# tumberger/gnark-fork

Hardware: AMD Instinct MI355X
Metric: Groth16 prove time + MSM G1 throughput (Mscalar-mul/s) BN254 2^24 R1CS, 1/2/4/8 GPU (higher is better)
Workload: dtype u32 limbs (BN254 Fp/Fr Montgomery, integer)

## Files before the change

gnark-fork_amd/csrc/groth16.hip:

```cpp
#include "common.h"
#include "curve.cuh"
#include "stage.h"
#include <chrono>
#include <future>
#include <memory>
#include <mutex>
#include <thread>
#include <vector>
#include <cstdlib>
#include <cstring>

struct gg_domain;
struct gg_msm_base;

namespace gg {
struct MsmSort;
struct MsmScratch;
struct MsmWork;
void compute_h_device(gg_domain* d, Fr* A, Fr* B, Fr* C, Fr* H, hipStream_t st);
void msm_device(gg_msm_base* b, const Fr* scalars_dev, void* out_jac, hipStream_t st);
size_t msm_scalars_needed(gg_msm_base* b);
gg_msm_base* msm_base_create_internal(int group, const void* host_points, size_t n,
                                      const uint32_t* sidx, int window_bits, bool keep_inf, int groups);
int choose_groups_multi(const double* bytes, const int* W, int k, double extra);
bool msm_same_shape(const gg_msm_base* a, const gg_msm_base* b);
MsmSort* msm_own_sort(gg_msm_base* b);
void msm_prepare_dev(gg_msm_base* b, MsmSort* s, const Fr* scalars_dev, hipStream_t st, int slog = 0,
                     uint32_t sres = 0);
void msm_finish_dev(gg_msm_base* b, MsmSort* s, void* out_jac, hipStream_t st, MsmScratch* scr = nullptr);
MsmWork* msm_work_new();
void msm_work_delete(MsmWork* w);
MsmSort* msm_work_sort(MsmWork* w);
void msm_prepare_derived_dev(gg_msm_base* a, MsmSort* sa, gg_msm_base* b, MsmSort* sb, const uint32_t* bmap,
                             hipStream_t st);
bool msm_derivable(const gg_msm_base* a, const gg_msm_base* b);
void msm_build_bmap(const gg_msm_base* a, const gg_msm_base* b, DevBuf& bmap);
MsmScratch* msm_work_scratch(MsmWork* w);
int msm_base_window(const gg_msm_base* b);
int choose_c(size_t n, size_t point_bytes, int total_bits);
void hshard_run(gg_hshard* hs, const Fr* a, const Fr* b, const Fr* c, size_t len, bool compact, Fr* send,
                Fr* recv, gg_exchange_fn xchg, void* ctx, hipStream_t st);
size_t hshard_m(const gg_hshard* hs, int* rank, int* world, int* log_n);
Fr* hshard_h(gg_hshard* hs);
int hshard_curve(const gg_hshard* hs);
}

struct DistH {
    gg_hshard* hs;
    gg_exchange_fn xchg;
    void* ctx;
    gg::Fr *send, *recv;
};

using namespace gg;

struct CurveBn254 {
    using FrT = Fr;
    using G1F = Fp;
    using G2F = Fp2;
    static constexpr int curve = GG_CURVE_BN254, g1 = GG_G1, g2 = GG_G2, total_bits = 255;
};
struct CurveBls12381 {
    using FrT = FrBls;
    using G1F = FpBls;
    using G2F = Fp2Bls;
    static constexpr int curve = GG_CURVE_BLS12_381, g1 = GG_BLS12_381_G1, g2 = GG_BLS12_381_G2, total_bits = 256;
};
struct PointSizes {
    size_t g1a, g2a, g1j, g2j;
};
static PointSizes point_sizes(int curve) {
    if (curve == GG_CURVE_BN254) return {64, 128, 96, 192};
    return {96, 192, 144, 288};
}

struct WireBases {
    gg_msm_base_t A = nullptr, B = nullptr, K = nullptr, B2 = nullptr;
    bool share_AK = false, share_B = false;
    bool derive_B = false;
    DevBuf bmap;
    int groups = 1;
    WireBases() = default;
    WireBases(const WireBases&) = delete;
    WireBases& operator=(const WireBases&) = delete;
    ~WireBases() {
        for (gg_msm_base_t b : {A, B, K, B2})
            if (b) gg_msm_base_release(b);
    }
};

struct WorkSet {
    MsmWork *A = nullptr, *B = nullptr, *K = nullptr, *B2 = nullptr;
    WorkSet() {
        A = msm_work_new();
        B = msm_work_new();
        K = msm_work_new();
        B2 = msm_work_new();
    }
    WorkSet(const WorkSet&) = delete;
    WorkSet& operator=(const WorkSet&) = delete;
    ~WorkSet() {
        for (MsmWork* w : {A, B, K, B2})
            if (w) msm_work_delete(w);
    }
};

struct gg_groth16_pk {
    int curve = GG_CURVE_BN254;
    int log_n = 0;
    size_t n = 0;
    gg_domain_t dom = nullptr;
    std::shared_ptr<WireBases> wb;
    gg_msm_base_t A = nullptr, B = nullptr, K = nullptr, Z = nullptr, B2 = nullptr;
    int slog = 0;
    uint32_t spart = 0;
    std::unique_ptr<WorkSet> work;
    uint8_t alpha[96], beta[96], delta[96], beta2[192], delta2[192];
    size_t n_wires = 0, nb_public = 0;
    size_t wire_lo = 0, wire_hi = 0, z_lo = 0, nZ = 0;
    bool share_AK = false, share_B = false;
    DevBuf wires, sa, sb, sc;
    hipStream_t s0 = nullptr, s1 = nullptr, s2 = nullptr, s3 = nullptr, s4 = nullptr;
    TaskQueue tq[5];
    hipStream_t* const* active() {
        act[0] = &s0, act[1] = &s1, act[2] = &s2, act[3] = &s3, act[4] = &s4;
        return act;
    }
    hipStream_t* act[5] = {};
    hipStream_t hprio = nullptr;
    std::unique_ptr<Stager> stager;
    int device = 0;
    std::mutex mu;
    ~gg_groth16_pk() {
        stager.reset();
        work.reset();
        wb.reset();
        if (Z) gg_msm_base_release(Z);
        if (dom) gg_domain_release(dom);
        task_streams_release(tq, 5, device);
        if (hprio) (void)hipStreamDestroy(hprio);
    }
};

static thread_local double g_timings[9];
static thread_local double g_ext[3];

static void ck(int rc) {
    if (rc != GG_OK) throw Error(rc, gg_last_error());
}

static std::shared_ptr<WireBases> wire_bases_build(int curve, int log_n, const void* g1_A, size_t nA,
                                                   const void* g1_B, size_t nB, const void* g1_K, size_t nK,
                                                   const void* g2_B, const uint8_t* inf_A, const uint8_t* inf_B,
                                                   size_t n_wires, size_t nb_public, const uint32_t* k_wire_index,
                                                   size_t lo, size_t hi, size_t nZ) {
    GG_CHECK(inf_A && inf_B, GG_ERR_INVALID_ARG, "null infinity masks");
    GG_CHECK(nb_public <= n_wires, GG_ERR_INVALID_ARG, "nb_public > n_wires");
    GG_CHECK(lo <= hi && hi <= n_wires, GG_ERR_INVALID_ARG, "bad wire shard range");
    GG_CHECK(curve == GG_CURVE_BN254 || curve == GG_CURVE_BLS12_381, GG_ERR_INVALID_ARG, "bad curve");
    const PointSizes ps = point_sizes(curve);
    const int g1 = curve == GG_CURVE_BN254 ? GG_G1 : GG_BLS12_381_G1;
    const int g2 = curve == GG_CURVE_BN254 ? GG_G2 : GG_BLS12_381_G2;
    const int tbits = curve == GG_CURVE_BN254 ? 255 : 256;
    std::vector<uint32_t> ia, ib, ik;
    for (size_t i = lo; i < hi; i++) {
        if (!inf_A[i]) ia.push_back((uint32_t)(i - lo));
        if (!inf_B[i]) ib.push_back((uint32_t)(i - lo));
    }
    GG_CHECK(ia.size() == nA, GG_ERR_INVALID_ARG, "len(pk.G1.A) != n_wires - NbInfinityA (shard)");
    GG_CHECK(ib.size() == nB, GG_ERR_INVALID_ARG, "len(pk.G1.B) != n_wires - NbInfinityB (shard)");
    ik.resize(nK);
    const size_t k0 = std::max(lo, nb_public);
    for (size_t i = 0; i < nK; i++) {
        size_t w = k_wire_index ? (size_t)k_wire_index[i] : k0 + i;
        GG_CHECK(w >= lo && w < hi, GG_ERR_INVALID_ARG, "K wire index outside the shard");
        ik[i] = (uint32_t)(w - lo);
    }
    GG_CHECK(nA == 0 || g1_A, GG_ERR_INVALID_ARG, "null g1_A");
    GG_CHECK(nB == 0 || (g1_B && g2_B), GG_ERR_INVALID_ARG, "null g1_B / g2_B");
    GG_CHECK(nK == 0 || g1_K, GG_ERR_INVALID_ARG, "null g1_K");
    const size_t nw = hi - lo;
    const int cAK = choose_c(std::max<size_t>(nw, 1), ps.g1a, tbits);
    int cB = choose_c(std::max<size_t>(nB, 1), 128, tbits);
    const bool try_derive = getenv("GG_G16_B_DERIVE") && atoi(getenv("GG_G16_B_DERIVE")) != 0;
    if (try_derive && cAK >= cB && cAK - cB <= 2 && nB) cB = cAK;
    if (const char* e = getenv("GG_G16_B_WINDOW")) cB = std::max(4, std::min(24, atoi(e)));
    const int cZ = choose_c(std::max<size_t>(nZ, 1), ps.g1a, tbits);
    auto wb = std::make_shared<WireBases>();
    {
        auto W = [&](int c) { return (tbits + c - 1) / c; };
        const double g1a = (double)ps.g1a, g2a = (double)ps.g2a;
        const double bytes[5] = {W(cAK) * (double)nw * g1a, W(cAK) * (double)nw * g1a, W(cB) * (double)nB * g1a,
                                 W(cB) * (double)nB * g2a, W(cZ) * (double)nZ * g1a};
        const int ws[5] = {W(cAK), W(cAK), W(cB), W(cB), W(cZ)};
        const double extra = 16.0 * (W(cAK) * (double)nw + W(cB) * (double)nB + W(cZ) * (double)nZ) +
                             12.0 * 32.0 * (double)((size_t)1 << log_n);
        wb->groups = choose_groups_multi(bytes, ws, 5, extra);
    }
    {
        const size_t pb = ps.g1a;
        std::vector<uint8_t> dense(nw * pb, 0);
        for (size_t j = 0; j < nA; j++) memcpy(&dense[(size_t)ia[j] * pb], (const uint8_t*)g1_A + j * pb, pb);
        wb->A = msm_base_create_internal(g1, dense.data(), nw, nullptr, cAK, true, wb->groups);
        std::fill(dense.begin(), dense.end(), 0);
        for (size_t j = 0; j < nK; j++) memcpy(&dense[(size_t)ik[j] * pb], (const uint8_t*)g1_K + j * pb, pb);
        wb->K = msm_base_create_internal(g1, dense.data(), nw, nullptr, cAK, true, wb->groups);
    }
    wb->B = msm_base_create_internal(g1, g1_B, nB, ib.data(), cB, false, wb->groups);
    wb->B2 = msm_base_create_internal(g2, g2_B, nB, ib.data(), msm_base_window(wb->B), false, wb->groups);
    wb->share_AK = msm_same_shape(wb->A, wb->K);
    wb->share_B = msm_same_shape(wb->B, wb->B2);
    if (try_derive && wb->share_B && msm_derivable(wb->A, wb->B)) {
        msm_build_bmap(wb->A, wb->B, wb->bmap);
        wb->derive_B = true;
    }
    return wb;
}

static void h_priority_ab(gg_groth16_pk* pk) {
    if (!(getenv("GG_G16_H_PRIORITY") && atoi(getenv("GG_G16_H_PRIORITY")))) return;
    if (!pk->hprio) create_copy_stream(&pk->hprio);
    pk->s1 = pk->hprio;
}

static void pk_finish(gg_groth16_pk* pk, std::shared_ptr<WireBases> wb, int curve, int log_n,
                      const void* omega_mont, const void* coset_gen_mont, const void* g1_Z, size_t z_lo, size_t nZ,
                      const void* alpha1, const void* beta1, const void* delta1, const void* beta2,
                      const void* delta2, size_t n_wires, size_t nb_public, size_t lo, size_t hi, int slog,
                      uint32_t spart) {
    GG_CHECK(omega_mont && coset_gen_mont && alpha1 && beta1 && delta1 && beta2 && delta2,
             GG_ERR_INVALID_ARG, "null argument");
    GG_CHECK(log_n >= 0 && log_n <= 28, GG_ERR_INVALID_ARG, "log_n out of range");
    const PointSizes ps = point_sizes(curve);
    const int g1 = curve == GG_CURVE_BN254 ? GG_G1 : GG_BLS12_381_G1;
    const int tbits = curve == GG_CURVE_BN254 ? 255 : 256;
    pk->curve = curve;
    pk->log_n = log_n;
    pk->n = (size_t)1 << log_n;
    pk->n_wires = n_wires;
    pk->nb_public = nb_public;
    pk->wire_lo = lo;
    pk->wire_hi = hi;
    pk->z_lo = z_lo;
    pk->nZ = nZ;
    const size_t nz_full = pk->n > 1 ? pk->n - 1 : 0;
    GG_CHECK(z_lo + nZ <= nz_full, GG_ERR_INVALID_ARG,
             "Z shard beyond domain cardinality - 1 (setup.go:266)");
    GG_CHECK(nZ == 0 || g1_Z, GG_ERR_INVALID_ARG, "null g1_Z");
    GG_HIP(hipGetDevice(&pk->device));
    memcpy(pk->alpha, alpha1, ps.g1a);
    memcpy(pk->beta, beta1, ps.g1a);
    memcpy(pk->delta, delta1, ps.g1a);
    memcpy(pk->beta2, beta2, ps.g2a);
    memcpy(pk->delta2, delta2, ps.g2a);
    ck(gg_domain_create_ex(curve, log_n, omega_mont, coset_gen_mont, &pk->dom));
    pk->wb = std::move(wb);
    pk->A = pk->wb->A;
    pk->B = pk->wb->B;
    pk->K = pk->wb->K;
    pk->B2 = pk->wb->B2;
    pk->share_AK = pk->wb->share_AK;
    pk->share_B = pk->wb->share_B;
    if (slog) {
        int cmin = 64;
        for (gg_msm_base_t b : {pk->A, pk->B})
            if (msm_scalars_needed(b)) cmin = std::min(cmin, msm_base_window(b));
        GG_CHECK(slog <= cmin - 2, GG_ERR_INVALID_ARG, "bucket stripe too fine for the tables' windows");
        GG_CHECK(spart < (1u << slog), GG_ERR_INVALID_ARG, "stripe part out of range");
        pk->slog = slog;
        pk->spart = spart;
        pk->work.reset(new WorkSet());
    }
    const int cZ = choose_c(std::max<size_t>(nZ, 1), ps.g1a, tbits);
    pk->Z = msm_base_create_internal(g1, g1_Z, nZ, nullptr, cZ, false, pk->wb->groups);
    int cur = 0;
    GG_HIP(hipGetDevice(&cur));
    task_streams_init(pk->active(), pk->tq, 5, cur, true);
    h_priority_ab(pk);
}

static void pk_build(gg_groth16_pk* pk, int curve, int log_n, const void* omega_mont, const void* coset_gen_mont,
                     const void* g1_A, size_t nA, const void* g1_B, size_t nB, const void* g1_Z,
                     size_t z_lo, size_t nZ, const void* g1_K, size_t nK, const void* alpha1,
                     const void* beta1, const void* delta1, const void* g2_B, const void* beta2,
                     const void* delta2, const uint8_t* inf_A, const uint8_t* inf_B, size_t n_wires,
                     size_t nb_public, const uint32_t* k_wire_index, size_t lo, size_t hi) {
    GG_CHECK(log_n >= 0 && log_n <= 28, GG_ERR_INVALID_ARG, "log_n out of range");
    auto wb = wire_bases_build(curve, log_n, g1_A, nA, g1_B, nB, g1_K, nK, g2_B, inf_A, inf_B, n_wires, nb_public,
                               k_wire_index, lo, hi, nZ);
    pk_finish(pk, std::move(wb), curve, log_n, omega_mont, coset_gen_mont, g1_Z, z_lo, nZ, alpha1, beta1, delta1,
              beta2, delta2, n_wires, nb_public, lo, hi, 0, 0);
}

namespace gg {
std::shared_ptr<WireBases> g16_wire_bases(int curve, int log_n, const void* g1_A, size_t nA, const void* g1_B,
                                          size_t nB, const void* g1_K, size_t nK, const void* g2_B,
                                          const uint8_t* inf_A, const uint8_t* inf_B, size_t n_wires,
                                          size_t nb_public, const uint32_t* k_wire_index, size_t nZ) {
    return wire_bases_build(curve, log_n, g1_A, nA, g1_B, nB, g1_K, nK, g2_B, inf_A, inf_B, n_wires, nb_public,
                            k_wire_index, 0, n_wires, nZ);
}
gg_groth16_pk* g16_stripe_shard(std::shared_ptr<WireBases> wb, int curve, int log_n, const void* omega_mont,
                                const void* coset_gen_mont, const void* g1_Z, size_t z_lo, size_t nZ,
                                const void* alpha1, const void* beta1, const void* delta1, const void* beta2,
                                const void* delta2, size_t n_wires, size_t nb_public, int slog, uint32_t spart) {
    std::unique_ptr<gg_groth16_pk> pk(new gg_groth16_pk());
    pk_finish(pk.get(), std::move(wb), curve, log_n, omega_mont, coset_gen_mont, g1_Z, z_lo, nZ, alpha1, beta1,
              delta1, beta2, delta2, n_wires, nb_public, 0, n_wires, slog, spart);
    return pk.release();
}
int g16_wire_window(int curve, size_t n_wires, size_t nB) {
    const PointSizes ps = point_sizes(curve);
    const int tbits = curve == GG_CURVE_BN254 ? 255 : 256;
    int c = 64;
    if (n_wires) c = std::min(c, choose_c(n_wires, ps.g1a, tbits));
    if (nB) c = std::min(c, choose_c(nB, 128, tbits));
    return c;
}
void g16_restream(gg_groth16_pk* pk, bool dedicated) {
    std::lock_guard<std::mutex> lk(pk->mu);
    task_streams_switch(pk->active(), pk->tq, 5, pk->device, dedicated);
    h_priority_ab(pk);
}
}

extern "C" int gg_groth16_pk_create_ex(int curve, int log_n, const void* omega_mont, const void* coset_gen_mont,
                                       const void* g1_A, size_t nA, const void* g1_B, size_t nB,
                                       const void* g1_Z, size_t nZ, const void* g1_K, size_t nK,
                                       const void* alpha1, const void* beta1, const void* delta1,
                                       const void* g2_B, const void* beta2, const void* delta2,
                                       const uint8_t* inf_A, const uint8_t* inf_B, size_t n_wires,
                                       size_t nb_public, const uint32_t* k_wire_index,
                                       gg_groth16_pk_t* out) {
    GG_CAPI_BEGIN
    GG_CHECK(out, GG_ERR_INVALID_ARG, "null argument");
    GG_CHECK(log_n >= 0 && log_n <= 28, GG_ERR_INVALID_ARG, "log_n out of range");
    const size_t n = (size_t)1 << log_n;
    GG_CHECK(nZ + 1 == n || (n == 1 && nZ == 0), GG_ERR_INVALID_ARG,
             "len(pk.G1.Z) must be domain cardinality - 1 (setup.go:266)");
    std::unique_ptr<gg_groth16_pk> pk(new gg_groth16_pk());
    if (!k_wire_index) GG_CHECK(nb_public + nK <= n_wires, GG_ERR_INVALID_ARG, "len(pk.G1.K) too large");
    pk_build(pk.get(), curve, log_n, omega_mont, coset_gen_mont, g1_A, nA, g1_B, nB, g1_Z, 0, nZ, g1_K, nK,
             alpha1, beta1, delta1, g2_B, beta2, delta2, inf_A, inf_B, n_wires, nb_public,
             k_wire_index, 0, n_wires);
    *out = pk.release();
    GG_CAPI_END
}

extern "C" int gg_groth16_pk_create(int log_n, const void* omega_mont, const void* coset_gen_mont,
                                    const void* g1_A, size_t nA, const void* g1_B, size_t nB,
                                    const void* g1_Z, size_t nZ, const void* g1_K, size_t nK,
                                    const void* alpha1, const void* beta1, const void* delta1,
                                    const void* g2_B, const void* beta2, const void* delta2,
                                    const uint8_t* inf_A, const uint8_t* inf_B, size_t n_wires,
                                    size_t nb_public, const uint32_t* k_wire_index,
                                    gg_groth16_pk_t* out) {
    return gg_groth16_pk_create_ex(GG_CURVE_BN254, log_n, omega_mont, coset_gen_mont, g1_A, nA, g1_B, nB, g1_Z,
                                   nZ, g1_K, nK, alpha1, beta1, delta1, g2_B, beta2, delta2, inf_A, inf_B,
                                   n_wires, nb_public, k_wire_index, out);
}

extern "C" int gg_groth16_pk_create_shard_ex(int curve, int log_n, const void* omega_mont,
                                             const void* coset_gen_mont, const void* g1_A, size_t nA,
                                             const void* g1_B, size_t nB, const void* g1_Z, size_t z_lo,
                                             size_t nZ, const void* g1_K, size_t nK, const void* alpha1,
                                             const void* beta1, const void* delta1, const void* g2_B,
                                             const void* beta2, const void* delta2, const uint8_t* inf_A,
                                             const uint8_t* inf_B, size_t n_wires, size_t nb_public,
                                             const uint32_t* k_wire_index, size_t wire_lo, size_t wire_hi,
                                             gg_groth16_pk_t* out) {
    GG_CAPI_BEGIN
    GG_CHECK(out, GG_ERR_INVALID_ARG, "null argument");
    std::unique_ptr<gg_groth16_pk> pk(new gg_groth16_pk());
    pk_build(pk.get(), curve, log_n, omega_mont, coset_gen_mont, g1_A, nA, g1_B, nB, g1_Z, z_lo, nZ, g1_K, nK,
             alpha1, beta1, delta1, g2_B, beta2, delta2, inf_A, inf_B, n_wires, nb_public, k_wire_index, wire_lo,
             wire_hi);
    *out = pk.release();
    GG_CAPI_END
}

extern "C" int gg_groth16_pk_create_shard(int log_n, const void* omega_mont, const void* coset_gen_mont,
                                          const void* g1_A, size_t nA, const void* g1_B, size_t nB,
                                          const void* g1_Z, size_t z_lo, size_t nZ, const void* g1_K,
                                          size_t nK, const void* alpha1, const void* beta1,
                                          const void* delta1, const void* g2_B, const void* beta2,
                                          const void* delta2, const uint8_t* inf_A,
                                          const uint8_t* inf_B, size_t n_wires, size_t nb_public,
                                          const uint32_t* k_wire_index, size_t wire_lo,
                                          size_t wire_hi, gg_groth16_pk_t* out) {
    return gg_groth16_pk_create_shard_ex(GG_CURVE_BN254, log_n, omega_mont, coset_gen_mont, g1_A, nA, g1_B, nB,
                                         g1_Z, z_lo, nZ, g1_K, nK, alpha1, beta1, delta1, g2_B, beta2, delta2,
                                         inf_A, inf_B, n_wires, nb_public, k_wire_index, wire_lo, wire_hi, out);
}

extern "C" int gg_groth16_pk_create_stripe_ex(int curve, int log_n, const void* omega_mont,
                                              const void* coset_gen_mont, const void* g1_A, size_t nA,
                                              const void* g1_B, size_t nB, const void* g1_Z, size_t z_lo,
                                              size_t nZ, const void* g1_K, size_t nK, const void* alpha1,
                                              const void* beta1, const void* delta1, const void* g2_B,
                                              const void* beta2, const void* delta2, const uint8_t* inf_A,
                                              const uint8_t* inf_B, size_t n_wires, size_t nb_public,
                                              const uint32_t* k_wire_index, int stripe_log, int stripe_part,
                                              gg_groth16_pk_t* out) {
    GG_CAPI_BEGIN
    GG_CHECK(out, GG_ERR_INVALID_ARG, "null argument");
    GG_CHECK(stripe_log >= 0 && stripe_log <= 8 && stripe_part >= 0 && stripe_part < (1 << stripe_log),
             GG_ERR_INVALID_ARG, "stripe_log in [0, 8], stripe_part < 2^stripe_log");
    GG_CHECK(log_n >= 0 && log_n <= 28, GG_ERR_INVALID_ARG, "log_n out of range");
    if (!k_wire_index) GG_CHECK(nb_public + nK <= n_wires, GG_ERR_INVALID_ARG, "len(pk.G1.K) too large");
    auto wb = wire_bases_build(curve, log_n, g1_A, nA, g1_B, nB, g1_K, nK, g2_B, inf_A, inf_B, n_wires, nb_public,
                               k_wire_index, 0, n_wires, nZ);
    *out = g16_stripe_shard(std::move(wb), curve, log_n, omega_mont, coset_gen_mont, g1_Z, z_lo, nZ, alpha1, beta1,
                            delta1, beta2, delta2, n_wires, nb_public, stripe_log, (uint32_t)stripe_part);
    GG_CAPI_END
}

extern "C" int gg_groth16_pk_stripe(gg_groth16_pk_t pk, int* stripe_log, int* stripe_part) {
    GG_CAPI_BEGIN
    GG_CHECK(pk, GG_ERR_INVALID_ARG, "null key");
    if (stripe_log) *stripe_log = pk->slog;
    if (stripe_part) *stripe_part = (int)pk->spart;
    GG_CAPI_END
}

extern "C" int gg_groth16_pk_base_info(gg_groth16_pk_t pk, int which, size_t* n_points, int* window_bits,
                                       int* n_windows) {
    GG_CAPI_BEGIN
    GG_CHECK(pk && which >= 0 && which <= 4, GG_ERR_INVALID_ARG, "bad argument");
    gg_msm_base_t b[5] = {pk->A, pk->B, pk->K, pk->Z, pk->B2};
    return gg_msm_base_info(b[which], n_points, window_bits, n_windows);
    GG_CAPI_END
}

extern "C" int gg_groth16_pk_base_layout(gg_groth16_pk_t pk, int which, int* groups, int* stored_windows,
                                         size_t* table_bytes) {
    GG_CAPI_BEGIN
    GG_CHECK(pk && which >= 0 && which <= 4, GG_ERR_INVALID_ARG, "bad argument");
    gg_msm_base_t b[5] = {pk->A, pk->B, pk->K, pk->Z, pk->B2};
    return gg_msm_base_layout(b[which], groups, stored_windows, table_bytes);
    GG_CAPI_END
}

extern "C" int gg_groth16_pk_release(gg_groth16_pk_t pk) {
    GG_CAPI_BEGIN
    delete pk;
    GG_CAPI_END
}

static double now_ms() {
    return std::chrono::duration<double, std::milli>(
               std::chrono::steady_clock::now().time_since_epoch())
        .count();
}

template <class T>
static T from_bytes(const void* p) {
    T x;
    memcpy(&x, p, sizeof(T));
    return x;
}

struct G16Partials {
    alignas(16) uint8_t a[144], b1[144], k[144], z[144];
    alignas(16) uint8_t b2[288];
};
static void set_g1_inf(int curve, void* p) {
    if (curve == GG_CURVE_BN254) {
        G1Jac j = G1Jac::inf();
        memcpy(p, &j, sizeof(j));
    } else {
        Jac<FpBls> j = Jac<FpBls>::inf();
        memcpy(p, &j, sizeof(j));
    }
}
static void partials_put(int curve, const G16Partials& p, void* out) {
    const PointSizes ps = point_sizes(curve);
    uint8_t* o = (uint8_t*)out;
    memcpy(o, p.a, ps.g1j);
    memcpy(o + ps.g1j, p.b1, ps.g1j);
    memcpy(o + 2 * ps.g1j, p.k, ps.g1j);
    memcpy(o + 3 * ps.g1j, p.z, ps.g1j);
    memcpy(o + 4 * ps.g1j, p.b2, ps.g2j);
}
static void partials_get(int curve, const void* in, G16Partials& p) {
    const PointSizes ps = point_sizes(curve);
    const uint8_t* q = (const uint8_t*)in;
    memcpy(p.a, q, ps.g1j);
    memcpy(p.b1, q + ps.g1j, ps.g1j);
    memcpy(p.k, q + 2 * ps.g1j, ps.g1j);
    memcpy(p.z, q + 3 * ps.g1j, ps.g1j);
    memcpy(p.b2, q + 4 * ps.g1j, ps.g2j);
}

struct Joiner {
    std::vector<gg::Task<void>>& v;
    ~Joiner() {
        for (auto& t : v)
            if (t.valid()) t.wait();
    }
};

static void prove_device(gg_groth16_pk* pk, const void* wires, const void* sol_a,
                         const void* sol_b, const void* sol_c, size_t n_cons,
                         bool inputs_on_device, void* h_dev_out, G16Partials& out,
                         const DistH* dh = nullptr) {
    double t0 = now_ms();
    const size_t n = pk->n;
    const size_t nbytes = n * 32;
    const size_t nw_shard = pk->wire_hi - pk->wire_lo;
    const Fr* wdev = (const Fr*)wires;
    if (!inputs_on_device) {
        if (!pk->stager) pk->stager.reset(new Stager(pk->device));
        pk->wires.reserve(std::max<size_t>(nw_shard, 1) * 32);
        pk->stager->upload(pk->wires.p, (const uint8_t*)wires + pk->wire_lo * 32, nw_shard * 32);
        const hipStream_t cons[4] = {pk->s0, pk->s2, pk->s3, pk->s4};
        pk->stager->ready(cons, 4);
        wdev = pk->wires.as<Fr>();
    } else {
        wdev += pk->wire_lo;
    }
    double t_up = now_ms();

    set_g1_inf(pk->curve, out.z);
    double t_h = 0, t_z = 0, t_a = 0, t_b = 0, t_k = 0, t_upabc = 0;
    std::mutex emu;
    std::string werr;
    int wcode = GG_OK;
    const int dev = pk->device;
    auto guarded = [&](auto fn) {
        return [&, fn]() {
            try {
                GG_HIP(hipSetDevice(dev));
                fn();
            } catch (const Error& e) {
                std::lock_guard<std::mutex> g(emu);
                if (wcode == GG_OK) { werr = e.what(); wcode = e.code; }
            } catch (const std::exception& e) {
                std::lock_guard<std::mutex> g(emu);
                if (wcode == GG_OK) { werr = e.what(); wcode = GG_ERR_INTERNAL; }
            }
        };
    };
    const bool serial = getenv("GG_G16_SERIAL") && atoi(getenv("GG_G16_SERIAL"));
    std::vector<gg::Task<void>> workers;
    Joiner joiner{workers};
    auto spawn = [&](auto fn) {
        if (serial) fn();
        else workers.push_back(gg::run_task(fn));
    };
    auto inputs_abc = [&](Fr*& A, Fr*& B, Fr*& C, size_t& len) {
        const void* src[3] = {sol_a, sol_b, sol_c};
        Fr* dst[3] = {pk->sa.as<Fr>(), pk->sb.as<Fr>(), pk->sc.as<Fr>()};
        len = n_cons;
        const double a = now_ms();
        if (inputs_on_device) {
            for (int i = 0; i < 3; i++) {
                if (dh) { dst[i] = (Fr*)src[i]; continue; }
                if (n_cons) GG_HIP(hipMemcpyAsync(dst[i], src[i], n_cons * 32, hipMemcpyDeviceToDevice, pk->s1));
                if (n_cons < n) GG_HIP(hipMemsetAsync((char*)dst[i] + n_cons * 32, 0, nbytes - n_cons * 32, pk->s1));
            }
        } else if (dh) {
            int rank = 0, world = 1, lg = 0;
            hshard_m(dh->hs, &rank, &world, &lg);
            len = n_cons > (size_t)rank ? (n_cons - (size_t)rank + world - 1) / world : 0;
            for (int i = 0; i < 3; i++)
                pk->stager->upload_strided(dst[i], src[i], 32, (size_t)rank, (size_t)world, len);
            pk->stager->ready(&pk->s1, 1);
        } else {
            for (int i = 0; i < 3; i++) {
                if (n_cons < n) GG_HIP(hipMemsetAsync((char*)dst[i] + n_cons * 32, 0, nbytes - n_cons * 32, pk->s1));
                pk->stager->upload(dst[i], src[i], n_cons * 32);
            }
            pk->stager->ready(&pk->s1, 1);
        }
        t_upabc = now_ms() - a;
        A = dst[0];
        B = dst[1];
        C = dst[2];
    };
    pk->sa.reserve(nbytes);
    pk->sb.reserve(nbytes);
    pk->sc.reserve(nbytes);
    if (dh) spawn(guarded([&] {
        Fr *A, *B, *C;
        size_t len;
        double a = now_ms();
        inputs_abc(A, B, C, len);
        const bool compact = !inputs_on_device;
        hshard_run(dh->hs, A, B, C, len, compact, dh->send, dh->recv, dh->xchg, dh->ctx, pk->s1);
        GG_WAIT_STREAM(pk->s1);
        double b = now_ms();
        t_h = b - a;
        msm_device(pk->Z, hshard_h(dh->hs), out.z, pk->s1);
        t_z = now_ms() - b;
    }));
    else spawn(guarded([&] {
        Fr *A, *B, *C;
        size_t len;
        double a = now_ms();
        inputs_abc(A, B, C, len);
        compute_h_device(pk->dom, A, B, C, A, pk->s1);
        GG_WAIT_STREAM(pk->s1);
        double b = now_ms();
        t_h = b - a;
        if (h_dev_out) GG_HIP(hipMemcpyAsync(h_dev_out, A, nbytes, hipMemcpyDeviceToDevice, pk->s1));
        if (n > 1) msm_device(pk->Z, A + pk->z_lo, out.z, pk->s1);
        t_z = now_ms() - b;
    }));
    MsmSort *sAK = nullptr, *sB = nullptr, *sK = nullptr, *sB2 = nullptr;
    MsmScratch *xA = nullptr, *xB = nullptr, *xK = nullptr, *xB2 = nullptr;
    WorkSet* ws = pk->work.get();
    guarded([&] {
        sAK = ws ? msm_work_sort(ws->A) : msm_own_sort(pk->A);
        sB = ws ? msm_work_sort(ws->B) : msm_own_sort(pk->B);
        sK = pk->share_AK ? sAK : (ws ? msm_work_sort(ws->K) : msm_own_sort(pk->K));
        sB2 = pk->share_B ? sB : (ws ? msm_work_sort(ws->B2) : msm_own_sort(pk->B2));
        if (ws) {
            xA = msm_work_scratch(ws->A);
            xB = msm_work_scratch(ws->B);
            xK = msm_work_scratch(ws->K);
            xB2 = msm_work_scratch(ws->B2);
        }
        msm_prepare_dev(pk->A, sAK, wdev, pk->s2, pk->slog, pk->spart);
        if (pk->wb->derive_B)
            msm_prepare_derived_dev(pk->A, sAK, pk->B, sB, pk->wb->bmap.as<uint32_t>(), pk->s3);
        else
            msm_prepare_dev(pk->B, sB, wdev, pk->s3, pk->slog, pk->spart);
        if (!pk->share_AK) msm_prepare_dev(pk->K, sK, wdev, pk->s4, pk->slog, pk->spart);
        if (!pk->share_B) msm_prepare_dev(pk->B2, sB2, wdev, pk->s0, pk->slog, pk->spart);
    })();
    double t2 = now_ms(), te = t2;
    if (wcode == GG_OK) {
        spawn(guarded([&] { double a = now_ms(); msm_finish_dev(pk->A, sAK, out.a, pk->s2, xA); t_a = now_ms() - a; }));
        spawn(guarded([&] { double a = now_ms(); msm_finish_dev(pk->B, sB, out.b1, pk->s3, xB); t_b = now_ms() - a; }));
        spawn(guarded([&] { double a = now_ms(); msm_finish_dev(pk->K, sK, out.k, pk->s4, xK); t_k = now_ms() - a; }));
        t2 = now_ms();
        guarded([&] { msm_finish_dev(pk->B2, sB2, out.b2, pk->s0, xB2); })();
        te = now_ms();
    }
    for (auto& w : workers) w.wait();
    if (wcode != GG_OK) throw Error(wcode, werr);
    g_timings[0] = t_up - t0;
    g_timings[1] = t_h;
    g_timings[2] = t_a;
    g_timings[3] = t_b;
    g_timings[4] = t_k;
    g_timings[5] = t_z;
    g_timings[6] = te - t2;
    g_ext[0] = t_upabc;
}

template <class Cv>
struct G16Fixed {
    typename Cv::FrT rc, sc;
    Jac<typename Cv::G1F> rd, sd, krd;
    Jac<typename Cv::G2F> sd2;
};

template <class Cv>
static gg::Task<G16Fixed<Cv>> fixed_terms_async(const void* delta_aff, const void* delta2_aff, const void* r_mont,
                                                   const void* s_mont) {
    using G1 = typename Cv::G1F;
    using G2 = typename Cv::G2F;
    using FrT = typename Cv::FrT;
    const Affine<G1> delta = from_bytes<Affine<G1>>(delta_aff);
    const Affine<G2> delta2 = from_bytes<Affine<G2>>(delta2_aff);
    const FrT r = from_bytes<FrT>(r_mont), s = from_bytes<FrT>(s_mont);
    return gg::run_task([delta, delta2, r, s] {
        G16Fixed<Cv> f;
        FrT kr = -(r * s);
        f.rc = from_mont(r);
        f.sc = from_mont(s);
        FrT krc = from_mont(kr);
        Jac<G1> dl = Jac<G1>::from_affine(delta);
        auto f_rd = gg::run_task([&] { return jac_mul(dl, f.rc.v); });
        auto f_sd = gg::run_task([&] { return jac_mul(dl, f.sc.v); });
        auto f_sd2 = gg::run_task([&] { return jac_mul(Jac<G2>::from_affine(delta2), f.sc.v); });
        f.krd = jac_mul(dl, krc.v);
        f.rd = f_rd.get();
        f.sd = f_sd.get();
        f.sd2 = f_sd2.get();
        return f;
    });
}

template <class Cv>
static void g16_combine(const G16Partials& p, const G16Fixed<Cv>& f, const void* alpha_aff, const void* beta_aff,
                        const void* beta2_aff, void* ar_aff, void* bs_aff, void* krs_aff) {
    using G1 = typename Cv::G1F;
    using G2 = typename Cv::G2F;
    const Affine<G1> alpha = from_bytes<Affine<G1>>(alpha_aff), beta = from_bytes<Affine<G1>>(beta_aff);
    const Affine<G2> beta2 = from_bytes<Affine<G2>>(beta2_aff);
    const Jac<G1> pa = from_bytes<Jac<G1>>(p.a), pb1 = from_bytes<Jac<G1>>(p.b1), pk = from_bytes<Jac<G1>>(p.k),
                  pz = from_bytes<Jac<G1>>(p.z);
    const Jac<G2> pb2 = from_bytes<Jac<G2>>(p.b2);
    Jac<G1> ar = jac_add(jac_add_affine(pa, alpha), f.rd);
    Jac<G1> bs1 = jac_add(jac_add_affine(pb1, beta), f.sd);
    auto f_sar = gg::run_task([&] { return jac_mul(ar, f.sc.v); });
    Jac<G1> rbs = jac_mul(bs1, f.rc.v);
    Jac<G1> krs = jac_add(jac_add(pk, f.krd), pz);
    krs = jac_add(krs, f_sar.get());
    krs = jac_add(krs, rbs);
    Jac<G2> bs = jac_add_affine(jac_add(pb2, f.sd2), beta2);
    const Affine<G1> o_ar = jac_to_affine(ar), o_krs = jac_to_affine(krs);
    const Affine<G2> o_bs = jac_to_affine(bs);
    memcpy(ar_aff, &o_ar, sizeof(o_ar));
    memcpy(krs_aff, &o_krs, sizeof(o_krs));
    memcpy(bs_aff, &o_bs, sizeof(o_bs));
}

template <class Cv>
static void prove_whole(gg_groth16_pk* pk, const void* wires, const void* sol_a, const void* sol_b,
                        const void* sol_c, size_t n_cons, bool on_dev, const void* r_mont, const void* s_mont,
                        void* ar_aff, void* bs_aff, void* krs_aff, void* h_dev_out) {
    double t0 = now_ms();
    auto fixed = fixed_terms_async<Cv>(pk->delta, pk->delta2, r_mont, s_mont);
    G16Partials p;
    prove_device(pk, wires, sol_a, sol_b, sol_c, n_cons, on_dev, h_dev_out, p);
    double tep = now_ms();
    g16_combine<Cv>(p, fixed.get(), pk->alpha, pk->beta, pk->beta2, ar_aff, bs_aff, krs_aff);
    double tend = now_ms();
    g_timings[7] = tend - tep;
    g_timings[8] = tend - t0;
}

static void check_prove_args(gg_groth16_pk_t pk, const void* wires, size_t n_wires, const void* a,
                             const void* b, const void* c, size_t n_cons) {
    GG_CHECK(pk && wires && a && b && c, GG_ERR_INVALID_ARG, "null argument");
    GG_CHECK(n_wires == pk->n_wires, GG_ERR_INVALID_ARG, "len(wires) != pk wires");
    GG_CHECK(n_cons <= pk->n, GG_ERR_INVALID_ARG, "nbConstraints > domain cardinality");
}

extern "C" int gg_groth16_prove(gg_groth16_pk_t pk, const void* wires, size_t n_wires,
                                const void* sol_a, const void* sol_b, const void* sol_c,
                                size_t n_cons, int inputs_on_device, const void* r_mont,
                                const void* s_mont, void* ar_aff, void* bs_aff, void* krs_aff,
                                void* h_dev_out) {
    GG_CAPI_BEGIN
    check_prove_args(pk, wires, n_wires, sol_a, sol_b, sol_c, n_cons);
    GG_CHECK(r_mont && s_mont && ar_aff && bs_aff && krs_aff, GG_ERR_INVALID_ARG, "null argument");
    GG_CHECK(pk->wire_lo == 0 && pk->wire_hi == pk->n_wires && pk->z_lo == 0 && pk->slog == 0 &&
                 pk->nZ == (pk->n > 1 ? pk->n - 1 : 0),
             GG_ERR_INVALID_ARG, "gg_groth16_prove needs the whole key; a shard proves with "
                                 "gg_groth16_prove_partial + gg_groth16_finalize");
    g_ext[1] = now_ms();
    std::lock_guard<std::mutex> lk(pk->mu);
    g_ext[0] = 0;
    if (pk->curve == GG_CURVE_BN254)
        prove_whole<CurveBn254>(pk, wires, sol_a, sol_b, sol_c, n_cons, inputs_on_device != 0, r_mont, s_mont,
                                ar_aff, bs_aff, krs_aff, h_dev_out);
    else
        prove_whole<CurveBls12381>(pk, wires, sol_a, sol_b, sol_c, n_cons, inputs_on_device != 0, r_mont, s_mont,
                                   ar_aff, bs_aff, krs_aff, h_dev_out);
    g_ext[2] = now_ms();
    if (kAccumProbe) {
        set_last_error("traffic-probe build (GG_ACCUM_PROBE): the MSM sums are wrong, the proof is NOT valid");
        return GG_REHEARSAL;
    }
    GG_CAPI_END
}

extern "C" int gg_groth16_prove_partial(gg_groth16_pk_t pk, const void* wires, size_t n_wires,
                                        const void* sol_a, const void* sol_b, const void* sol_c,
                                        size_t n_cons, int inputs_on_device, void* partials,
                                        void* h_dev_out) {
    GG_CAPI_BEGIN
    check_prove_args(pk, wires, n_wires, sol_a, sol_b, sol_c, n_cons);
    GG_CHECK(partials, GG_ERR_INVALID_ARG, "null argument");
    std::lock_guard<std::mutex> lk(pk->mu);
    g_ext[0] = 0;
    double t0 = now_ms();
    G16Partials p;
    prove_device(pk, wires, sol_a, sol_b, sol_c, n_cons, inputs_on_device != 0, h_dev_out, p);
    partials_put(pk->curve, p, partials);
    g_timings[7] = 0;
    g_timings[8] = now_ms() - t0;
    GG_PROBE_GUARD();
    GG_CAPI_END
}

extern "C" int gg_groth16_prove_partial_dist(gg_groth16_pk_t pk, gg_hshard_t hs, const void* wires,
                                             size_t n_wires, const void* sol_a, const void* sol_b,
                                             const void* sol_c, size_t n_cons, int inputs_on_device,
                                             gg_exchange_fn xchg, void* xchg_ctx, void* send_dev,
                                             void* recv_dev, void* partials) {
    GG_CAPI_BEGIN
    check_prove_args(pk, wires, n_wires, sol_a, sol_b, sol_c, n_cons);
    GG_CHECK(hs && xchg && send_dev && recv_dev && partials, GG_ERR_INVALID_ARG, "null argument");
    GG_CHECK(hshard_curve(hs) == pk->curve, GG_ERR_INVALID_ARG, "hshard and key are over different curves");
    int rank = 0, world = 1, log_n = 0;
    size_t m = hshard_m(hs, &rank, &world, &log_n);
    GG_CHECK(log_n == pk->log_n, GG_ERR_INVALID_ARG, "hshard and key have different domains");
    GG_CHECK(pk->z_lo == (size_t)rank * m && pk->nZ == std::min(m, pk->n - 1 - pk->z_lo),
             GG_ERR_INVALID_ARG, "key shard must own Z positions [rank*m, (rank+1)*m)");
    std::lock_guard<std::mutex> lk(pk->mu);
    g_ext[0] = 0;
    double t0 = now_ms();
    G16Partials p;
    DistH dh{hs, xchg, xchg_ctx, (Fr*)send_dev, (Fr*)recv_dev};
    prove_device(pk, wires, sol_a, sol_b, sol_c, n_cons, inputs_on_device != 0, nullptr, p, &dh);
    partials_put(pk->curve, p, partials);
    g_timings[7] = 0;
    g_timings[8] = now_ms() - t0;
    GG_PROBE_GUARD();
    GG_CAPI_END
}

extern "C" int gg_groth16_finalize_ex(int curve, const void* alpha1, const void* beta1, const void* delta1,
                                      const void* beta2, const void* delta2, const void* partials,
                                      const void* r_mont, const void* s_mont, void* ar_aff, void* bs_aff,
                                      void* krs_aff) {
    GG_CAPI_BEGIN
    GG_CHECK(alpha1 && beta1 && delta1 && beta2 && delta2 && partials && r_mont && s_mont && ar_aff && bs_aff &&
                 krs_aff,
             GG_ERR_INVALID_ARG, "null argument");
    GG_CHECK(curve == GG_CURVE_BN254 || curve == GG_CURVE_BLS12_381, GG_ERR_INVALID_ARG, "bad curve");
    G16Partials p;
    partials_get(curve, partials, p);
    if (curve == GG_CURVE_BN254) {
        auto fixed = fixed_terms_async<CurveBn254>(delta1, delta2, r_mont, s_mont);
        g16_combine<CurveBn254>(p, fixed.get(), alpha1, beta1, beta2, ar_aff, bs_aff, krs_aff);
    } else {
        auto fixed = fixed_terms_async<CurveBls12381>(delta1, delta2, r_mont, s_mont);
        g16_combine<CurveBls12381>(p, fixed.get(), alpha1, beta1, beta2, ar_aff, bs_aff, krs_aff);
    }
    GG_CAPI_END
}

struct gg_g16_fixed {
    int curve = GG_CURVE_BN254;
    gg::Task<G16Fixed<CurveBn254>> bn;
    gg::Task<G16Fixed<CurveBls12381>> bls;
};

extern "C" int gg_groth16_finalize_begin(int curve, const void* delta1, const void* delta2, const void* r_mont,
                                         const void* s_mont, gg_g16_fixed_t* out) {
    GG_CAPI_BEGIN
    GG_CHECK(delta1 && delta2 && r_mont && s_mont && out, GG_ERR_INVALID_ARG, "null argument");
    GG_CHECK(curve == GG_CURVE_BN254 || curve == GG_CURVE_BLS12_381, GG_ERR_INVALID_ARG, "bad curve");
    std::unique_ptr<gg_g16_fixed> h(new gg_g16_fixed());
    h->curve = curve;
    if (curve == GG_CURVE_BN254) h->bn = fixed_terms_async<CurveBn254>(delta1, delta2, r_mont, s_mont);
    else h->bls = fixed_terms_async<CurveBls12381>(delta1, delta2, r_mont, s_mont);
    *out = h.release();
    GG_CAPI_END
}

extern "C" int gg_groth16_finalize_end(gg_g16_fixed_t h, const void* alpha1, const void* beta1, const void* beta2,
                                       const void* partials, void* ar_aff, void* bs_aff, void* krs_aff) {
    GG_CAPI_BEGIN
    GG_CHECK(h, GG_ERR_INVALID_ARG, "null handle");
    std::unique_ptr<gg_g16_fixed> own(h);
    if (!partials) return GG_OK;
    GG_CHECK(alpha1 && beta1 && beta2 && ar_aff && bs_aff && krs_aff, GG_ERR_INVALID_ARG, "null argument");
    G16Partials p;
    partials_get(h->curve, partials, p);
    if (h->curve == GG_CURVE_BN254) g16_combine<CurveBn254>(p, h->bn.get(), alpha1, beta1, beta2, ar_aff, bs_aff, krs_aff);
    else g16_combine<CurveBls12381>(p, h->bls.get(), alpha1, beta1, beta2, ar_aff, bs_aff, krs_aff);
    GG_CAPI_END
}

extern "C" int gg_groth16_finalize(const void* alpha1, const void* beta1, const void* delta1,
                                   const void* beta2, const void* delta2, const void* partials,
                                   const void* r_mont, const void* s_mont, void* ar_aff,
                                   void* bs_aff, void* krs_aff) {
    return gg_groth16_finalize_ex(GG_CURVE_BN254, alpha1, beta1, delta1, beta2, delta2, partials, r_mont, s_mont,
                                  ar_aff, bs_aff, krs_aff);
}

extern "C" int gg_groth16_last_timings_ex(double* ms, int cap) {
    GG_CAPI_BEGIN
    GG_CHECK(ms && cap >= 0, GG_ERR_INVALID_ARG, "null argument");
    double all[12];
    memcpy(all, g_timings, sizeof(g_timings));
    all[9] = g_ext[0];
    all[10] = g_ext[1];
    all[11] = g_ext[2];
    memcpy(ms, all, sizeof(double) * (size_t)std::min(cap, 12));
    GG_CAPI_END
}

extern "C" int gg_groth16_last_timings(double* ms9) {
    GG_CAPI_BEGIN
    GG_CHECK(ms9, GG_ERR_INVALID_ARG, "null argument");
    memcpy(ms9, g_timings, sizeof(g_timings));
    GG_CAPI_END
}
```

gnark-fork_amd/csrc/msm.hip:

```cpp
#include "msm_impl.cuh"
#include <cmath>

namespace gg {
void create_base_g1(gg_msm_base* b, const void* points, size_t n, int on_device,
                    const uint32_t* sidx, int window_bits, bool keep_inf, int groups);
void create_base_g2(gg_msm_base* b, const void* points, size_t n, int on_device,
                    const uint32_t* sidx, int window_bits, bool keep_inf, int groups);
void create_base_bls(gg_msm_base* b, const void* points, size_t n, int on_device,
                     const uint32_t* sidx, int window_bits, bool keep_inf, int groups);
void create_base_bls2(gg_msm_base* b, const void* points, size_t n, int on_device,
                      const uint32_t* sidx, int window_bits, bool keep_inf, int groups);
void msm_run_bls2(gg_msm_base* b, MsmWork* w, const Fr* scalars_dev, void* out_jac, hipStream_t st);
void msm_finish_bls2(gg_msm_base* b, MsmSort* s, MsmScratch* scr, void* out_jac, hipStream_t st);
void msm_run_g1(gg_msm_base* b, MsmWork* w, const Fr* scalars_dev, void* out_jac, hipStream_t st);
void msm_run_g2(gg_msm_base* b, MsmWork* w, const Fr* scalars_dev, void* out_jac, hipStream_t st);
void msm_run_bls(gg_msm_base* b, MsmWork* w, const Fr* scalars_dev, void* out_jac, hipStream_t st);
void msm_finish_g1(gg_msm_base* b, MsmSort* s, MsmScratch* scr, void* out_jac, hipStream_t st);
void msm_finish_g2(gg_msm_base* b, MsmSort* s, MsmScratch* scr, void* out_jac, hipStream_t st);
void msm_finish_bls(gg_msm_base* b, MsmSort* s, MsmScratch* scr, void* out_jac, hipStream_t st);
void msm_run_batch_g1(gg_msm_base* b, MsmWork* w, const VecPtrs& vp, int nvec, void* const* out_jac, hipStream_t st);
void msm_run_batch_g2(gg_msm_base* b, MsmWork* w, const VecPtrs& vp, int nvec, void* const* out_jac, hipStream_t st);
void msm_run_batch_bls(gg_msm_base* b, MsmWork* w, const VecPtrs& vp, int nvec, void* const* out_jac, hipStream_t st);
void msm_run_batch_bls2(gg_msm_base* b, MsmWork* w, const VecPtrs& vp, int nvec, void* const* out_jac,
                        hipStream_t st);
}

using namespace gg;

extern "C" int gg_msm_base_create(int group, const void* points, size_t n, int points_on_device,
                                  const uint32_t* scalar_index, int window_bits,
                                  gg_msm_base_t* out) {
    GG_CAPI_BEGIN
    GG_CHECK(out, GG_ERR_INVALID_ARG, "null out");
    GG_CHECK(group == GG_G1 || group == GG_G2 || group == GG_BLS12_381_G1 || group == GG_BLS12_381_G2,
             GG_ERR_INVALID_ARG, "group must be GG_G1, GG_G2, GG_BLS12_381_G1 or GG_BLS12_381_G2");
    GG_CHECK(n == 0 || points, GG_ERR_INVALID_ARG, "null points");
    GG_CHECK(n < 0x80000000ull, GG_ERR_INVALID_ARG, "n too large");
    std::unique_ptr<gg_msm_base> b(new gg_msm_base());
    b->group = group;
    if (group == GG_G1) create_base_g1(b.get(), points, n, points_on_device, scalar_index, window_bits, false, 0);
    else if (group == GG_G2) create_base_g2(b.get(), points, n, points_on_device, scalar_index, window_bits, false, 0);
    else if (group == GG_BLS12_381_G1) create_base_bls(b.get(), points, n, points_on_device, scalar_index, window_bits, false, 0);
    else create_base_bls2(b.get(), points, n, points_on_device, scalar_index, window_bits, false, 0);
    *out = b.release();
    GG_CAPI_END
}

extern "C" int gg_msm_base_release(gg_msm_base_t b) {
    GG_CAPI_BEGIN
    delete b;
    GG_CAPI_END
}

extern "C" int gg_msm_base_layout(gg_msm_base_t b, int* groups, int* stored_windows, size_t* table_bytes) {
    GG_CAPI_BEGIN
    GG_CHECK(b, GG_ERR_INVALID_ARG, "null base");
    if (groups) *groups = b->G;
    if (stored_windows) *stored_windows = b->Ws;
    if (table_bytes) *table_bytes = b->pts.bytes;
    GG_CAPI_END
}

extern "C" int gg_msm_base_info(gg_msm_base_t b, size_t* n_points, int* window_bits, int* n_windows) {
    GG_CAPI_BEGIN
    GG_CHECK(b, GG_ERR_INVALID_ARG, "null base");
    if (n_points) *n_points = b->n;
    if (window_bits) *window_bits = b->c;
    if (n_windows) *n_windows = b->W;
    GG_CAPI_END
}

namespace gg {
void msm_device_work(gg_msm_base* b, MsmWork* w, const Fr* scalars_dev, void* out_jac, hipStream_t st) {
    if (b->group == GG_G1) msm_run_g1(b, w, scalars_dev, out_jac, st);
    else if (b->group == GG_G2) msm_run_g2(b, w, scalars_dev, out_jac, st);
    else if (b->group == GG_BLS12_381_G1) msm_run_bls(b, w, scalars_dev, out_jac, st);
    else msm_run_bls2(b, w, scalars_dev, out_jac, st);
}
void msm_device_work_batch(gg_msm_base* b, MsmWork* w, const Fr* const* scalars_dev, int nvec, void* const* out_jac,
                           hipStream_t st) {
    GG_CHECK(nvec >= 1 && nvec <= kMaxBatch, GG_ERR_INVALID_ARG, "batch of 1..4 scalar vectors");
    VecPtrs vp{};
    for (int v = 0; v < nvec; v++) vp.p[v] = scalars_dev[v];
    if (b->group == GG_G1) msm_run_batch_g1(b, w, vp, nvec, out_jac, st);
    else if (b->group == GG_G2) msm_run_batch_g2(b, w, vp, nvec, out_jac, st);
    else if (b->group == GG_BLS12_381_G1) msm_run_batch_bls(b, w, vp, nvec, out_jac, st);
    else msm_run_batch_bls2(b, w, vp, nvec, out_jac, st);
}
static void msm_device_locked(gg_msm_base* b, const Fr* scalars_dev, void* out_jac, hipStream_t st) {
    msm_device_work(b, &b->own, scalars_dev, out_jac, st);
}
void msm_device(gg_msm_base* b, const Fr* scalars_dev, void* out_jac, hipStream_t st) {
    std::lock_guard<std::mutex> lk(b->mu);
    msm_device_locked(b, scalars_dev, out_jac, st);
}
gg_msm_base* msm_base_create_internal(int group, const void* host_points, size_t n,
                                      const uint32_t* sidx, int window_bits, bool keep_inf, int groups) {
    std::unique_ptr<gg_msm_base> b(new gg_msm_base());
    b->group = group;
    if (group == GG_G1) create_base_g1(b.get(), host_points, n, 0, sidx, window_bits, keep_inf, groups);
    else if (group == GG_G2) create_base_g2(b.get(), host_points, n, 0, sidx, window_bits, keep_inf, groups);
    else if (group == GG_BLS12_381_G1) create_base_bls(b.get(), host_points, n, 0, sidx, window_bits, keep_inf, groups);
    else create_base_bls2(b.get(), host_points, n, 0, sidx, window_bits, keep_inf, groups);
    return b.release();
}
bool msm_same_shape(const gg_msm_base* a, const gg_msm_base* b) {
    if (a->n != b->n || a->c != b->c || a->W != b->W || a->G != b->G || a->has_sidx != b->has_sidx) return false;
    if (!a->has_sidx || a->n == 0) return true;
    std::vector<uint32_t> x(a->n), y(b->n);
    GG_HIP(hipMemcpy(x.data(), a->sidx.p, a->n * 4, hipMemcpyDeviceToHost));
    GG_HIP(hipMemcpy(y.data(), b->sidx.p, b->n * 4, hipMemcpyDeviceToHost));
    return x == y;
}
MsmSort* msm_own_sort(gg_msm_base* b) { return &b->own.sort; }
MsmWork* msm_work_new() { return new MsmWork(); }
void msm_work_delete(MsmWork* w) { delete w; }
int msm_base_window(const gg_msm_base* b) { return b->c; }
int msm_base_groups(const gg_msm_base* b) { return b->G; }
void msm_prepare_dev(gg_msm_base* b, MsmSort* s, const Fr* scalars_dev, hipStream_t st, int slog, uint32_t sres) {
    if (b->n) msm_prepare(b, s, scalars_dev, st, slog, sres);
}
void msm_finish_dev(gg_msm_base* b, MsmSort* s, void* out_jac, hipStream_t st, MsmScratch* scr) {
    if (!scr) scr = &b->own.scr;
    if (b->group == GG_G1) msm_finish_g1(b, s, scr, out_jac, st);
    else if (b->group == GG_G2) msm_finish_g2(b, s, scr, out_jac, st);
    else if (b->group == GG_BLS12_381_G1) msm_finish_bls(b, s, scr, out_jac, st);
    else msm_finish_bls2(b, s, scr, out_jac, st);
}
void msm_prepare_derived_dev(gg_msm_base* a, MsmSort* sa, gg_msm_base* b, MsmSort* sb, const uint32_t* bmap,
                             hipStream_t st) {
    if (b->n) msm_prepare_derived(a, sa, b, sb, bmap, st);
}
__global__ void k_bmap_scatter(const uint32_t* sidx, size_t nb_pts, uint32_t na, uint32_t* bmap) {
    const size_t j = (size_t)blockIdx.x * blockDim.x + threadIdx.x;
    if (j < nb_pts && sidx[j] < na) bmap[sidx[j]] = (uint32_t)j;
}
void msm_build_bmap(const gg_msm_base* a, const gg_msm_base* b, DevBuf& bmap) {
    bmap.alloc(std::max<size_t>(a->n, 1) * 4);
    GG_HIP(hipMemset(bmap.p, 0xff, std::max<size_t>(a->n, 1) * 4));
    if (b->n) {
        hipLaunchKernelGGL(k_bmap_scatter, dim3(grid_for(b->n, 256)), dim3(256), 0, hipStreamPerThread,
                           b->sidx.as<uint32_t>(), b->n, (uint32_t)a->n, bmap.as<uint32_t>());
        GG_HIP(hipGetLastError());
    }
    GG_WAIT_STREAM(hipStreamPerThread);
}
bool msm_derivable(const gg_msm_base* a, const gg_msm_base* b) {
    if (a->c != b->c || a->W != b->W || a->G != b->G || a->has_sidx || !b->has_sidx) return false;
    for (int w = 0; w < a->W; w++)
        if (a->win.bits[w] != b->win.bits[w] || a->win.off[w] != b->win.off[w]) return false;
    return (double)a->W * (double)a->n < 4294967295.0;
}
MsmSort* msm_work_sort(MsmWork* w) { return &w->sort; }
MsmScratch* msm_work_scratch(MsmWork* w) { return &w->scr; }
bool msm_batch_fits(size_t n, int W, int c, int G, int nvec) {
    int kp = 1;
    while (kp < nvec) kp <<= 1;
    const double entries = (double)W * (double)n * (double)nvec;
    const double buckets = (double)G * std::ldexp(1.0, c - 1) * (double)kp;
    return entries + 64.0 < 4294967296.0 && buckets < 2147483648.0;
}
bool msm_base_batch_fits(const gg_msm_base* b, int nvec) { return msm_batch_fits(b->n, b->W, b->c, b->G, nvec); }
size_t msm_scalars_needed(gg_msm_base* b) {
    return b->has_sidx ? (b->n ? (size_t)b->max_sidx + 1 : 0) : b->n;
}
}

extern "C" int gg_msm(gg_msm_base_t b, const void* scalars, size_t n_scalars, int scalars_on_device,
                      void* out_jac, void* hip_stream) {
    GG_CAPI_BEGIN
    GG_CHECK(b && out_jac, GG_ERR_INVALID_ARG, "null argument");
    hipStream_t st = hip_stream ? (hipStream_t)hip_stream : hipStreamPerThread;
    size_t need = msm_scalars_needed(b);
    GG_CHECK(n_scalars >= need, GG_ERR_INVALID_ARG,
             "scalar vector shorter than the points/index map require");
    GG_CHECK(need == 0 || scalars, GG_ERR_INVALID_ARG, "null scalars");
    std::lock_guard<std::mutex> lk(b->mu);
    const Fr* sdev = (const Fr*)scalars;
    if (!scalars_on_device && need) {
        b->own.scr.scal.reserve(need * 32);
        GG_HIP(hipMemcpyAsync(b->own.scr.scal.p, scalars, need * 32, hipMemcpyHostToDevice, st));
        sdev = b->own.scr.scal.as<Fr>();
    }
    msm_device_locked(b, sdev, out_jac, st);
    GG_PROBE_GUARD();
    GG_CAPI_END
}

extern "C" int gg_msm_batch(gg_msm_base_t b, const void* const* scalars, int n_vectors, size_t n_scalars,
                            int scalars_on_device, void* const* out_jac, void* hip_stream) {
    GG_CAPI_BEGIN
    GG_CHECK(b && scalars && out_jac, GG_ERR_INVALID_ARG, "null argument");
    GG_CHECK(n_vectors >= 1 && n_vectors <= kMaxBatch, GG_ERR_INVALID_ARG, "n_vectors must be 1..4");
    hipStream_t st = hip_stream ? (hipStream_t)hip_stream : hipStreamPerThread;
    const size_t need = msm_scalars_needed(b);
    GG_CHECK(n_scalars >= need, GG_ERR_INVALID_ARG, "scalar vector shorter than the points/index map require");
    for (int v = 0; v < n_vectors; v++) {
        GG_CHECK(need == 0 || scalars[v], GG_ERR_INVALID_ARG, "null scalars");
        GG_CHECK(out_jac[v], GG_ERR_INVALID_ARG, "null out_jac");
    }
    GG_CHECK(msm_base_batch_fits(b, n_vectors), GG_ERR_UNSUPPORTED,
             "MSM batch too large for 32-bit sort indices (gg_msm_batch_shape); use one MSM per vector");
    std::lock_guard<std::mutex> lk(b->mu);
    const Fr* sdev[kMaxBatch] = {};
    if (!scalars_on_device && need) {
        b->own.scr.scal.reserve((size_t)n_vectors * need * 32);
        for (int v = 0; v < n_vectors; v++) {
            sdev[v] = b->own.scr.scal.as<Fr>() + (size_t)v * need;
            GG_HIP(hipMemcpyAsync((void*)sdev[v], scalars[v], need * 32, hipMemcpyHostToDevice, st));
        }
    } else {
        for (int v = 0; v < n_vectors; v++) sdev[v] = (const Fr*)scalars[v];
    }
    msm_device_work_batch(b, &b->own, sdev, n_vectors, out_jac, st);
    GG_PROBE_GUARD();
    GG_CAPI_END
}

extern "C" int gg_msm_stripe(gg_msm_base_t b, const void* scalars, size_t n_scalars, int scalars_on_device,
                             int stripe_log, int stripe_part, void* out_jac, void* hip_stream) {
    GG_CAPI_BEGIN
    GG_CHECK(b && out_jac, GG_ERR_INVALID_ARG, "null argument");
    GG_CHECK(stripe_log >= 0 && stripe_log <= b->c - 2 && stripe_part >= 0 && stripe_part < (1 << stripe_log),
             GG_ERR_INVALID_ARG, "bucket stripe out of range (stripe_log <= window_bits - 2, part < 2^stripe_log)");
    hipStream_t st = hip_stream ? (hipStream_t)hip_stream : hipStreamPerThread;
    size_t need = msm_scalars_needed(b);
    GG_CHECK(n_scalars >= need, GG_ERR_INVALID_ARG,
             "scalar vector shorter than the points/index map require");
    GG_CHECK(need == 0 || scalars, GG_ERR_INVALID_ARG, "null scalars");
    std::lock_guard<std::mutex> lk(b->mu);
    const Fr* sdev = (const Fr*)scalars;
    if (!scalars_on_device && need) {
        b->own.scr.scal.reserve(need * 32);
        GG_HIP(hipMemcpyAsync(b->own.scr.scal.p, scalars, need * 32, hipMemcpyHostToDevice, st));
        sdev = b->own.scr.scal.as<Fr>();
    }
    if (b->n == 0) {
        msm_device_work(b, &b->own, sdev, out_jac, st);
        return GG_OK;
    }
    msm_prepare_dev(b, &b->own.sort, sdev, st, stripe_log, (uint32_t)stripe_part);
    msm_finish_dev(b, &b->own.sort, out_jac, st, nullptr);
    GG_PROBE_GUARD();
    GG_CAPI_END
}

extern "C" int gg_msm_batch_shape(size_t n_points, int window_bits, int n_windows, int groups, int n_vectors) {
    GG_CAPI_BEGIN
    GG_CHECK(window_bits >= 2 && window_bits <= 30 && n_windows >= 1 && groups >= 1 && (groups & (groups - 1)) == 0,
             GG_ERR_INVALID_ARG, "window_bits 2..30, n_windows >= 1, groups a power of two");
    GG_CHECK(n_vectors >= 1 && n_vectors <= kMaxBatch, GG_ERR_INVALID_ARG, "n_vectors must be 1..4");
    GG_CHECK(msm_batch_fits(n_points, n_windows, window_bits, groups, n_vectors), GG_ERR_UNSUPPORTED,
             "MSM batch too large for 32-bit sort indices: n_vectors * n_windows * n_points entries must stay "
             "below 2^32 and n_vectors' bucket spaces below 2^31 buckets; use one MSM per vector");
    GG_CAPI_END
}
```

gnark-fork_amd/csrc/msm_bls.hip:

```cpp
#include "msm_impl.cuh"

namespace gg {
void create_base_bls(gg_msm_base* b, const void* points, size_t n, int on_device,
                     const uint32_t* sidx, int window_bits, bool keep_inf, int groups) {
    create_base<FpBls>(b, points, n, on_device, sidx, window_bits, keep_inf, 1, groups);
}
void msm_run_bls(gg_msm_base* b, MsmWork* w, const Fr* scalars_dev, void* out_jac, hipStream_t st) {
    Jac<FpBls> j = xyzz_to_jac(msm_run<FpBls>(b, w, scalars_dev, st));
    memcpy(out_jac, &j, sizeof(j));
}
void msm_finish_bls(gg_msm_base* b, MsmSort* s, MsmScratch* scr, void* out_jac, hipStream_t st) {
    Jac<FpBls> j = xyzz_to_jac(msm_finish<FpBls>(b, s, scr, st));
    memcpy(out_jac, &j, sizeof(j));
}
void msm_run_batch_bls(gg_msm_base* b, MsmWork* w, const VecPtrs& vp, int nvec, void* const* out_jac,
                        hipStream_t st) {
    Xyzz<FpBls> r[kMaxBatch];
    msm_run_batch<FpBls>(b, w, vp, nvec, st, r);
    for (int v = 0; v < nvec; v++) {
        Jac<FpBls> j = xyzz_to_jac(r[v]);
        memcpy(out_jac[v], &j, sizeof(j));
    }
}
}
```

gnark-fork_amd/csrc/msm_g1.hip:

```cpp
#include "msm_impl.cuh"

namespace gg {
void create_base_g1(gg_msm_base* b, const void* points, size_t n, int on_device,
                    const uint32_t* sidx, int window_bits, bool keep_inf, int groups) {
    create_base<Fp>(b, points, n, on_device, sidx, window_bits, keep_inf, 0, groups);
}
void msm_run_g1(gg_msm_base* b, MsmWork* w, const Fr* scalars_dev, void* out_jac, hipStream_t st) {
    G1Jac j = xyzz_to_jac(msm_run<Fp>(b, w, scalars_dev, st));
    memcpy(out_jac, &j, sizeof(j));
}
void msm_finish_g1(gg_msm_base* b, MsmSort* s, MsmScratch* scr, void* out_jac, hipStream_t st) {
    G1Jac j = xyzz_to_jac(msm_finish<Fp>(b, s, scr, st));
    memcpy(out_jac, &j, sizeof(j));
}
void msm_run_batch_g1(gg_msm_base* b, MsmWork* w, const VecPtrs& vp, int nvec, void* const* out_jac,
                        hipStream_t st) {
    Xyzz<Fp> r[kMaxBatch];
    msm_run_batch<Fp>(b, w, vp, nvec, st, r);
    for (int v = 0; v < nvec; v++) {
        G1Jac j = xyzz_to_jac(r[v]);
        memcpy(out_jac[v], &j, sizeof(j));
    }
}
}
```

gnark-fork_amd/csrc/msm_impl.cuh:

```cuda
#pragma once
#include "common.h"
#include "curve.cuh"
#include "field29.cuh"
#include "prof.h"
#include <mutex>
#include <vector>
#include <algorithm>
#include <memory>
#include <cmath>
#include <cstdlib>
#include <cstring>

struct gg_msm_base;

namespace gg {

template <class T>
__device__ __forceinline__ T ld(const T* p) {
    static_assert(sizeof(T) % 16 == 0, "16B multiple");
    T r;
    const uint4* s = reinterpret_cast<const uint4*>(p);
    uint4* d = reinterpret_cast<uint4*>(&r);
#pragma unroll
    for (int i = 0; i < (int)(sizeof(T) / 16); i++) d[i] = s[i];
    return r;
}
template <class T>
__device__ __forceinline__ void st(T* p, const T& v) {
    uint4* d = reinterpret_cast<uint4*>(p);
    const uint4* s = reinterpret_cast<const uint4*>(&v);
#pragma unroll
    for (int i = 0; i < (int)(sizeof(T) / 16); i++) d[i] = s[i];
}

__global__ void k_scan_block(const uint32_t* in, uint32_t* out, uint32_t* sums, size_t n);
__global__ void k_scan_add(uint32_t* out, const uint32_t* sums, size_t n);
__global__ void k_set_total(uint32_t* out, const uint32_t* in, size_t n);
__global__ void k_bucket_max(const uint32_t* offsets, size_t nb, uint32_t* maxcnt);
void exclusive_scan(const uint32_t* in, uint32_t* out, size_t n, hipStream_t st,
                    std::vector<DevBuf>& tmp, int depth = 0);
int choose_c(size_t n, size_t point_bytes, int total_bits = 255);
int choose_groups(double bytes, double extra, int W);
int choose_groups_multi(const double* bytes, const int* W, int k, double extra);
inline int scalar_total_bits(int scurve) { return scurve ? 256 : 255; }
struct WinSpec {
    uint8_t bits[64];
    uint8_t off[64];
};
inline WinSpec make_windows(int c, int W, int total) {
    WinSpec ws{};
    const int q = total / W, r = total % W;
    int o = 0;
    for (int w = 0; w < W; w++) {
        ws.bits[w] = (uint8_t)(q + (w < r ? 1 : 0));
        ws.off[w] = (uint8_t)o;
        o += ws.bits[w];
    }
    (void)c;
    return ws;
}
struct MsmSort;
constexpr int kMaxBatch = 4;
struct VecPtrs {
    const void* p[kMaxBatch];
};
void sort_entries(const gg_msm_base* b, MsmSort* s, const VecPtrs& vp, hipStream_t st);
void msm_prepare(const gg_msm_base* b, MsmSort* s, const Fr* scalars_dev, hipStream_t st, int slog = 0,
                 uint32_t sres = 0);
bool msm_batch_fits(size_t n, int W, int c, int G, int nvec);
void msm_prepare_batch(const gg_msm_base* b, MsmSort* s, const VecPtrs& vp, int nvec, hipStream_t st, int slog = 0,
                       uint32_t sres = 0);
void msm_prepare_derived(const gg_msm_base* a, const MsmSort* sa, const gg_msm_base* b, MsmSort* sb,
                         const uint32_t* bmap, hipStream_t st);

constexpr uint32_t LIGHT = 16;
__device__ __forceinline__ uint32_t bucket_perm(uint32_t B, int c) {
    const uint32_t m = (1u << (c - 1)) - 1;
    return (B & ~m) | (__brev(B & m) >> (33 - c));
}
template <class F>
struct RadixOf {
    static constexpr bool on = false;
    using C = Fp29Cfg;
};
template <>
struct RadixOf<Fp> {
    static constexpr bool on = true;
    using C = Fp29Cfg;
};
template <>
struct RadixOf<Fp2> {
    static constexpr bool on = true;
    using C = Fp29Cfg;
};
template <>
struct RadixOf<FpBls> {
    static constexpr bool on = true;
    using C = FpBls28Cfg;
};
template <class C>
__global__ void __launch_bounds__(256) k_to_radix(Fe<typename C::Std>* v, size_t n) {
    const size_t i = (size_t)blockIdx.x * blockDim.x + threadIdx.x;
    if (i >= n) return;
    Fe<typename C::Std> x = v[i];
    v[i] = to_rl<C>(x);
}

template <class F>
struct PartialOf {
    using T = Xyzz<F>;
};
template <>
struct PartialOf<Fp> {
    using T = XyzzL<Fp29Cfg>;
};
template <>
struct PartialOf<FpBls> {
    using T = XyzzL<FpBls28Cfg>;
};
template <>
struct PartialOf<Fp2> {
    using T = Xyzz2_29;
};

template <class F>
struct PartialOps {
    using T = typename PartialOf<F>::T;
    using C = typename RadixOf<F>::C;
    static __device__ __forceinline__ T inf() { return inf_l<C>(); }
    static __device__ __forceinline__ T add(const T& p, const T& q) { return xyzzl_add(p, q); }
    static __device__ __forceinline__ T neg(const T& p) {
        T r = p;
        if (!is_inf_l(r)) r.y = sub<8>(Fl<C>{}, r.y);
        return r;
    }
};
template <>
struct PartialOps<Fp2> {
    using T = Xyzz2_29;
    static __device__ __forceinline__ T inf() { return inf2_29(); }
    static __device__ __forceinline__ T add(const T& p, const T& q) { return xyzz2_29_add(p, q); }
    static __device__ __forceinline__ T neg(const T& p) { return xyzz2_29_neg(p); }
};

template <class P>
__device__ __forceinline__ void range_store(const P& acc, bool first, bool last, uint32_t q, int c, size_t t,
                                            P* head, P* tail, P* S) {
    if (first) st(head + t, acc);
    else if (last) st(tail + t, acc);
    else st(S + bucket_perm(q, c), acc);
}

#ifndef GG_G2_WAVES1
#define GG_G2_WAVES1 0
#endif
#ifndef GG_G1_WAVES
#define GG_G1_WAVES 2
#endif
#ifndef GG_BLS_WAVES
#define GG_BLS_WAVES 2
#endif
template <class F>
constexpr int kAccumWaves = (GG_G2_WAVES1 && std::is_same<F, Fp2>::value) || std::is_same<F, Fp2Bls>::value
                                ? 1
                                : (std::is_same<F, Fp>::value ? GG_G1_WAVES
                                                              : (std::is_same<F, FpBls>::value ? GG_BLS_WAVES : 2));

__device__ __forceinline__ uint32_t chunk_at(const uint4& c, uint32_t k) {
    return k == 0 ? c.x : (k == 1 ? c.y : (k == 2 ? c.z : c.w));
}
__device__ __forceinline__ uint4 chunk_ld(const uint32_t* sorted, uint32_t base4) {
    return *reinterpret_cast<const uint4*>(sorted + base4);
}

#ifndef GG_ACCUM_R4LOOP
#define GG_ACCUM_R4LOOP 0
#endif
#ifndef GG_G1_PIPE
#define GG_G1_PIPE 0
#endif
#ifndef GG_PT_NT
#define GG_PT_NT 1
#endif
template <bool NT, class T>
__device__ __forceinline__ T ld_pt(const T* p) {
    if constexpr (NT) {
        typedef unsigned int u4v __attribute__((ext_vector_type(4)));
        static_assert(sizeof(T) % 16 == 0, "16B multiple");
        T r;
        const u4v* s = reinterpret_cast<const u4v*>(p);
        u4v* d = reinterpret_cast<u4v*>(&r);
#pragma unroll
        for (int i = 0; i < (int)(sizeof(T) / 16); i++) d[i] = __builtin_nontemporal_load(s + i);
        return r;
    } else {
        return ld(p);
    }
}
template <int NCH>
struct LdsRing {
    uint4* wb;
    uint32_t lane;
    __device__ __forceinline__ explicit LdsRing(uint4* lds)
        : wb(lds + (threadIdx.x >> 6) * (2u * NCH * 64u)), lane(threadIdx.x & 63u) {}
    __device__ __forceinline__ void gather(const void* src, uint32_t slot) const {
#pragma unroll
        for (int k = 0; k < NCH; k++)
            __builtin_amdgcn_global_load_lds((const void*)((const char*)src + 16 * k),
                                             (__attribute__((address_space(3))) void*)(wb + (slot * NCH + k) * 64u),
                                             16, 0, GG_PT_NT == 2 ? 2 : 0);
    }
    template <class T>
    __device__ __forceinline__ T read(uint32_t slot) const {
        static_assert(sizeof(T) == 16 * NCH, "point size");
        T r;
        uint4* d = reinterpret_cast<uint4*>(&r);
#pragma unroll
        for (int k = 0; k < NCH; k++) d[k] = wb[(slot * NCH + k) * 64u + lane];
        return r;
    }
};
#ifndef GG_RING_CHUNKS
#define GG_RING_CHUNKS 1
#endif
#ifndef GG_RING_CHUNKS_G2
#define GG_RING_CHUNKS_G2 0
#endif
struct EntryChunks {
    uint4 c0, c1;
    __device__ __forceinline__ EntryChunks(const uint32_t* sorted, uint32_t e0)
        : c0(chunk_ld(sorted, e0)), c1(chunk_ld(sorted, e0 + 4)) {}
    __device__ __forceinline__ void advance(const uint32_t* sorted, uint32_t e0, uint32_t i) {
        if (((i + 2) & 3u) == 0) {
            c0 = c1;
            c1 = chunk_ld(sorted, e0 + i + 6);
        }
    }
    __device__ __forceinline__ uint32_t next2(uint32_t i) const { return chunk_at(c0, (i + 2) & 3u); }
};
#ifndef GG_G1_LDS
#define GG_G1_LDS 1
#endif
template <class F>
constexpr bool kLdsGather = !GG_ACCUM_R4LOOP && (std::is_same<F, Fp2>::value || std::is_same<F, FpBls>::value ||
                                                 (GG_G1_LDS && std::is_same<F, Fp>::value));
template <class F>
constexpr size_t kAccumLds = kLdsGather<F> ? 4 * 2 * sizeof(Affine<F>) * 64 : 0;

template <class F, bool NT>
__global__ void __launch_bounds__(256, kAccumWaves<F>) k_accum_range(const Affine<F>* pts, const uint32_t* sorted,
                                                     const uint32_t* offsets, uint32_t nb, int c,
                                                     uint32_t K, int skip_inf, typename PartialOf<F>::T* head,
                                                     typename PartialOf<F>::T* tail, typename PartialOf<F>::T* S,
                                                     uint32_t* tbucket, uint32_t pmask) {
    const uint32_t E = offsets[nb];
    const size_t t = (size_t)blockIdx.x * blockDim.x + threadIdx.x;
    const uint64_t e0w = (uint64_t)t * K;
    if (e0w >= E) return;
    const uint32_t e0 = (uint32_t)e0w;
    const uint32_t e1 = (uint32_t)min<uint64_t>(e0w + K, E);
    uint32_t lo = 0, hi = nb;
    while (hi - lo > 1) {
        const uint32_t mid = (lo + hi) >> 1;
        if (offsets[mid] <= e0) lo = mid;
        else hi = mid;
    }
    uint32_t q = lo;
    tbucket[t] = q;
    uint32_t bnd = offsets[q + 1], bnd2 = offsets[min(q + 2, nb)];
    uint32_t seg0 = e0;
    if constexpr (std::is_same<F, Fp>::value || std::is_same<F, FpBls>::value) {
        using C = typename RadixOf<F>::C;
        XyzzL<C> acc = inf_l<C>();
        if constexpr (kLdsGather<F>) {
            extern __shared__ uint4 acc_lds[];
            const LdsRing<sizeof(Affine<F>) / 16> ring(acc_lds);
#if GG_RING_CHUNKS
            EntryChunks ec(sorted, e0);
            uint32_t v = ec.c0.x, vn = ec.c0.y;
            ring.gather(pts + (v & pmask), 0);
            for (uint32_t i = 0;; i++) {
                const uint32_t e = e0 + i;
                if (e >= e1) break;
                const uint32_t sl = i & 1u;
                const Affine<F> qp = ring.template read<Affine<F>>(sl);
                const uint32_t cv = v;
                if (e == bnd) {
                    range_store(acc, seg0 == e0, false, q, c, t, head, tail, S);
                    acc = inf_l<C>();
                    seg0 = e;
                    q++;
                    bnd = bnd2;
                    if (bnd == e) {
                        uint32_t b2;
                        do {
                            q++;
                            b2 = offsets[min(q + 1, nb)];
                        } while (b2 == e);
                        bnd = b2;
                    }
                }
                ec.advance(sorted, e0, i);
                const uint32_t nidx = (e + 1 < e1) ? vn : v;
                ring.gather(pts + (nidx & pmask), sl ^ 1u);
                v = nidx;
                vn = ec.next2(i);
                bnd2 = offsets[min(q + 2, nb)];
#else
            const uint32_t elast = e1 - 1;
            uint32_t v = sorted[e0], vn = sorted[min(e0 + 1, elast)];
            ring.gather(pts + (v & pmask), 0);
            for (uint32_t e = e0; e < e1; e++) {
                const uint32_t sl = (e - e0) & 1u;
                const Affine<F> qp = ring.template read<Affine<F>>(sl);
                const uint32_t cv = v;
                if (e == bnd) {
                    range_store(acc, seg0 == e0, false, q, c, t, head, tail, S);
                    acc = inf_l<C>();
                    seg0 = e;
                    q++;
                    bnd = bnd2;
                    if (bnd == e) {
                        uint32_t b2;
                        do {
                            q++;
                            b2 = offsets[min(q + 1, nb)];
                        } while (b2 == e);
                        bnd = b2;
                    }
                }
                const uint32_t nidx = (e + 1 < e1) ? vn : v;
                ring.gather(pts + (nidx & pmask), sl ^ 1u);
                v = nidx;
                vn = sorted[min(e + 2, elast)];
                bnd2 = offsets[min(q + 2, nb)];
#endif
                if (skip_inf && qp.is_inf()) continue;
                const Fl<C> x = unpack_l<C>(qp.x);
                Fl<C> y = unpack_l<C>(qp.y);
                if (cv >> 31) y = sub_nn<2>(Fl<C>{}, y);
                xyzzl_madd(acc, x, y);
            }
            range_store(acc, seg0 == e0, true, q, c, t, head, tail, S);
            return;
        }
#if !GG_G1_PIPE
        uint4 ch = chunk_ld(sorted, (e0 + 1) & ~3u);
        uint32_t v = sorted[e0], vn = (e0 + 1 < e1) ? chunk_at(ch, (e0 + 1) & 3u) : 0u;
        Affine<F> p = ld_pt<NT>(pts + (v & pmask));
        for (uint32_t e = e0; e < e1; e++) {
            Affine<F> qp = p;
            const uint32_t cv = v;
            if (e + 1 < e1) {
                p = ld_pt<NT>(pts + (vn & pmask));
                v = vn;
                if (e + 2 < e1) {
                    const uint32_t j = e + 2;
                    if ((j & 3u) == 0) ch = chunk_ld(sorted, j);
                    vn = chunk_at(ch, j & 3u);
                }
            }
            if (e == bnd) {
                range_store(acc, seg0 == e0, false, q, c, t, head, tail, S);
                acc = inf_l<C>();
                seg0 = e;
                do { q++; bnd = bnd2; bnd2 = offsets[min(q + 2, nb)]; } while (bnd == e);
            }
#else
        const uint32_t elast = e1 - 1;
        uint32_t v = sorted[e0], vn = sorted[min(e0 + 1, elast)];
        Affine<F> p = ld_pt<NT>(pts + (v & pmask));
        for (uint32_t e = e0; e < e1; e++) {
            Affine<F> qp = p;
            const uint32_t cv = v;
            const uint32_t nidx = (e + 1 < e1) ? vn : v;
            p = ld_pt<NT>(pts + (nidx & pmask));
            v = nidx;
            vn = sorted[min(e + 2, elast)];
            if (e == bnd) {
                range_store(acc, seg0 == e0, false, q, c, t, head, tail, S);
                acc = inf_l<C>();
                seg0 = e;
                q++;
                bnd = bnd2;
                if (bnd == e) {
                    uint32_t b2;
                    do {
                        q++;
                        b2 = offsets[min(q + 1, nb)];
                    } while (b2 == e);
                    bnd = b2;
                }
            }
            bnd2 = offsets[min(q + 2, nb)];
#endif
            if (skip_inf && qp.is_inf()) continue;
            const Fl<C> x = unpack_l<C>(qp.x);
            Fl<C> y = unpack_l<C>(qp.y);
            if (cv >> 31) y = sub_nn<2>(Fl<C>{}, y);
            xyzzl_madd(acc, x, y);
        }
        range_store(acc, seg0 == e0, true, q, c, t, head, tail, S);
        return;
    }
    if constexpr (std::is_same<F, Fp2>::value) {
#if GG_ACCUM_R4LOOP
        Xyzz2_29 acc = inf2_29();
        uint2 ch = *reinterpret_cast<const uint2*>(sorted + (e0 & ~1u));
        for (uint32_t e = e0; e < e1; e++) {
            if (e == bnd) {
                range_store(acc, seg0 == e0, false, q, c, t, head, tail, S);
                acc = inf2_29();
                seg0 = e;
                do { q++; bnd = bnd2; bnd2 = offsets[min(q + 2, nb)]; } while (bnd == e);
            }
            if ((e & 1u) == 0 && e != e0) ch = *reinterpret_cast<const uint2*>(sorted + e);
            const uint32_t cv = (e & 1u) ? ch.y : ch.x;
            const Affine<F> pt = ld(pts + (cv & pmask));
#else
        extern __shared__ uint4 acc_lds[];
        const LdsRing<8> ring(acc_lds);
        Xyzz2_29 acc = inf2_29();
#if GG_RING_CHUNKS_G2
        EntryChunks ec(sorted, e0);
        uint32_t v = ec.c0.x, vn = ec.c0.y;
        ring.gather(pts + (v & pmask), 0);
        for (uint32_t i = 0;; i++) {
            const uint32_t e = e0 + i;
            if (e >= e1) break;
            const uint32_t s = i & 1u;
#else
        const uint32_t elast = e1 - 1;
        uint32_t v = sorted[e0], vn = sorted[min(e0 + 1, elast)];
        ring.gather(pts + (v & pmask), 0);
        for (uint32_t e = e0; e < e1; e++) {
            const uint32_t s = (e - e0) & 1u;
#endif
            const Affine<F> pt = ring.template read<Affine<F>>(s);
            const uint32_t cv = v;
            if (e == bnd) {
                range_store(acc, seg0 == e0, false, q, c, t, head, tail, S);
                acc = inf2_29();
                seg0 = e;
                q++;
                bnd = bnd2;
                if (bnd == e) {
                    uint32_t b2;
                    do {
                        q++;
                        b2 = offsets[min(q + 1, nb)];
                    } while (b2 == e);
                    bnd = b2;
                }
            }
#if GG_RING_CHUNKS_G2
            ec.advance(sorted, e0, i);
            const uint32_t nidx = (e + 1 < e1) ? vn : v;
            ring.gather(pts + (nidx & pmask), s ^ 1u);
            v = nidx;
            vn = ec.next2(i);
#else
            const uint32_t nidx = (e + 1 < e1) ? vn : v;
            ring.gather(pts + (nidx & pmask), s ^ 1u);
            v = nidx;
            vn = sorted[min(e + 2, elast)];
#endif
            bnd2 = offsets[min(q + 2, nb)];
#endif
            if (skip_inf && pt.is_inf()) continue;
            const Fp2_29 x{unpack29(pt.x.a0), unpack29(pt.x.a1)};
            Fp2_29 y{unpack29(pt.y.a0), unpack29(pt.y.a1)};
            if (cv >> 31) y = Fp2_29{sub<2>(Fp29{}, y.c0), sub<2>(Fp29{}, y.c1)};
            xyzz2_29_madd(acc, x, y);
        }
        range_store(acc, seg0 == e0, true, q, c, t, head, tail, S);
        return;
    }
    if constexpr (std::is_same<typename PartialOf<F>::T, Xyzz<F>>::value) {
        Xyzz<F> acc = Xyzz<F>::inf();
        if constexpr (sizeof(F) <= 32) {
            uint32_t v = sorted[e0], vn = (e0 + 1 < e1) ? sorted[e0 + 1] : 0u;
            Affine<F> p = ld(pts + (v & pmask));
            for (uint32_t e = e0; e < e1; e++) {
                Affine<F> qp = p;
                const uint32_t cv = v;
                if (e + 1 < e1) {
                    p = ld(pts + (vn & pmask));
                    v = vn;
                    if (e + 2 < e1) vn = sorted[e + 2];
                }
                if (e == bnd) {
                    range_store(acc, seg0 == e0, false, q, c, t, head, tail, S);
                    acc = Xyzz<F>::inf();
                    seg0 = e;
                    do { q++; bnd = bnd2; bnd2 = offsets[min(q + 2, nb)]; } while (bnd == e);
                }
                if (skip_inf && qp.is_inf()) continue;
                if (cv >> 31) qp.y = -qp.y;
                xyzz_madd_inplace(acc, qp);
            }
        } else {
            for (uint32_t e = e0; e < e1; e++) {
                if (e == bnd) {
                    range_store(acc, seg0 == e0, false, q, c, t, head, tail, S);
                    acc = Xyzz<F>::inf();
                    seg0 = e;
                    do { q++; bnd = bnd2; bnd2 = offsets[min(q + 2, nb)]; } while (bnd == e);
                }
                const uint32_t v = sorted[e];
                Affine<F> p = ld(pts + (v & pmask));
                if (skip_inf && p.is_inf()) continue;
                if (v >> 31) p.y = -p.y;
                xyzz_madd_inplace(acc, p);
            }
        }
        range_store(acc, seg0 == e0, true, q, c, t, head, tail, S);
    }
}

template <int SRC, class T>
__device__ __forceinline__ T quad_bcast(const T& v) {
    static_assert(sizeof(T) % 4 == 0 && SRC >= 0 && SRC < 4, "word-sized, lane of a quad");
    T r;
    const int* s = reinterpret_cast<const int*>(&v);
    int* d = reinterpret_cast<int*>(&r);
#pragma unroll
    for (int i = 0; i < (int)(sizeof(T) / 4); i++)
        d[i] = __builtin_amdgcn_mov_dpp(s[i], SRC * 0x55, 0xf, 0xf, false);
    return r;
}

template <class T>
__device__ __forceinline__ T sel4(uint32_t k, const T& a0, const T& a1, const T& a2, const T& a3) {
    T r;
    const uint32_t* w0 = reinterpret_cast<const uint32_t*>(&a0);
    const uint32_t* w1 = reinterpret_cast<const uint32_t*>(&a1);
    const uint32_t* w2 = reinterpret_cast<const uint32_t*>(&a2);
    const uint32_t* w3 = reinterpret_cast<const uint32_t*>(&a3);
    uint32_t* d = reinterpret_cast<uint32_t*>(&r);
    const uint32_t m0 = 0u - (k == 0), m1 = 0u - (k == 1), m2 = 0u - (k == 2), m3 = 0u - (k == 3);
#pragma unroll
    for (int i = 0; i < (int)(sizeof(T) / 4); i++)
        d[i] = (w0[i] & m0) | (w1[i] & m1) | (w2[i] & m2) | (w3[i] & m3);
    return r;
}

template <class F>
__device__ __forceinline__ void xyzz_add_quad(Xyzz<F>& p, const Xyzz<F>& q, uint32_t k) {
    if (q.is_inf()) return;
    if (p.is_inf()) {
        p = q;
        return;
    }
    F m = sel4(k, p.x, p.y, q.x, q.y) * sel4(k, q.zz, q.zzz, p.zz, p.zzz);
    const F U1 = quad_bcast<0>(m), S1 = quad_bcast<1>(m);
    const F P = quad_bcast<2>(m) - U1, R = quad_bcast<3>(m) - S1;
    if (P.is_zero()) {
        p = R.is_zero() ? xyzz_dbl(p) : Xyzz<F>::inf();
        return;
    }
    m = sel4(k, P, R, p.zz, p.zzz) * sel4(k, P, R, q.zz, q.zzz);
    const F PP = quad_bcast<0>(m), RR = quad_bcast<1>(m), Z2 = quad_bcast<2>(m), Z3 = quad_bcast<3>(m);
    m = sel4(k, P, U1, Z2, P) * PP;
    const F PPP = quad_bcast<0>(m), Q = quad_bcast<1>(m), ZZ3 = quad_bcast<2>(m);
    const F X3 = RR - PPP - dbl(Q);
    const F D = Q - X3;
    m = sel4(k, R, S1, Z3, R) * sel4(k, D, PPP, PPP, D);
    p.y = quad_bcast<0>(m) - quad_bcast<1>(m);
    p.zzz = quad_bcast<2>(m);
    p.x = X3;
    p.zz = ZZ3;
}

template <class T>
__device__ __forceinline__ T shfl_xor_words(const T& v, int mask) {
    static_assert(sizeof(T) % 4 == 0, "word-sized struct");
    T r;
    const int* s = reinterpret_cast<const int*>(&v);
    int* d = reinterpret_cast<int*>(&r);
#pragma unroll
    for (int i = 0; i < (int)(sizeof(T) / 4); i++) d[i] = __shfl_xor(s[i], mask, 64);
    return r;
}

struct BucketSpan {
    uint32_t t0, t1;
    bool empty, first, direct;
};
__device__ __forceinline__ BucketSpan bucket_span(const uint32_t* offsets, uint32_t q, uint32_t E, uint32_t K) {
    BucketSpan s{};
    const uint32_t o0 = offsets[q], o1 = offsets[q + 1];
    s.empty = o0 == o1;
    if (s.empty) return s;
    s.t0 = o0 / K;
    s.t1 = (o1 - 1) / K;
    s.first = o0 == s.t0 * K;
    const uint32_t end1 = (uint32_t)min<uint64_t>((uint64_t)(s.t1 + 1) * K, E);
    s.direct = s.t0 == s.t1 && !s.first && o1 != end1;
    return s;
}

template <class F>
__global__ void __launch_bounds__(256) k_range_tree(Xyzz<F>* head, const uint32_t* tbucket,
                                                    const uint32_t* offsets, uint32_t nb, uint32_t K,
                                                    uint32_t stride, uint32_t fan) {
    const size_t g = (size_t)blockIdx.x * blockDim.x + threadIdx.x;
    const uint32_t lane = (uint32_t)g & 3;
    const size_t p = g >> 2;
    const uint32_t E = offsets[nb];
    if ((uint64_t)p * K >= E) return;
    const uint32_t q = tbucket[p];
    const BucketSpan s = bucket_span(offsets, q, E, K);
    const uint32_t m = s.t1 - s.t0;
    if (m <= LIGHT || p <= s.t0) return;
    const uint32_t j = (uint32_t)p - (s.t0 + 1);
    if (j % (fan * stride)) return;
    if (j + stride >= m) return;
    Xyzz<F> acc = ld(head + p);
    for (uint32_t k = 1; k < fan && j + k * stride < m; k++) xyzz_add_quad(acc, ld(head + p + k * stride), lane);
    if (lane == 0) st(head + p, acc);
}

template <class F>
__global__ void __launch_bounds__(256) k_bucket_combine(const Xyzz<F>* head, const Xyzz<F>* tail,
                                                        const uint32_t* offsets, uint32_t nb, int c,
                                                        uint32_t K, Xyzz<F>* S) {
    const size_t g = (size_t)blockIdx.x * blockDim.x + threadIdx.x;
    const uint32_t lane = (uint32_t)g & 3;
    const size_t q = g >> 2;
    if (q >= nb) return;
    const uint32_t E = offsets[nb];
    const BucketSpan s = bucket_span(offsets, (uint32_t)q, E, K);
    Xyzz<F>* out = S + bucket_perm((uint32_t)q, c);
    if (s.empty) {
        if (lane == 0) st(out, Xyzz<F>::inf());
        return;
    }
    if (s.direct) return;
    Xyzz<F> acc = ld((s.first ? head : tail) + s.t0);
    const uint32_t m = s.t1 - s.t0;
    if (m > LIGHT) xyzz_add_quad(acc, ld(head + s.t0 + 1), lane);
    else
        for (uint32_t t = s.t0 + 1; t <= s.t1; t++) xyzz_add_quad(acc, ld(head + t), lane);
    if (lane == 0) st(out, acc);
}

template <class F>
__global__ void __launch_bounds__(256) k_bucket_combine_r(const typename PartialOf<F>::T* headP,
                                                          const typename PartialOf<F>::T* tailP,
                                                          const typename PartialOf<F>::T* SP, const uint32_t* offsets,
                                                          uint32_t nb, int c, uint32_t K, Xyzz<F>* S) {
    const size_t g = (size_t)blockIdx.x * blockDim.x + threadIdx.x;
    const uint32_t lane = (uint32_t)g & 3;
    const size_t q = g >> 2;
    if (q >= nb) return;
    const uint32_t E = offsets[nb];
    const BucketSpan s = bucket_span(offsets, (uint32_t)q, E, K);
    const uint32_t pq = bucket_perm((uint32_t)q, c);
    Xyzz<F>* out = S + pq;
    if (s.empty) {
        if (lane == 0) st(out, Xyzz<F>::inf());
        return;
    }
    if (s.direct) {
        if (lane == 0) st(out, to_std(ld(SP + pq)));
        return;
    }
    Xyzz<F> acc = to_std(ld((s.first ? headP : tailP) + s.t0));
    const uint32_t m = s.t1 - s.t0;
    if (m > LIGHT) xyzz_add_quad(acc, to_std(ld(headP + s.t0 + 1)), lane);
    else
        for (uint32_t t = s.t0 + 1; t <= s.t1; t++) xyzz_add_quad(acc, to_std(ld(headP + t)), lane);
    if (lane == 0) st(out, acc);
}

template <class F>
__global__ void __launch_bounds__(256) k_range_tree_r(typename PartialOf<F>::T* head, const uint32_t* tbucket,
                                                      const uint32_t* offsets, uint32_t nb, uint32_t K,
                                                      uint32_t stride, uint32_t fan) {
    using O = PartialOps<F>;
    const size_t p = (size_t)blockIdx.x * blockDim.x + threadIdx.x;
    const uint32_t E = offsets[nb];
    if ((uint64_t)p * K >= E) return;
    const BucketSpan s = bucket_span(offsets, tbucket[p], E, K);
    const uint32_t m = s.t1 - s.t0;
    if (m <= LIGHT || p <= s.t0) return;
    const uint32_t j = (uint32_t)p - (s.t0 + 1);
    if (j % (fan * stride) || j + stride >= m) return;
    typename O::T acc = ld(head + p);
    for (uint32_t k = 1; k < fan && j + k * stride < m; k++) acc = O::add(acc, ld(head + p + k * stride));
    st(head + p, acc);
}

template <class F>
__global__ void __launch_bounds__(256) k_partials_to_std(const typename PartialOf<F>::T* in, size_t n,
                                                         Xyzz<F>* out) {
    const size_t i = (size_t)blockIdx.x * blockDim.x + threadIdx.x;
    if (i < n) st(out + i, to_std(ld(in + i)));
}

#ifndef GG_G2_SUM_WAVES
#define GG_G2_SUM_WAVES 1
#endif
template <class F>
constexpr int kSumWaves = std::is_same<F, Fp2>::value ? GG_G2_SUM_WAVES : 1;
template <class F>
__global__ void __launch_bounds__(256, kSumWaves<F>) k_bucket_sum_r(const typename PartialOf<F>::T* head,
                                                       const typename PartialOf<F>::T* tail,
                                                       const typename PartialOf<F>::T* S, const uint32_t* offsets,
                                                       uint32_t nb_total, int c, uint32_t K, int logL,
                                                       typename PartialOf<F>::T* Sr) {
    using O = PartialOps<F>;
    const uint32_t B = blockIdx.x * blockDim.x + threadIdx.x;
    if (B >= nb_total) return;
    const uint32_t nseg = nb_total >> logL;
    const BucketSpan sp = bucket_span(offsets, bucket_perm(B, c), offsets[nb_total], K);
    typename O::T acc = O::inf();
    if (!sp.empty) {
        acc = ld(sp.direct ? S + B : (sp.first ? head : tail) + sp.t0);
        const uint32_t rend = sp.direct ? sp.t0 : (sp.t1 - sp.t0 > LIGHT ? sp.t0 + 1 : sp.t1);
        for (uint32_t r = sp.t0 + 1; r <= rend; r++) acc = O::add(acc, ld(head + r));
    }
    st(Sr + (size_t)(B & ((1u << logL) - 1)) * nseg + (B >> logL), acc);
}

template <class F>
__global__ void __launch_bounds__(256) k_bucket_runsum(const typename PartialOf<F>::T* Sr, uint32_t nseg, int logL,
                                                        Xyzz<F>* Dout, Xyzz<F>* Rout) {
    using O = PartialOps<F>;
    using T = typename O::T;
    constexpr bool kPf = !std::is_same<F, Fp2>::value;
    const uint32_t t = blockIdx.x * blockDim.x + threadIdx.x;
    if (t >= nseg) return;
    const int L = 1 << logL, steps = 2 * L + logL + 1;
    T R = O::inf(), A = O::inf(), cur, nxt;
    if constexpr (kPf) nxt = ld(Sr + (size_t)(L - 1) * nseg + t);
    for (int k = 0; k < steps; k++) {
        T x, y;
        if (k < 2 * L) {
            const int i = L - 1 - (k >> 1);
            if (k & 1) {
                x = A;
                y = R;
            } else {
                if constexpr (kPf) {
                    cur = nxt;
                    if (i > 0) nxt = ld(Sr + (size_t)(i - 1) * nseg + t);
                } else {
                    cur = ld(Sr + (size_t)i * nseg + t);
                }
                x = R;
                y = cur;
            }
        } else {
            if (k == 2 * L) st(Rout + t, to_std(R));
            x = k < 2 * L + logL ? R : A;
            y = k < 2 * L + logL ? R : O::neg(R);
        }
        const T z = O::add(x, y);
        if (k < 2 * L) {
            if (k & 1) A = z;
            else R = z;
        } else if (k < 2 * L + logL) {
            R = z;
        } else {
            A = z;
        }
    }
    st(Dout + t, to_std(A));
}

constexpr int MAX_GATHER = 192;
template <class F>
struct GatherList {
    const Xyzz<F>* src[MAX_GATHER];
    uint32_t off[MAX_GATHER + 1];
    int n;
};
template <class F>
__global__ void k_gather_items(GatherList<F> L, Xyzz<F>* out) {
    uint32_t t = blockIdx.x * blockDim.x + threadIdx.x;
    int q = 0;
    while (q < L.n && t >= L.off[q + 1]) q++;
    if (q >= L.n) return;
    st(out + t, ld(L.src[q] + (t - L.off[q])));
}

template <class F>
struct RedJob {
    const Xyzz<F>* in;
    Xyzz<F>* out;
    uint32_t A, Bc, sa, sb, G, nthreads;
};
constexpr int MAX_RED_JOBS = 16;
template <class F>
struct RedJobs {
    RedJob<F> j[MAX_RED_JOBS];
    int n;
};

template <class F>
__global__ void __launch_bounds__(256) k_reduce_jobs(RedJobs<F> J) {
    const uint32_t g = blockIdx.x * blockDim.x + threadIdx.x;
    const uint32_t lane = g & 3;
    uint32_t t = g >> 2;
    int q = 0;
    while (q < J.n && t >= J.j[q].nthreads) { t -= J.j[q].nthreads; q++; }
    if (q >= J.n) return;
    const RedJob<F>& jb = J.j[q];
    uint32_t a2 = t / jb.Bc, c = t % jb.Bc;
    uint32_t a0 = a2 * jb.G;
    uint32_t a1 = min(jb.A, a0 + jb.G);
    Xyzz<F> acc = ld(jb.in + (size_t)a0 * jb.sa + (size_t)c * jb.sb);
    for (uint32_t a = a0 + 1; a < a1; a++)
        xyzz_add_quad(acc, ld(jb.in + (size_t)a * jb.sa + (size_t)c * jb.sb), lane);
    if (lane == 0) st(jb.out + (size_t)a2 * jb.Bc + c, acc);
}

template <class F>
__global__ void __launch_bounds__(256) k_reduce_block(RedJobs<F> J) {
    __shared__ Xyzz<F> sh[32];
    uint32_t t = blockIdx.x;
    int q = 0;
    while (q < J.n && t >= J.j[q].nthreads) { t -= J.j[q].nthreads; q++; }
    if (q >= J.n) return;
    const RedJob<F>& jb = J.j[q];
    const uint32_t lane = threadIdx.x & 3, quad = threadIdx.x >> 2, NQ = blockDim.x >> 2;
    Xyzz<F> acc = Xyzz<F>::inf();
    for (uint32_t a = quad; a < jb.A; a += NQ)
        xyzz_add_quad(acc, ld(jb.in + (size_t)a * jb.sa + (size_t)t * jb.sb), lane);
    for (uint32_t h = NQ >> 1; h >= 1; h >>= 1) {
        if (quad >= h && quad < 2 * h && lane == 0) sh[quad - h] = acc;
        __syncthreads();
        if (quad < h) xyzz_add_quad(acc, sh[quad], lane);
        __syncthreads();
    }
    if (threadIdx.x == 0) st(jb.out + t, acc);
}

template <class F>
__global__ void k_pre_init(const Affine<F>* in, size_t n, Affine<F>* out0, Xyzz<F>* cur) {
    size_t i = (size_t)blockIdx.x * blockDim.x + threadIdx.x;
    if (i >= n) return;
    Affine<F> p = ld(in + i);
    st(out0 + i, p);
    st(cur + i, Xyzz<F>::from_affine(p));
}

template <class F>
__global__ void __launch_bounds__(256) k_pre_dbl(Xyzz<F>* cur, size_t n, int c) {
    size_t i = (size_t)blockIdx.x * blockDim.x + threadIdx.x;
    if (i >= n) return;
    Xyzz<F> p = ld(cur + i);
    for (int k = 0; k < c; k++) p = xyzz_dbl(p);
    st(cur + i, p);
}


template <class F>
__global__ void __launch_bounds__(256) k_pre_normalize(const Xyzz<F>* cur, size_t n, size_t T,
                                                       F* prefix, Affine<F>* out) {
    size_t t = (size_t)blockIdx.x * blockDim.x + threadIdx.x;
    if (t >= T) return;
    F acc = F::one();
    for (size_t i = t; i < n; i += T) {
        st(prefix + i, acc);
        F z = ld(cur + i).zzz;
        if (!z.is_zero()) acc = acc * z;
    }
    F inv = inverse(acc);
    size_t last = t + ((n - 1 - t) / T) * T;
    for (size_t i = last;; i -= T) {
        Xyzz<F> p = ld(cur + i);
        if (p.zzz.is_zero()) {
            st(out + i, Affine<F>::inf());
        } else {
            F izzz = inv * ld(prefix + i);
            inv = inv * p.zzz;
            F izz = sqr(izzz) * sqr(p.zz);
            st(out + i, Affine<F>{p.x * izz, p.y * izzz});
        }
        if (i < T) break;
    }
}

}

using gg::DevBuf;
namespace gg {
struct MsmSort {
    DevBuf sorted, counts, offsets, maxcnt;
    DevBuf keys, tmp_entry, tmp_key, hist, hoff, bin_start, seg2, chunk_start, chunk_hist, chunk_pos,
        chunk_desc;
    std::vector<DevBuf> scan_tmp;
    int slog = 0;
    uint32_t sres = 0;
    int nvec = 1, kp = 1;
    uint32_t* pin = nullptr;
    hipEvent_t pin_ev = nullptr;
    hipEvent_t ready_ev = nullptr;
    void ensure_events() {
        if (!pin) GG_HIP(hipHostMalloc((void**)&pin, 16, hipHostMallocDefault));
        if (!pin_ev) GG_HIP(hipEventCreateWithFlags(&pin_ev, hipEventDisableTiming));
        if (!ready_ev) GG_HIP(hipEventCreateWithFlags(&ready_ev, hipEventDisableTiming));
    }
    MsmSort() = default;
    MsmSort(const MsmSort&) = delete;
    MsmSort& operator=(const MsmSort&) = delete;
    ~MsmSort() {
        if (pin) (void)hipHostFree(pin);
        if (pin_ev) (void)hipEventDestroy(pin_ev);
        if (ready_ev) (void)hipEventDestroy(ready_ev);
    }
};
struct MsmScratch {
    DevBuf head, tail, tbucket, S, arena, scal, seg;
    DevBuf headP, tailP, SP;
};
struct MsmWork {
    MsmSort sort;
    MsmScratch scr;
};
}

struct gg_msm_base {
    int group = GG_G1;
    size_t n = 0;
    int c = 0, W = 0;
    gg::WinSpec win{};
    int G = 1, Ws = 0;
    size_t nb = 0;
    DevBuf pts;
    DevBuf sidx;
    bool has_sidx = false;
    bool has_inf = false;
    int scurve = 0;
    uint32_t max_sidx = 0;
    std::mutex mu;
    gg::MsmWork own;
};

namespace gg {

template <class F>
inline void precompute(gg_msm_base* b, const Affine<F>* dev_in, hipStream_t st) {
    const size_t n = b->n;
    b->pts.alloc((size_t)b->Ws * n * sizeof(Affine<F>));
    Affine<F>* out = b->pts.as<Affine<F>>();
    DevBuf cur(n * sizeof(Xyzz<F>));
    const size_t T = std::min<size_t>(n, std::max<size_t>(16384, n / 64));
    DevBuf prefix(n * sizeof(F));
    hipLaunchKernelGGL(k_pre_init<F>, dim3(grid_for(n, 256)), dim3(256), 0, st, dev_in, n, out,
                       cur.as<Xyzz<F>>());
    GG_HIP(hipGetLastError());
    for (int w = 1; w < b->Ws; w++) {
        const int dbl = b->G == 1 ? (int)b->win.bits[w - 1] : b->G * b->c;
        hipLaunchKernelGGL(k_pre_dbl<F>, dim3(grid_for(n, 256)), dim3(256), 0, st,
                           cur.as<Xyzz<F>>(), n, dbl);
        GG_HIP(hipGetLastError());
        hipLaunchKernelGGL(k_pre_normalize<F>, dim3(grid_for(T, 256)), dim3(256), 0, st,
                           (const Xyzz<F>*)cur.p, n, T, prefix.as<F>(), out + (size_t)w * n);
        GG_HIP(hipGetLastError());
    }
    if constexpr (RadixOf<F>::on) {
        using C = typename RadixOf<F>::C;
        using E = Fe<typename C::Std>;
        const size_t total = (size_t)b->Ws * n * 2 * (sizeof(F) / sizeof(E));
        hipLaunchKernelGGL(k_to_radix<C>, dim3(grid_for(total, 256)), dim3(256), 0, st, (E*)out, total);
        GG_HIP(hipGetLastError());
    }
    GG_WAIT_STREAM(st);
}

template <class F>
struct RedItem {
    const Xyzz<F>* X;
    uint32_t n, off;
    int mlog;
    bool plain;
    int mult = 1;
    int res = 0;
};

template <class F>
inline std::vector<Xyzz<F>> reduce_terms_multi(std::vector<RedItem<F>> items, int nres, MsmScratch* scr,
                                               hipStream_t st) {
    static const bool split = getenv("GG_RED_SPLIT") && atoi(getenv("GG_RED_SPLIT"));
    if (split && items.size() > 1) {
        std::vector<Xyzz<F>> acc(nres, Xyzz<F>::inf());
        for (const auto& it : items)
            acc[it.res] = xyzz_add(acc[it.res], reduce_terms_multi<F>({it}, nres, scr, st)[it.res]);
        return acc;
    }
    const size_t XB = sizeof(Xyzz<F>);
    size_t total = 0;
    for (const auto& it : items) total += it.n;
    const size_t arena_elems = 3 * total + 1024 * (items.size() + 1);
    scr->arena.reserve(arena_elems * XB);
    Xyzz<F>* arena = scr->arena.as<Xyzz<F>>();
    size_t used = 0;
    auto alloc = [&](size_t cnt) {
        GG_CHECK(used + cnt <= arena_elems, GG_ERR_INTERNAL, "bucket reduction arena overflow");
        Xyzz<F>* p = arena + used;
        used += cnt;
        return p;
    };
    using Item = RedItem<F>;
    struct Job { const Xyzz<F>* in; uint32_t A, Bc, sa, sb; Item dest; };
    std::vector<Item> host_items;
    uint32_t HOST_N = 8;
    if (const char* e = getenv("GG_RED_HOST_N")) HOST_N = (uint32_t)std::max(2, atoi(e));
    while (!items.empty()) {
        std::vector<Job> jobs;
        for (const Item& it : items) {
            if (it.n <= HOST_N) { host_items.push_back(it); continue; }
            int lg = 31 - __builtin_clz(it.n);
            int mlg = lg / 2;
            uint32_t M = 1u << mlg, rows = it.n >> mlg;
            if (it.plain) {
                jobs.push_back({it.X, M, rows, 1u, M, Item{nullptr, rows, 0u, it.mlog, true, it.mult, it.res}});
                continue;
            }
            jobs.push_back({it.X, M, rows, 1u, M, Item{nullptr, rows, 0u, it.mlog + mlg, false, it.mult, it.res}});
            jobs.push_back({it.X, rows, M, M, 1u, Item{nullptr, M, it.off, it.mlog, false, it.mult, it.res}});
        }
        static const bool block_mode = !(getenv("GG_RED_BLOCK") && atoi(getenv("GG_RED_BLOCK")) == 0);
        if (block_mode && !jobs.empty()) {
            RedJobs<F> J;
            J.n = 0;
            size_t blocks = 0;
            uint32_t maxA = 1;
            auto flush = [&]() {
                if (!J.n) return;
                uint32_t nq = 1;
                while (nq < maxA && nq < 64) nq <<= 1;
                hipLaunchKernelGGL(k_reduce_block<F>, dim3((unsigned)blocks), dim3(4 * nq), 0, st, J);
                GG_HIP(hipGetLastError());
                J.n = 0;
                blocks = 0;
                maxA = 1;
            };
            for (auto& j : jobs) {
                Xyzz<F>* out = alloc(j.Bc);
                J.j[J.n++] = RedJob<F>{j.in, out, j.A, j.Bc, j.sa, j.sb, j.A, j.Bc};
                blocks += j.Bc;
                maxA = std::max(maxA, j.A);
                j.in = out;
                j.A = 1;
                j.sa = j.Bc;
                j.sb = 1;
                if (J.n == MAX_RED_JOBS) flush();
            }
            flush();
        }
        bool active = false;
        for (auto& j : jobs) if (j.A > 1) active = true;
        while (active) {
            size_t t2 = 0;
            for (auto& j : jobs) if (j.A > 1) t2 += (size_t)((j.A + 1) / 2) * j.Bc;
            uint32_t G = t2 >= (256u << 10) ? 8 : (t2 >= (96u << 10) ? 4 : 2);
            RedJobs<F> J;
            J.n = 0;
            size_t threads = 0;
            auto flush = [&]() {
                if (!J.n) return;
                hipLaunchKernelGGL(k_reduce_jobs<F>, dim3(grid_for(4 * threads, 256)), dim3(256), 0, st, J);
                GG_HIP(hipGetLastError());
                J.n = 0;
                threads = 0;
            };
            active = false;
            for (auto& j : jobs) {
                if (j.A <= 1) continue;
                uint32_t A2 = (j.A + G - 1) / G;
                Xyzz<F>* out = alloc((size_t)A2 * j.Bc);
                J.j[J.n++] = RedJob<F>{j.in, out, j.A, j.Bc, j.sa, j.sb, G, A2 * j.Bc};
                threads += (size_t)A2 * j.Bc;
                j.in = out;
                j.A = A2;
                j.sa = j.Bc;
                j.sb = 1;
                if (A2 > 1) active = true;
                if (J.n == MAX_RED_JOBS) flush();
            }
            flush();
        }
        std::vector<Item> next;
        for (auto& j : jobs) { Item it = j.dest; it.X = j.in; next.push_back(it); }
        items.swap(next);
    }
    GG_CHECK(host_items.size() <= (size_t)MAX_GATHER, GG_ERR_INTERNAL, "too many host reduction items");
    GatherList<F> GL;
    GL.n = (int)host_items.size();
    GL.off[0] = 0;
    for (size_t k = 0; k < host_items.size(); k++) {
        GL.src[k] = host_items[k].X;
        GL.off[k + 1] = GL.off[k] + host_items[k].n;
    }
    std::vector<Xyzz<F>> flat(GL.off[GL.n]);
    if (GL.n) {
        Xyzz<F>* stage = alloc(GL.off[GL.n]);
        hipLaunchKernelGGL(k_gather_items<F>, dim3(grid_for(GL.off[GL.n], 256)), dim3(256), 0, st, GL, stage);
        GG_HIP(hipGetLastError());
        GG_HIP(hipMemcpyAsync(flat.data(), stage, flat.size() * XB, hipMemcpyDeviceToHost, st));
    }
    GG_WAIT_STREAM(st);
    std::vector<std::vector<Xyzz<F>>> hx(host_items.size());
    for (size_t k = 0; k < host_items.size(); k++)
        hx[k].assign(flat.begin() + GL.off[k], flat.begin() + GL.off[k + 1]);
    std::vector<std::vector<std::pair<int, Xyzz<F>>>> vals(nres);
    auto scaled = [](const Xyzz<F>& v, int m) {
        if (m == 1 || v.is_inf()) return v;
        const uint32_t u = (uint32_t)(m < 0 ? -m : m);
        Xyzz<F> r = Xyzz<F>::inf();
        for (int bit = 31; bit >= 0; bit--) {
            if (!r.is_inf()) r = xyzz_dbl(r);
            if ((u >> bit) & 1u) r = xyzz_add(r, v);
        }
        if (m < 0 && !r.is_inf()) r.y = -r.y;
        return r;
    };
    auto finish = [&](int r) {
        auto& vr = vals[r];
        for (size_t k = 0; k < host_items.size(); k++) {
            if (host_items[k].res != r) continue;
            const auto& X = hx[k];
            Xyzz<F> run = Xyzz<F>::inf(), acc = Xyzz<F>::inf();
            if (host_items[k].plain) {
                for (const auto& x : X) acc = xyzz_add(acc, x);
                vr.push_back({host_items[k].mlog, scaled(acc, host_items[k].mult)});
                continue;
            }
            for (size_t j = X.size(); j-- > 1;) {
                run = xyzz_add(run, X[j]);
                acc = xyzz_add(acc, run);
            }
            if (host_items[k].off) {
                run = xyzz_add(run, X[0]);
                for (uint32_t o = 0; o < host_items[k].off; o++) acc = xyzz_add(acc, run);
            }
            vr.push_back({host_items[k].mlog, scaled(acc, host_items[k].mult)});
        }
        std::sort(vr.begin(), vr.end(), [](const auto& x, const auto& y) { return x.first > y.first; });
        Xyzz<F> acc = Xyzz<F>::inf();
        int cur = vr.empty() ? 0 : vr[0].first;
        for (auto& v : vr) {
            for (; cur > v.first; cur--) acc = acc.is_inf() ? acc : xyzz_dbl(acc);
            acc = xyzz_add(acc, v.second);
        }
        for (; cur > 0; cur--) acc = acc.is_inf() ? acc : xyzz_dbl(acc);
        return acc;
    };
    std::vector<Xyzz<F>> out(nres, Xyzz<F>::inf());
    for (int r = 0; r < nres; r++) out[r] = finish(r);
    return out;
}
template <class F>
inline Xyzz<F> reduce_terms(std::vector<RedItem<F>> items, MsmScratch* scr, hipStream_t st) {
    return reduce_terms_multi<F>(std::move(items), 1, scr, st)[0];
}

template <class F>
constexpr bool kSegsumGroup = RadixOf<F>::on && (std::is_same<F, Fp>::value || std::is_same<F, FpBls>::value ||
                                                   std::is_same<F, Fp2>::value);
inline bool segsum_enabled() {
    const char* e = getenv("GG_MSM_SEGSUM");
    return !(e && atoi(e) == 0);
}
inline bool combine_fused() {
    const char* e = getenv("GG_MSM_COMBINE_FUSED");
    return !(e && atoi(e) == 0);
}


template <class F>
inline uint32_t range_length(size_t E) {
    if (const char* e = getenv("GG_MSM_K1")) return (uint32_t)std::max(1, atoi(e));
    static const double C = [] {
        int blocks = 0, cus = 0, dev = 0;
        if (hipGetDevice(&dev) != hipSuccess ||
            hipDeviceGetAttribute(&cus, hipDeviceAttributeMultiprocessorCount, dev) != hipSuccess ||
            hipOccupancyMaxActiveBlocksPerMultiprocessor(&blocks, k_accum_range<F, false>, 256, kAccumLds<F>) != hipSuccess ||
            blocks < 1 || cus < 1) {
            (void)hipGetLastError();
            return 256.0 * 256 * 2;
        }
        return (double)blocks * cus * 256;
    }();
    const double kpref = E < ((size_t)4 << 20) ? 32 : (E >= ((size_t)1 << 26) ? 128 : 64);
    const double rounds = std::max(1.0, std::round((double)E / (C * kpref)));
    return (uint32_t)std::max(1.0, std::ceil((double)E / (rounds * C)));
}

template <class F>
inline void msm_finish_multi(gg_msm_base* b, MsmSort* s, MsmScratch* scr, hipStream_t st, Xyzz<F>* out) {
    const int slog = s->slog, nvec = s->nvec, kp = s->kp;
    const size_t n = b->n, nb = (b->nb >> slog) * (size_t)kp;
    const int ce = b->c - slog;
    const int Gb = b->G, Ge = b->G * kp;
    for (int v = 0; v < nvec; v++) out[v] = Xyzz<F>::inf();
    if (n == 0) return;
    GG_HIP(hipStreamWaitEvent(st, s->ready_ev, 0));
    const uint32_t* offs = s->offsets.as<uint32_t>();
    size_t E = (size_t)b->W * n * (size_t)nvec;
    if (slog) {
        GG_WAIT_EVENT(s->pin_ev);
        E = std::max<size_t>(s->pin[1], 1);
    }
    uint32_t K = range_length<F>(E);
    if constexpr (kLdsGather<F>)
        if ((std::is_same<F, Fp2>::value ? GG_RING_CHUNKS_G2 : GG_RING_CHUNKS) != 0) K = (K + 3u) & ~3u;
    const size_t T = (E + K - 1) / K;
    using PT = typename PartialOf<F>::T;
    constexpr bool kRadixP = !std::is_same<PT, Xyzz<F>>::value;
    scr->head.reserve((T + 1) * sizeof(Xyzz<F>));
    scr->tail.reserve((T + 1) * sizeof(Xyzz<F>));
    scr->tbucket.reserve((T + 1) * 4);
    scr->S.reserve(nb * sizeof(Xyzz<F>));
    Xyzz<F>* head = scr->head.as<Xyzz<F>>();
    Xyzz<F>* S = scr->S.as<Xyzz<F>>();
    PT *hP = (PT*)head, *tP = scr->tail.as<PT>(), *SP = (PT*)S;
    if constexpr (kRadixP) {
        scr->headP.reserve((T + 1) * sizeof(PT));
        scr->tailP.reserve((T + 1) * sizeof(PT));
        scr->SP.reserve(nb * sizeof(PT));
        hP = scr->headP.as<PT>();
        tP = scr->tailP.as<PT>();
        SP = scr->SP.as<PT>();
    }
    {
        const char* acc_name = sizeof(F) == sizeof(Fp) ? "msm_accum" : (sizeof(F) == sizeof(Fp2) ? "msm_accum_g2" : "msm_accum_bls");
        ProfScope ps_acc(acc_name, st, (double)n);
        uint32_t pmask = 0x7fffffffu;
        if (kAccumProbe) {
            pmask = 1023u;
            while (pmask && pmask >= n) pmask >>= 1;
        }
        static const double nt_min = [] {
            const char* e = getenv("GG_ACCUM_NT_GB");
            return 1e9 * (e ? atof(e) : 4.0);
        }();
        const bool nt = !kLdsGather<F> && (GG_PT_NT == 2 || (GG_PT_NT == 1 && std::is_same<F, Fp>::value &&
                                                              (double)b->pts.bytes >= nt_min));
        auto* const accum = nt ? &k_accum_range<F, true> : &k_accum_range<F, false>;
        hipLaunchKernelGGL(accum, dim3(grid_for(T, 256)), dim3(256), kAccumLds<F>, st,
                           (const Affine<F>*)b->pts.p,
                           s->sorted.as<uint32_t>(), offs, (uint32_t)nb, ce, K, (int)b->has_inf, hP, tP, SP,
                           scr->tbucket.as<uint32_t>(), pmask);
        GG_HIP(hipGetLastError());
        ps_acc.stop(st);
    }
    GG_WAIT_EVENT(s->pin_ev);
    const uint32_t maxcnt = s->pin[0];
    const uint32_t max_ranges = maxcnt / K + 1;
    ProfScope ps_acc2("msm_accum2", st, (double)n);
    const size_t nbg = nb / (size_t)Ge;
    static const int seg_minlog = [] {
        const char* e = getenv("GG_MSM_SEGSUM_MINLOG");
        return e ? std::max(8, std::min(18, atoi(e))) : 17;
    }();
    static const int segs_log = [] {
        const char* e = getenv("GG_MSM_SEGS_LOG");
        return e ? std::max(12, std::min(20, atoi(e))) : 17;
    }();
    const int lgb = 31 - __builtin_clz((unsigned)std::max<size_t>(nbg, 1));
    const int logL = lgb >= segs_log + 1 ? std::min(4, lgb - segs_log) : (lgb >= seg_minlog ? 1 : 0);
    if constexpr (kSegsumGroup<F>) {
        if (segsum_enabled() && logL >= 1) {
            for (uint32_t stride = 1; max_ranges > LIGHT && stride < max_ranges;) {
                const uint32_t fan = (stride == 1) ? 4u : 2u;
                hipLaunchKernelGGL(k_range_tree_r<F>, dim3(grid_for(T, 256)), dim3(256), 0, st, hP,
                                   (const uint32_t*)scr->tbucket.p, offs, (uint32_t)nb, K, stride, fan);
                GG_HIP(hipGetLastError());
                stride *= fan;
            }
            const uint32_t Tg = (uint32_t)(nbg >> logL), G = (uint32_t)Ge;
            scr->seg.reserve(2 * (size_t)G * Tg * sizeof(Xyzz<F>) + nb * sizeof(PT));
            Xyzz<F>* D = scr->seg.as<Xyzz<F>>();
            Xyzz<F>* Rs = D + (size_t)G * Tg;
            PT* Sr = reinterpret_cast<PT*>(Rs + (size_t)G * Tg);
            hipLaunchKernelGGL(k_bucket_sum_r<F>, dim3(grid_for(nb, 256)), dim3(256), 0, st, (const PT*)hP,
                               (const PT*)tP, (const PT*)SP, offs, (uint32_t)nb, ce, K, logL, Sr);
            GG_HIP(hipGetLastError());
            hipLaunchKernelGGL(k_bucket_runsum<F>, dim3(grid_for((size_t)G * Tg, 256)), dim3(256), 0, st,
                               (const PT*)Sr, (uint32_t)(G * Tg), logL, D, Rs);
            GG_HIP(hipGetLastError());
            ps_acc2.stop(st);
            ProfScope ps_red("msm_reduce", st, (double)nb);
            const int sneg = slog ? -(int)((1u << slog) - 1u - s->sres) : 0;
            std::vector<RedItem<F>> terms;
            for (int jg = 0; jg < nvec * Gb; jg++) {
                const int j = jg % Gb, v = jg / Gb;
                terms.push_back({(const Xyzz<F>*)Rs + (size_t)jg * Tg, Tg, 1u, j * b->c + logL + slog, false, 1, v});
                terms.push_back({(const Xyzz<F>*)D + (size_t)jg * Tg, Tg, 0u, j * b->c + slog, true, 1, v});
                if (sneg) terms.push_back({(const Xyzz<F>*)Rs + (size_t)jg * Tg, Tg, 0u, j * b->c, true, sneg, v});
            }
            const std::vector<Xyzz<F>> res = reduce_terms_multi<F>(std::move(terms), nvec, scr, st);
            for (int v = 0; v < nvec; v++) out[v] = res[v];
            ps_red.stop(st);
            return;
        }
    }
    bool combined = false;
    if constexpr (kRadixP) {
        if (combine_fused()) {
            for (uint32_t stride = 1; max_ranges > LIGHT && stride < max_ranges;) {
                const uint32_t fan = (stride == 1) ? 4u : 2u;
                hipLaunchKernelGGL(k_range_tree_r<F>, dim3(grid_for(T, 256)), dim3(256), 0, st, hP,
                                   (const uint32_t*)scr->tbucket.p, offs, (uint32_t)nb, K, stride, fan);
                GG_HIP(hipGetLastError());
                stride *= fan;
            }
            hipLaunchKernelGGL(k_bucket_combine_r<F>, dim3(grid_for(4 * nb, 256)), dim3(256), 0, st, (const PT*)hP,
                               (const PT*)tP, (const PT*)SP, offs, (uint32_t)nb, ce, K, S);
            GG_HIP(hipGetLastError());
            combined = true;
        } else {
            hipLaunchKernelGGL(k_partials_to_std<F>, dim3(grid_for(T + 1, 256)), dim3(256), 0, st, (const PT*)hP,
                               T + 1, head);
            hipLaunchKernelGGL(k_partials_to_std<F>, dim3(grid_for(T + 1, 256)), dim3(256), 0, st, (const PT*)tP,
                               T + 1, scr->tail.as<Xyzz<F>>());
            hipLaunchKernelGGL(k_partials_to_std<F>, dim3(grid_for(nb, 256)), dim3(256), 0, st, (const PT*)SP, nb, S);
            GG_HIP(hipGetLastError());
        }
    }
    if (!combined) {
        for (uint32_t stride = 1; max_ranges > LIGHT && stride < max_ranges;) {
            const uint32_t fan = (stride == 1) ? 4u : 2u;
            hipLaunchKernelGGL(k_range_tree<F>, dim3(grid_for(4 * T, 256)), dim3(256), 0, st, head,
                               (const uint32_t*)scr->tbucket.p, offs, (uint32_t)nb, K, stride, fan);
            GG_HIP(hipGetLastError());
            stride *= fan;
        }
        hipLaunchKernelGGL(k_bucket_combine<F>, dim3(grid_for(4 * nb, 256)), dim3(256), 0, st, (const Xyzz<F>*)head,
                           (const Xyzz<F>*)scr->tail.p, offs, (uint32_t)nb, ce, K, S);
        GG_HIP(hipGetLastError());
    }
    ps_acc2.stop(st);
    ProfScope ps_red("msm_reduce", st, (double)nb);
    const int sneg = slog ? -(int)((1u << slog) - 1u - s->sres) : 0;
    std::vector<RedItem<F>> terms;
    for (int jg = 0; jg < nvec * Gb; jg++) {
        const int j = jg % Gb, v = jg / Gb;
        const Xyzz<F>* Sj = (const Xyzz<F>*)S + (size_t)jg * nbg;
        terms.push_back({Sj, (uint32_t)nbg, 1u, j * b->c + slog, false, 1, v});
        if (sneg) terms.push_back({Sj, (uint32_t)nbg, 0u, j * b->c, true, sneg, v});
    }
    const std::vector<Xyzz<F>> res = reduce_terms_multi<F>(std::move(terms), nvec, scr, st);
    for (int v = 0; v < nvec; v++) out[v] = res[v];
    ps_red.stop(st);
}

template <class F>
inline Xyzz<F> msm_finish(gg_msm_base* b, MsmSort* s, MsmScratch* scr, hipStream_t st) {
    GG_CHECK(s->nvec == 1, GG_ERR_INTERNAL, "msm_finish of a batch sort");
    Xyzz<F> r;
    msm_finish_multi<F>(b, s, scr, st, &r);
    return r;
}

template <class F>
inline Xyzz<F> msm_run(gg_msm_base* b, MsmWork* w, const Fr* scalars_dev, hipStream_t st) {
    if (b->n == 0) return Xyzz<F>::inf();
    msm_prepare(b, &w->sort, scalars_dev, st);
    return msm_finish<F>(b, &w->sort, &w->scr, st);
}

template <class F>
inline void msm_run_batch(gg_msm_base* b, MsmWork* w, const VecPtrs& vp, int nvec, hipStream_t st, Xyzz<F>* out) {
    if (b->n == 0) {
        for (int v = 0; v < nvec; v++) out[v] = Xyzz<F>::inf();
        return;
    }
    msm_prepare_batch(b, &w->sort, vp, nvec, st);
    msm_finish_multi<F>(b, &w->sort, &w->scr, st, out);
}

template <class F>
__global__ void k_base_keep(const Affine<F>* pts, size_t n, int keep_inf, uint32_t* keep, uint32_t* any_inf) {
    const size_t i = (size_t)blockIdx.x * blockDim.x + threadIdx.x;
    if (i >= n) return;
    const bool inf = pts[i].is_inf();
    if (inf) *any_inf = 1u;
    keep[i] = (!inf || keep_inf) ? 1u : 0u;
}
template <class F>
__global__ void k_base_compact(const Affine<F>* pts, size_t n, const uint32_t* keep, const uint32_t* pos,
                               Affine<F>* out, uint32_t* idx) {
    const size_t i = (size_t)blockIdx.x * blockDim.x + threadIdx.x;
    if (i >= n || !keep[i]) return;
    out[pos[i]] = pts[i];
    idx[pos[i]] = (uint32_t)i;
}

template <class F>
inline void window_layout(gg_msm_base* b, int window_bits, int total, int groups) {
    const size_t pb = sizeof(Affine<F>);
    b->c = window_bits ? window_bits : choose_c(std::max<size_t>(b->n, 1), pb, total);
    GG_CHECK(b->c >= 2 && b->c <= 24, GG_ERR_INVALID_ARG, "window_bits out of range [2, 24]");
    b->W = (total + b->c - 1) / b->c;
    b->c = (total + b->W - 1) / b->W;
    GG_CHECK(b->W <= 64, GG_ERR_INVALID_ARG, "too many windows");
    if (groups == 0) groups = choose_groups((double)b->W * (double)b->n * (double)pb, 0.0, b->W);
    GG_CHECK(groups >= 1 && groups <= 16 && (groups & (groups - 1)) == 0, GG_ERR_INVALID_ARG,
             "precompute groups must be 1, 2, 4, 8 or 16");
    b->G = std::min(groups, 1 << (31 - __builtin_clz((unsigned)b->W)));
    b->Ws = (b->W + b->G - 1) / b->G;
    if (b->G == 1) {
        b->win = make_windows(b->c, b->W, total);
    } else {
        for (int w = 0; w < b->W; w++) {
            b->win.bits[w] = (uint8_t)b->c;
            b->win.off[w] = (uint8_t)(w * b->c);
        }
    }
    b->nb = (size_t)b->G << (b->c - 1);
    GG_CHECK(b->nb < ((size_t)1 << 30), GG_ERR_UNSUPPORTED, "too many buckets");
    GG_CHECK((double)b->W * (double)b->n < 2147483648.0, GG_ERR_UNSUPPORTED,
             "too many points x windows for 31-bit entry ids");
}

template <class F>
inline void create_base_dev(gg_msm_base* b, const Affine<F>* pts, size_t n, int window_bits, bool keep_inf,
                            int total, int groups) {
    hipStream_t st = hipStreamPerThread;
    DevBuf keep(std::max<size_t>(n, 1) * 4), pos(std::max<size_t>(n, 1) * 4), flag(16);
    GG_HIP(hipMemsetAsync(flag.p, 0, 4, st));
    hipLaunchKernelGGL(k_base_keep<F>, dim3(grid_for(n, 256)), dim3(256), 0, st, pts, n, (int)keep_inf,
                       keep.as<uint32_t>(), flag.as<uint32_t>());
    GG_HIP(hipGetLastError());
    std::vector<DevBuf> tmp;
    exclusive_scan(keep.as<uint32_t>(), pos.as<uint32_t>(), n, st, tmp);
    uint32_t last_pos = 0, last_keep = 0, any_inf = 0;
    GG_HIP(hipMemcpyAsync(&last_pos, pos.as<uint32_t>() + (n - 1), 4, hipMemcpyDeviceToHost, st));
    GG_HIP(hipMemcpyAsync(&last_keep, keep.as<uint32_t>() + (n - 1), 4, hipMemcpyDeviceToHost, st));
    GG_HIP(hipMemcpyAsync(&any_inf, flag.p, 4, hipMemcpyDeviceToHost, st));
    GG_WAIT_STREAM(st);
    const size_t kept = (size_t)last_pos + last_keep;
    b->n = kept;
    b->has_inf = keep_inf && any_inf;
    const bool dropped = kept < n;
    b->has_sidx = dropped;
    window_layout<F>(b, window_bits, total, groups);
    if (!kept) {
        b->max_sidx = 0;
        if (dropped) b->sidx.alloc(4);
        return;
    }
    DevBuf cmp(kept * sizeof(Affine<F>)), idx(kept * 4);
    hipLaunchKernelGGL(k_base_compact<F>, dim3(grid_for(n, 256)), dim3(256), 0, st, pts, n, keep.as<uint32_t>(),
                       pos.as<uint32_t>(), cmp.as<Affine<F>>(), idx.as<uint32_t>());
    GG_HIP(hipGetLastError());
    uint32_t max_idx = 0;
    GG_HIP(hipMemcpyAsync(&max_idx, idx.as<uint32_t>() + (kept - 1), 4, hipMemcpyDeviceToHost, st));
    GG_WAIT_STREAM(st);
    b->max_sidx = max_idx;
    if (dropped) b->sidx = std::move(idx);
    precompute<F>(b, cmp.as<Affine<F>>(), st);
}

template <class F>
inline void create_base(gg_msm_base* b, const void* points, size_t n, int on_device,
                        const uint32_t* sidx, int window_bits, bool keep_inf = false,
                        int scurve = 0, int groups = 0) {
    b->scurve = scurve;
    const int total = scalar_total_bits(scurve);
    const size_t pb = sizeof(Affine<F>);
    if (on_device && !sidx && n) {
        create_base_dev<F>(b, (const Affine<F>*)points, n, window_bits, keep_inf, total, groups);
        return;
    }
    std::vector<uint8_t> host;
    const uint8_t* src;
    if (on_device) {
        host.resize(n * pb);
        if (n) GG_HIP(hipMemcpy(host.data(), points, n * pb, hipMemcpyDeviceToHost));
        src = host.data();
    } else {
        src = (const uint8_t*)points;
    }
    std::vector<uint8_t> keep;
    keep.reserve(n * pb);
    std::vector<uint32_t> idx;
    idx.reserve(n);
    bool dropped = false;
    static const uint8_t zero[128] = {0};
    for (size_t i = 0; i < n; i++) {
        const uint8_t* p = src + i * pb;
        if (memcmp(p, zero, pb) == 0) {
            if (keep_inf) b->has_inf = true;
            else { dropped = true; continue; }
        }
        keep.insert(keep.end(), p, p + pb);
        idx.push_back(sidx ? sidx[i] : (uint32_t)i);
    }
    b->n = idx.size();
    b->has_sidx = dropped || sidx != nullptr;
    b->max_sidx = 0;
    for (uint32_t v : idx) b->max_sidx = std::max(b->max_sidx, v);
    window_layout<F>(b, window_bits, total, groups);
    if (b->has_sidx) {
        b->sidx.alloc(std::max<size_t>(b->n, 1) * 4);
        if (b->n) GG_HIP(hipMemcpy(b->sidx.p, idx.data(), b->n * 4, hipMemcpyHostToDevice));
    }
    if (b->n == 0) return;
    DevBuf tmp(b->n * pb);
    GG_HIP(hipMemcpy(tmp.p, keep.data(), b->n * pb, hipMemcpyHostToDevice));
    precompute<F>(b, tmp.as<Affine<F>>(), hipStreamPerThread);
}

}
```

gnark-fork_amd/csrc/ntt.hip:

```cpp
#include "common.h"
#include "field.cuh"
#include "prof.h"
#include <vector>
#include <mutex>
#include <memory>
#include <algorithm>
#include <cstring>
#include <type_traits>

namespace gg {

enum ScaleKind {
    SK_G_NAT = 0,
    SK_G_BR = 1,
    SK_GINV_NAT_N = 2,
    SK_GINV_BR_N = 3,
    SK_NINV = 4,
    SK_H_FWD = 5,
    SK_H_INV = 6,
    SK_DEN_N = 7,
    SK_COUNT = 8
};

template <class F>
struct ScaleSpec {
    const F* hi;
    const F* lo;
    int shift;
    int bitrev;
};

template <class F>
struct PassParams {
    const F* in;
    F* out;
    const F* tw;
    int log_n;
    int b_lo;
    int k;
    int tl;
    int dit;
    int has_pre;
    ScaleSpec<F> pre;
    int has_post;
    ScaleSpec<F> post;
    int epi_mul_sub;
    int epi_mul;
    int epi_sub;
    const F* ea;
    const F* eb;
    int canon_out;
};

template <class F>
struct NttLazy {
    static constexpr bool on = false;
};
template <>
struct NttLazy<Fr> {
    static constexpr bool on = true;
};
template <class C>
GG_HD constexpr uint32_t twop_limb(int i) {
    uint64_t c = 0;
    uint32_t v = 0;
    for (int j = 0; j <= i; j++) {
        const uint64_t t = (uint64_t)C::P[j] * 2 + c;
        v = (uint32_t)t;
        c = t >> 32;
    }
    return v;
}
template <class C>
__device__ __forceinline__ Fe<C> red2p(const Fe<C>& x) {
    Fe<C> s, r;
    uint32_t br = 0;
#pragma unroll
    for (int i = 0; i < 8; i++) s.v[i] = __builtin_subc(x.v[i], twop_limb<C>(i), br, &br);
#pragma unroll
    for (int i = 0; i < 8; i++) r.v[i] = br ? x.v[i] : s.v[i];
    return r;
}
template <class C>
__device__ __forceinline__ Fe<C> add2p(const Fe<C>& a, const Fe<C>& b) {
    Fe<C> r;
    uint32_t c = 0;
#pragma unroll
    for (int i = 0; i < 8; i++) r.v[i] = __builtin_addc(a.v[i], b.v[i], c, &c);
    return red2p(r);
}
template <class C>
__device__ __forceinline__ Fe<C> subnr2p(const Fe<C>& a, const Fe<C>& b) {
    Fe<C> r;
    uint32_t br = 0, c = 0;
#pragma unroll
    for (int i = 0; i < 8; i++) r.v[i] = __builtin_subc(a.v[i], b.v[i], br, &br);
#pragma unroll
    for (int i = 0; i < 8; i++) r.v[i] = __builtin_addc(r.v[i], twop_limb<C>(i), c, &c);
    return r;
}
template <class C>
__device__ __forceinline__ Fe<C> sub2p(const Fe<C>& a, const Fe<C>& b) {
    Fe<C> r, s;
    uint32_t br = 0, c = 0;
#pragma unroll
    for (int i = 0; i < 8; i++) r.v[i] = __builtin_subc(a.v[i], b.v[i], br, &br);
#pragma unroll
    for (int i = 0; i < 8; i++) s.v[i] = __builtin_addc(r.v[i], twop_limb<C>(i), c, &c);
#pragma unroll
    for (int i = 0; i < 8; i++) r.v[i] = br ? s.v[i] : r.v[i];
    return r;
}
template <class C>
__device__ __forceinline__ Fe<C> canon(const Fe<C>& x) {
    Fe<C> s, r;
    uint32_t br = 0;
#pragma unroll
    for (int i = 0; i < 8; i++) s.v[i] = __builtin_subc(x.v[i], C::P[i], br, &br);
#pragma unroll
    for (int i = 0; i < 8; i++) r.v[i] = br ? x.v[i] : s.v[i];
    return r;
}

__device__ __forceinline__ uint32_t brev_bits(uint32_t i, int L) {
    return L ? (__brev(i) >> (32 - L)) : 0u;
}

template <class F>
__device__ __forceinline__ F apply_scale(const ScaleSpec<F>& s, uint32_t g, int L, const F& x) {
    uint32_t e = s.bitrev ? brev_bits(g, L) : g;
    F f = ld_fr(s.hi + (e >> s.shift));
    if (s.lo) f = f * ld_fr(s.lo + (e & ((1u << s.shift) - 1)));
    return x * f;
}

__device__ __forceinline__ int lidx(int e) { return e + (e >> 5); }

template <class F, int NB, bool DIT>
__device__ __forceinline__ void ntt_round(const PassParams<F>& P, uint32_t* lds, int TP, int T, int qlo,
                                          bool first, bool last, uint32_t base_hi, uint32_t lo0) {
    constexpr int R = 1 << NB;
    const int tl = P.tl;
    const uint32_t tl_mask = (1u << tl) - 1;
    const int pos = qlo + tl;
    const uint32_t lowmask = (1u << pos) - 1;
    const int groups = T >> NB;
    for (int gi = threadIdx.x; gi < groups; gi += blockDim.x) {
        uint32_t e[R], g[R];
        F x[R];
        const uint32_t low = (uint32_t)gi & lowmask, high = ((uint32_t)gi >> pos) << (pos + NB);
#pragma unroll
        for (int m = 0; m < R; m++) {
            e[m] = high | ((uint32_t)m << pos) | low;
            g[m] = base_hi | ((e[m] >> tl) << P.b_lo) | (lo0 + (e[m] & tl_mask));
        }
        if (first) {
#pragma unroll
            for (int m = 0; m < R; m++) {
                x[m] = ld_fr(P.in + g[m]);
                if (P.has_pre) x[m] = apply_scale(P.pre, g[m], P.log_n, x[m]);
            }
        } else {
#pragma unroll
            for (int m = 0; m < R; m++) {
#pragma unroll
                for (int l = 0; l < 8; l++) x[m].v[l] = lds[l * TP + lidx((int)e[m])];
            }
        }
#pragma unroll
        for (int s2 = 0; s2 < NB; s2++) {
            const int r = DIT ? s2 : (NB - 1 - s2);
            const int b = P.b_lo + qlo + r;
            const uint32_t bmask = (1u << b) - 1;
            const F* twb = P.tw + bmask;
#pragma unroll
            for (int m = 0; m < R; m++) {
                if (m & (1 << r)) continue;
                const int m2 = m | (1 << r);
                const uint32_t i = g[m] & bmask;
                if constexpr (NttLazy<F>::on) {
                    if (DIT) {
                        F t = i ? mul_nored(x[m2], ld_fr(twb + i)) : x[m2];
                        x[m2] = sub2p(x[m], t);
                        x[m] = add2p(x[m], t);
                    } else {
                        F d = subnr2p(x[m], x[m2]);
                        x[m] = add2p(x[m], x[m2]);
                        x[m2] = i ? mul_nored(d, ld_fr(twb + i)) : red2p(d);
                    }
                    continue;
                }
                if (DIT) {
                    F t = i ? x[m2] * ld_fr(twb + i) : x[m2];
                    x[m2] = x[m] - t;
                    x[m] = x[m] + t;
                } else {
                    F d = x[m] - x[m2];
                    x[m] = x[m] + x[m2];
                    x[m2] = i ? d * ld_fr(twb + i) : d;
                }
            }
        }
        if (last) {
#pragma unroll
            for (int m = 0; m < R; m++) {
                F y = x[m];
                if (NttLazy<F>::on && P.canon_out && !P.has_post) y = canon(y);
                if (P.has_post) y = apply_scale(P.post, g[m], P.log_n, y);
                if (P.epi_mul_sub) y = ld_fr(P.ea + g[m]) * ld_fr(P.eb + g[m]) - y;
                if (P.epi_mul) y = ld_fr(P.ea + g[m]) * y;
                if (P.epi_sub) y = y - ld_fr(P.ea + g[m]);
                st_fr(P.out + g[m], y);
            }
        } else {
#pragma unroll
            for (int m = 0; m < R; m++) {
#pragma unroll
                for (int l = 0; l < 8; l++) lds[l * TP + lidx((int)e[m])] = x[m].v[l];
            }
        }
    }
}

template <int MAXNB>
constexpr int kNttThreads = MAXNB == 3 ? 256 : (MAXNB == 2 ? 512 : 1024);
template <int MAXNB>
constexpr int kNttWaves = MAXNB == 3 ? 1 : (MAXNB == 2 ? 4 : 8);
template <class F, bool DIT, int MAXNB>
__global__ void __launch_bounds__(kNttThreads<MAXNB>, kNttWaves<MAXNB>) k_ntt_pass(PassParams<F> P) {
    extern __shared__ __attribute__((aligned(16))) uint32_t lds[];
    const int k = P.k, tl = P.tl;
    const int T = 1 << (k + tl);
    const int TP = T + (T >> 5);
    const int nlo_log = P.b_lo - tl;
    const uint32_t tile = blockIdx.x;
    const uint32_t lob = tile & ((1u << nlo_log) - 1);
    const uint32_t hi = tile >> nlo_log;
    const uint32_t base_hi = hi << (P.b_lo + k);
    const uint32_t lo0 = lob << tl;
    if (k == 0) {
        for (int e = threadIdx.x; e < T; e += blockDim.x) {
            uint32_t g = base_hi | (lo0 + (uint32_t)e);
            F x = ld_fr(P.in + g);
            if (P.has_pre) x = apply_scale(P.pre, g, P.log_n, x);
            if (P.has_post) x = apply_scale(P.post, g, P.log_n, x);
            if (P.epi_mul_sub) x = ld_fr(P.ea + g) * ld_fr(P.eb + g) - x;
            if (P.epi_mul) x = ld_fr(P.ea + g) * x;
            if (P.epi_sub) x = x - ld_fr(P.ea + g);
            st_fr(P.out + g, x);
        }
        return;
    }
    int done = 0;
    bool first = true;
    while (done < k) {
        const int nb = min(MAXNB, k - done);
        const int qlo = DIT ? done : (k - done - nb);
        const bool last = (done + nb == k);
        if (!first) __syncthreads();
        if constexpr (MAXNB >= 3) {
            if (nb == 3) {
                ntt_round<F, 3, DIT>(P, lds, TP, T, qlo, first, last, base_hi, lo0);
                first = false;
                done += nb;
                continue;
            }
        }
        if constexpr (MAXNB >= 2) {
            if (nb == 2) {
                ntt_round<F, 2, DIT>(P, lds, TP, T, qlo, first, last, base_hi, lo0);
                first = false;
                done += nb;
                continue;
            }
        }
        ntt_round<F, 1, DIT>(P, lds, TP, T, qlo, first, last, base_hi, lo0);
        first = false;
        done += nb;
    }
}

template <class F>
__global__ void k_stage_twiddles(F* out, size_t count, int L, const F* hi, const F* lo, int S) {
    size_t t = (size_t)blockIdx.x * blockDim.x + threadIdx.x;
    if (t >= count) return;
    uint32_t v = (uint32_t)t + 1;
    int b = 31 - __clz((int)v);
    uint32_t i = v - (1u << b);
    uint32_t ex = i << (L - 1 - b);
    F x = ld_fr(hi + (ex >> S)) * ld_fr(lo + (ex & ((1u << S) - 1)));
    st_fr(out + t, x);
}


struct Pass {
    int b_lo, k, tl;
};

static std::vector<Pass> plan_passes(int L, bool dit) {
    std::vector<Pass> up;
    if (L <= 11) {
        up.push_back({0, L, 0});
    } else {
        up.push_back({0, 11, 0});
        int rem = L - 11, P = (rem + 8) / 9, b = 11;
        for (int i = 0; i < P; i++) {
            int k = rem / (P - i);
            up.push_back({b, k, 11 - k});
            b += k;
            rem -= k;
        }
    }
    if (dit) return up;
    std::vector<Pass> v(up.rbegin(), up.rend());
    return v;
}

}

using namespace gg;

namespace gg {
template <class C>
struct DomainT {
    using F = Fe<C>;
    int log_n = 0;
    size_t n = 1;
    F omega, omega_inv, g, g_inv, n_inv, den;
    DevBuf tw, twinv;
    int S = 0;
    DevBuf scale_hi[SK_COUNT], scale_lo[SK_COUNT];
    ScaleSpec<F> spec[SK_COUNT];
};
}

struct gg_domain {
    int curve = GG_CURVE_BN254;
    int log_n = 0;
    size_t n = 1;
    std::unique_ptr<DomainT<FrCfg>> bn;
    std::unique_ptr<DomainT<FrBlsCfg>> bls;
    DevBuf scratch;
    std::mutex mu;
};

namespace gg {

template <class F>
static void build_pow_tables(int L, int S, const F& x, const F& c, std::vector<F>& hi,
                             std::vector<F>& lo) {
    size_t nlo = (size_t)1 << S, nhi = (size_t)1 << (L - S);
    lo.resize(nlo);
    hi.resize(nhi);
    F acc = F::one();
    for (size_t i = 0; i < nlo; i++) { lo[i] = acc; acc = acc * x; }
    F step = acc;
    acc = c;
    for (size_t i = 0; i < nhi; i++) { hi[i] = acc; acc = acc * step; }
}

template <class F>
static void upload(DevBuf& b, const std::vector<F>& v) {
    b.alloc(v.size() * sizeof(F));
    GG_HIP(hipMemcpy(b.p, v.data(), v.size() * sizeof(F), hipMemcpyHostToDevice));
}

static int ntt_radix() {
    const char* e = getenv("GG_NTT_RADIX");
    const int r = e ? atoi(e) : 4;
    return (r == 2 || r == 8) ? r : 4;
}

static hipStream_t pick_stream(void* s) { return s ? (hipStream_t)s : hipStreamPerThread; }

enum { EPI_MUL_SUB = 0, EPI_MUL = 1, EPI_SUB = 2 };
template <class C>
void run_transform(DomainT<C>* d, const Fe<C>* in, Fe<C>* out, bool dit, bool inverse_tw, int pre_kind,
                   int post_kind, const Fe<C>* ea, const Fe<C>* eb, hipStream_t st, int epi = EPI_MUL_SUB,
                   const std::vector<Pass>* only = nullptr) {
    using F = Fe<C>;
    const int L = d->log_n;
    auto passes = only ? *only : plan_passes(L, dit);
    const F* src = in;
    for (size_t pi = 0; pi < passes.size(); pi++) {
        const Pass& ps = passes[pi];
        PassParams<F> P{};
        P.in = src;
        P.out = out;
        P.tw = (const F*)(inverse_tw ? d->twinv.p : d->tw.p);
        P.log_n = L;
        P.b_lo = ps.b_lo;
        P.k = ps.k;
        P.tl = ps.tl;
        P.dit = dit ? 1 : 0;
        if (pi == 0 && pre_kind >= 0) { P.has_pre = 1; P.pre = d->spec[pre_kind]; }
        bool last = (pi + 1 == passes.size());
        if (last && post_kind >= 0) { P.has_post = 1; P.post = d->spec[post_kind]; }
        if (last && ea) {
            P.epi_mul_sub = epi == EPI_MUL_SUB;
            P.epi_mul = epi == EPI_MUL;
            P.epi_sub = epi == EPI_SUB;
            P.ea = ea;
            P.eb = eb;
        }
        P.canon_out = last ? 1 : 0;
        int T = 1 << (ps.k + ps.tl);
        unsigned tiles = (unsigned)(d->n / (size_t)T);
        size_t lds = (ps.k > 3) ? (size_t)(T + (T >> 5)) * 32 : 0;
        ProfScope prof("ntt_pass", st, (double)d->n);
        static const int radix = ntt_radix();
        if (radix == 4) {
            lds = (ps.k > 2) ? (size_t)(T + (T >> 5)) * 32 : 0;
            if (dit) hipLaunchKernelGGL((k_ntt_pass<F, true, 2>), dim3(tiles), dim3(512), lds, st, P);
            else hipLaunchKernelGGL((k_ntt_pass<F, false, 2>), dim3(tiles), dim3(512), lds, st, P);
        } else if (radix == 2) {
            lds = (ps.k > 1) ? (size_t)(T + (T >> 5)) * 32 : 0;
            if (dit) hipLaunchKernelGGL((k_ntt_pass<F, true, 1>), dim3(tiles), dim3(1024), lds, st, P);
            else hipLaunchKernelGGL((k_ntt_pass<F, false, 1>), dim3(tiles), dim3(1024), lds, st, P);
        } else {
            if (dit) hipLaunchKernelGGL((k_ntt_pass<F, true, 3>), dim3(tiles), dim3(256), lds, st, P);
            else hipLaunchKernelGGL((k_ntt_pass<F, false, 3>), dim3(tiles), dim3(256), lds, st, P);
        }
        GG_HIP(hipGetLastError());
        prof.stop(st);
        src = out;
    }
}

}

namespace gg {
template <class C>
static DomainT<C>* domain_build(int log_n, const void* omega_mont, const void* coset_gen_mont) {
    using F = Fe<C>;
    std::unique_ptr<DomainT<C>> d(new DomainT<C>());
    d->log_n = log_n;
    d->n = (size_t)1 << log_n;
    memcpy(d->omega.v, omega_mont, 32);
    memcpy(d->g.v, coset_gen_mont, 32);
    F x = d->omega;
    for (int i = 0; i < log_n; i++) {
        if (i == log_n - 1) GG_CHECK(!(x == F::one()), GG_ERR_INVALID_ARG, "omega order < n");
        x = sqr(x);
    }
    GG_CHECK(x == F::one(), GG_ERR_INVALID_ARG, "omega^n != 1");
    GG_CHECK(!d->g.is_zero(), GG_ERR_INVALID_ARG, "coset generator is zero");
    d->omega_inv = inverse(d->omega);
    d->g_inv = inverse(d->g);
    F nn = F::zero();
    nn.v[0] = (uint32_t)d->n;
    nn.v[1] = (uint32_t)((uint64_t)d->n >> 32);
    nn = to_mont(nn);
    d->n_inv = inverse(nn);
    F gn = pow_u64(d->g, d->n);
    F t = gn - F::one();
    GG_CHECK(!t.is_zero(), GG_ERR_INVALID_ARG, "g^n == 1: coset generator in the domain");
    d->den = inverse(t);

    const int L = log_n;
    d->S = (L + 1) / 2;
    const int S = d->S;
    std::vector<F> hi, lo;
    struct KindDef { F x, c; int br; };
    KindDef defs[SK_COUNT] = {
        {d->g, F::one(), 0},
        {d->g, F::one(), 1},
        {d->g_inv, d->n_inv, 0},
        {d->g_inv, d->n_inv, 1},
        {F::one(), d->n_inv, 0},
        {d->g, d->n_inv, 1},
        {d->g_inv, d->den * d->n_inv, 1},
        {F::one(), d->den * d->n_inv, 0},
    };
    for (int kd = 0; kd < SK_COUNT; kd++) {
        build_pow_tables(L, S, defs[kd].x, defs[kd].c, hi, lo);
        upload(d->scale_hi[kd], hi);
        upload(d->scale_lo[kd], lo);
        d->spec[kd] = ScaleSpec<F>{(const F*)d->scale_hi[kd].p, (const F*)d->scale_lo[kd].p, S,
                                   defs[kd].br};
    }
    size_t cnt = d->n - 1;
    d->tw.alloc((cnt + 1) * 32);
    d->twinv.alloc((cnt + 1) * 32);
    if (cnt) {
        for (int inv = 0; inv < 2; inv++) {
            DevBuf h1, l1;
            build_pow_tables(L, S, inv ? d->omega_inv : d->omega, F::one(), hi, lo);
            upload(h1, hi);
            upload(l1, lo);
            hipLaunchKernelGGL(k_stage_twiddles<F>, dim3(grid_for(cnt, 256)), dim3(256), 0, 0,
                               (inv ? d->twinv : d->tw).template as<F>(), cnt, L, h1.as<F>(), l1.as<F>(), S);
            GG_HIP(hipGetLastError());
            GG_HIP(hipDeviceSynchronize());
        }
    }
    return d.release();
}

template <class C>
static void ntt_apply(DomainT<C>* d, void* data_dev, int inverse, bool dit, int coset, hipStream_t st) {
    Fe<C>* a = (Fe<C>*)data_dev;
    int pre = -1, post = -1;
    if (!inverse) {
        if (coset) pre = dit ? SK_G_BR : SK_G_NAT;
    } else {
        if (!coset) post = SK_NINV;
        else post = dit ? SK_GINV_NAT_N : SK_GINV_BR_N;
    }
    run_transform(d, a, a, dit, inverse != 0, pre, post, (const Fe<C>*)nullptr, (const Fe<C>*)nullptr, st);
}
}

extern "C" int gg_domain_create_ex(int curve, int log_n, const void* omega_mont,
                                   const void* coset_gen_mont, gg_domain_t* out) {
    GG_CAPI_BEGIN
    GG_CHECK(out && omega_mont && coset_gen_mont, GG_ERR_INVALID_ARG, "null argument");
    GG_CHECK(curve == GG_CURVE_BN254 || curve == GG_CURVE_BLS12_381, GG_ERR_INVALID_ARG, "bad curve");
    GG_CHECK(log_n >= 0 && log_n <= (curve == GG_CURVE_BN254 ? 28 : 30), GG_ERR_INVALID_ARG,
             "log_n out of range");
    std::unique_ptr<gg_domain> d(new gg_domain());
    d->curve = curve;
    d->log_n = log_n;
    d->n = (size_t)1 << log_n;
    if (curve == GG_CURVE_BN254) d->bn.reset(domain_build<FrCfg>(log_n, omega_mont, coset_gen_mont));
    else d->bls.reset(domain_build<FrBlsCfg>(log_n, omega_mont, coset_gen_mont));
    *out = d.release();
    GG_CAPI_END
}

extern "C" int gg_domain_create(int log_n, const void* omega_mont, const void* coset_gen_mont,
                                gg_domain_t* out) {
    return gg_domain_create_ex(GG_CURVE_BN254, log_n, omega_mont, coset_gen_mont, out);
}

extern "C" int gg_domain_release(gg_domain_t d) {
    GG_CAPI_BEGIN
    delete d;
    GG_CAPI_END
}

extern "C" int gg_domain_log_n(gg_domain_t d, int* log_n) {
    GG_CAPI_BEGIN
    GG_CHECK(d && log_n, GG_ERR_INVALID_ARG, "null argument");
    *log_n = d->log_n;
    GG_CAPI_END
}

extern "C" int gg_ntt(gg_domain_t d, void* data_dev, int inverse, int decimation, int coset,
                      void* hip_stream) {
    GG_CAPI_BEGIN
    GG_CHECK(d && data_dev, GG_ERR_INVALID_ARG, "null argument");
    GG_CHECK(decimation == GG_DIF || decimation == GG_DIT, GG_ERR_INVALID_ARG, "bad decimation");
    hipStream_t st = pick_stream(hip_stream);
    bool dit = decimation == GG_DIT;
    if (d->curve == GG_CURVE_BN254) ntt_apply(d->bn.get(), data_dev, inverse, dit, coset, st);
    else ntt_apply(d->bls.get(), data_dev, inverse, dit, coset, st);
    GG_CAPI_END
}

namespace gg {
template <class C>
static void compute_h_t(DomainT<C>* d, Fe<C>* A, Fe<C>* B, Fe<C>* Cv, Fe<C>* H, hipStream_t st) {
    const Fe<C>* nul = nullptr;
    run_transform(d, A, A, false, true, -1, SK_H_FWD, nul, nul, st);
    run_transform(d, A, A, true, false, -1, -1, nul, nul, st);
    run_transform(d, B, B, false, true, -1, SK_H_FWD, nul, nul, st);
    run_transform(d, B, B, true, false, -1, -1, (const Fe<C>*)A, nul, st, EPI_MUL);
    run_transform(d, Cv, Cv, false, true, -1, SK_DEN_N, nul, nul, st);
    GG_CHECK(H != Cv, GG_ERR_INTERNAL, "computeH: h must not alias c");
    run_transform(d, B, H, false, true, -1, SK_H_INV, (const Fe<C>*)Cv, nul, st, EPI_SUB);
}
void compute_h_device(gg_domain* dom, Fr* A, Fr* B, Fr* C, Fr* H, hipStream_t st) {
    if (dom->curve == GG_CURVE_BN254) compute_h_t(dom->bn.get(), A, B, C, H, st);
    else compute_h_t(dom->bls.get(), (FrBls*)A, (FrBls*)B, (FrBls*)C, (FrBls*)H, st);
}
}

extern "C" int gg_groth16_compute_h(gg_domain_t d, const void* a, const void* b, const void* c,
                                    size_t len, int inputs_on_device, void* h_dev,
                                    void* hip_stream) {
    GG_CAPI_BEGIN
    GG_CHECK(d && a && b && c && h_dev, GG_ERR_INVALID_ARG, "null argument");
    GG_CHECK(len <= d->n, GG_ERR_INVALID_ARG, "len > domain cardinality");
    std::lock_guard<std::mutex> lk(d->mu);
    hipStream_t st = pick_stream(hip_stream);
    size_t nb = d->n * 32;
    d->scratch.reserve(3 * nb);
    char* base = (char*)d->scratch.p;
    Fr* A = (Fr*)base;
    Fr* B = (Fr*)(base + nb);
    Fr* C = (Fr*)(base + 2 * nb);
    hipMemcpyKind kind = inputs_on_device ? hipMemcpyDeviceToDevice : hipMemcpyHostToDevice;
    const void* src[3] = {a, b, c};
    Fr* dst[3] = {A, B, C};
    for (int i = 0; i < 3; i++) {
        if (len) GG_HIP(hipMemcpyAsync(dst[i], src[i], len * 32, kind, st));
        if (len < d->n) GG_HIP(hipMemsetAsync((char*)dst[i] + len * 32, 0, nb - len * 32, st));
    }
    compute_h_device(d, A, B, C, (Fr*)h_dev, st);
    GG_WAIT_STREAM(st);
    GG_CAPI_END
}

namespace gg {
size_t domain_size(gg_domain* d, int* curve) {
    if (curve) *curve = d->curve;
    return d->n;
}
void any_ntt_inplace(gg_domain* d, void* data, int inverse, int dit, int coset, hipStream_t st) {
    if (d->curve == GG_CURVE_BN254) ntt_apply(d->bn.get(), data, inverse, dit != 0, coset, st);
    else ntt_apply(d->bls.get(), data, inverse, dit != 0, coset, st);
}
void ntt_inverse_dit_noscale(gg_domain* d, void* data, hipStream_t st) {
    if (d->curve == GG_CURVE_BN254)
        run_transform(d->bn.get(), (const Fr*)data, (Fr*)data, true, true, -1, -1, (const Fr*)nullptr,
                      (const Fr*)nullptr, st);
    else
        run_transform(d->bls.get(), (const FrBls*)data, (FrBls*)data, true, true, -1, -1, (const FrBls*)nullptr,
                      (const FrBls*)nullptr, st);
}
void ntt_tail_inverse_coset(gg_domain* d, void* data, int u, hipStream_t st) {
    const int L = d->log_n;
    GG_CHECK(u >= 1 && u <= 4 && L >= 12, GG_ERR_INTERNAL, "tail transform: 1..4 stages of a >= 2^12 domain");
    const std::vector<Pass> tail = {{L - u, u, 11 - u}};
    if (d->curve == GG_CURVE_BN254)
        run_transform(d->bn.get(), (const Fr*)data, (Fr*)data, true, true, -1, SK_GINV_NAT_N, (const Fr*)nullptr,
                      (const Fr*)nullptr, st, EPI_MUL_SUB, &tail);
    else
        run_transform(d->bls.get(), (const FrBls*)data, (FrBls*)data, true, true, -1, SK_GINV_NAT_N,
                      (const FrBls*)nullptr, (const FrBls*)nullptr, st, EPI_MUL_SUB, &tail);
}
template <class C>
static void xn_minus_one_inv_t(const DomainT<C>* d, size_t n_small, void* out) {
    using F = Fe<C>;
    const size_t rho = d->n / n_small;
    std::vector<F> res(rho);
    res[0] = pow_u64(d->g, n_small);
    const F t = pow_u64(d->omega, n_small);
    for (size_t i = 1; i < rho; i++) res[i] = res[i - 1] * t;
    for (size_t i = 0; i < rho; i++) {
        res[i] = res[i] - F::one();
        GG_CHECK(!res[i].is_zero(), GG_ERR_INVALID_ARG, "x^n - 1 vanishes on the big coset");
        res[i] = inverse(res[i]);
    }
    memcpy(out, res.data(), rho * sizeof(F));
}
void xn_minus_one_inv(gg_domain* big, size_t n_small, void* out) {
    if (big->curve == GG_CURVE_BN254) xn_minus_one_inv_t(big->bn.get(), n_small, out);
    else xn_minus_one_inv_t(big->bls.get(), n_small, out);
}
}




namespace gg {
template <class C>
struct HShardT {
    using F = Fe<C>;
    std::unique_ptr<DomainT<C>> loc;
    F invN, invN_den;
    DevBuf w_hi, w_lo, wi_hi, wi_lo, g_hi, g_lo, gi_hi, gi_lo;
    int S = 0;
    F wN[16], wNi[16];
    F gm[16], gmi[16];
    DevBuf y, full;
    DevBuf hblk;
    DevBuf ccoef;
};
}

struct gg_hshard {
    int curve = GG_CURVE_BN254;
    int log_n = 0, rank = 0, world = 1, log_w = 0, M = 0;
    size_t n = 0, m = 0, chunk = 0;
    std::unique_ptr<gg::HShardT<gg::FrCfg>> bn;
    std::unique_ptr<gg::HShardT<gg::FrBlsCfg>> bls;
    int last_phase = 0;
    hipStream_t st = nullptr;
    std::mutex mu;
    ~gg_hshard() {
        if (st) (void)hipStreamDestroy(st);
    }
};

namespace gg {
template <class F>
struct PowTab {
    const F *hi, *lo;
    int S;
    __device__ __forceinline__ F at(uint32_t e) const {
        return ld_fr(hi + (e >> S)) * ld_fr(lo + (e & ((1u << S) - 1)));
    }
};

template <class F, int N>
struct SmallRoots {
    F fwd[N], inv[N], cs[N];
};

template <class F, int N>
__device__ __forceinline__ void dft_small(F (&x)[N], const F (&r)[N]) {
    constexpr int LG = N <= 1 ? 0 : (N == 2 ? 1 : (N == 4 ? 2 : (N == 8 ? 3 : 4)));
#pragma unroll
    for (int i = 0; i < N; i++) {
        int j = 0;
#pragma unroll
        for (int b = 0; b < LG; b++) j |= ((i >> b) & 1) << (LG - 1 - b);
        if (i < j) {
            F t = x[i];
            x[i] = x[j];
            x[j] = t;
        }
    }
#pragma unroll
    for (int len = 2; len <= N; len <<= 1)
#pragma unroll
        for (int i = 0; i < N; i += len)
#pragma unroll
            for (int j = 0; j < len / 2; j++) {
                const F u = x[i + j];
                F v = x[i + j + len / 2];
                if (j) v = v * r[(N / len) * j];
                x[i + j] = u + v;
                x[i + j + len / 2] = u - v;
            }
}

template <class F>
__global__ void k_gather_cyclic(F* y, const F* x, size_t len, size_t m, int rank, int N) {
    size_t j = (size_t)blockIdx.x * blockDim.x + threadIdx.x;
    if (j >= m) return;
    size_t i = (size_t)rank + (size_t)N * j;
    F v = i < len ? ld_fr(x + i) : F::zero();
    st_fr(y + j, v);
}

template <class F>
__global__ void k_twist_scatter(F* send, const F* y, size_t m, size_t chunk, int M, int npoly, int poly,
                                uint32_t rank, PowTab<F> tw) {
    size_t p = (size_t)blockIdx.x * blockDim.x + threadIdx.x;
    if (p >= m) return;
    uint32_t c1 = brev_bits((uint32_t)p, M);
    F v = ld_fr(y + p);
    if (rank) v = v * tw.at(rank * c1);
    size_t r = p / chunk, q = p - r * chunk;
    st_fr(send + (r * npoly + poly) * chunk + q, v);
}

template <class F, int N>
__global__ void __launch_bounds__(256) k_cross_fwd(F* send, const F* recv, size_t chunk, int M, uint32_t rank,
                                                   SmallRoots<F, N> R, PowTab<F> gpow, PowTab<F> wpow, F* ccoef,
                                                   F cden) {
    size_t t = (size_t)blockIdx.x * blockDim.x + threadIdx.x;
    if (t >= chunk * 3) return;
    const int poly = (int)(t / chunk);
    const size_t q = t - (size_t)poly * chunk;
    const uint32_t c1 = brev_bits((uint32_t)(rank * chunk + q), M);
    F x[N];
#pragma unroll
    for (int k = 0; k < N; k++) x[k] = ld_fr(recv + ((size_t)k * 3 + poly) * chunk + q);
    dft_small<F, N>(x, R.inv);
    if (poly == 2) {
#pragma unroll
        for (int c2 = 0; c2 < N; c2++) st_fr(ccoef + (size_t)c2 * chunk + q, x[c2] * cden);
        return;
    }
#pragma unroll
    for (int c2 = 0; c2 < N; c2++) x[c2] = x[c2] * R.cs[c2];
    dft_small<F, N>(x, R.fwd);
    const F wc = wpow.at(c1);
    F f = gpow.at(c1);
#pragma unroll
    for (int k2 = 0; k2 < N; k2++) {
        if (k2) f = f * wc;
        st_fr(send + ((size_t)k2 * 2 + poly) * chunk + q, x[k2] * f);
    }
}

template <class F>
__global__ void k_unpack(F* y, const F* recv, size_t m, size_t chunk, int npoly, int poly) {
    size_t p = (size_t)blockIdx.x * blockDim.x + threadIdx.x;
    if (p >= m) return;
    size_t r = p / chunk, q = p - r * chunk;
    st_fr(y + p, ld_fr(recv + (r * npoly + poly) * chunk + q));
}

template <class F, int N>
__global__ void __launch_bounds__(256) k_cross_inv_out(F* h, const F* recv, size_t chunk, int M, int logN,
                                                       uint32_t rank, SmallRoots<F, N> R, PowTab<F> gipow,
                                                       const F* ccoef) {
    size_t q = (size_t)blockIdx.x * blockDim.x + threadIdx.x;
    if (q >= chunk) return;
    const uint32_t c1 = brev_bits((uint32_t)(rank * chunk + q), M);
    F x[N];
#pragma unroll
    for (int k = 0; k < N; k++) x[k] = ld_fr(recv + (size_t)k * chunk + q);
    dft_small<F, N>(x, R.inv);
    const F gi = gipow.at(c1);
#pragma unroll
    for (int c2 = 0; c2 < N; c2++)
        st_fr(h + (size_t)N * q + brev_bits((uint32_t)c2, logN),
                 x[c2] * R.cs[c2] * gi - ld_fr(ccoef + (size_t)c2 * chunk + q));
}

template <class F>
static void pow_tab_upload(int L, int S, const F& x, DevBuf& hi, DevBuf& lo) {
    std::vector<F> h, l;
    build_pow_tables(L, S, x, F::one(), h, l);
    upload(hi, h);
    upload(lo, l);
}

template <class C>
static HShardT<C>* hs_impl(gg_hshard* hs) {
    if constexpr (std::is_same<C, FrCfg>::value) return hs->bn.get();
    else return hs->bls.get();
}

template <class C, int N>
static void launch_cross_fwd(gg_hshard* hs, Fe<C>* send, const Fe<C>* recv, hipStream_t st) {
    using F = Fe<C>;
    HShardT<C>* t = hs_impl<C>(hs);
    SmallRoots<F, N> R;
    for (int i = 0; i < N; i++) {
        R.fwd[i] = t->wN[i];
        R.inv[i] = t->wNi[i];
        R.cs[i] = t->invN * t->gm[i];
    }
    PowTab<F> gp{t->g_hi.template as<F>(), t->g_lo.template as<F>(), t->S};
    PowTab<F> wp{t->w_hi.template as<F>(), t->w_lo.template as<F>(), t->S};
    hipLaunchKernelGGL((k_cross_fwd<F, N>), dim3(grid_for(hs->chunk * 3, 256)), dim3(256), 0, st, send, recv,
                       hs->chunk, hs->M, (uint32_t)hs->rank, R, gp, wp, t->ccoef.template as<F>(), t->invN_den);
    GG_HIP(hipGetLastError());
}

template <class C, int N>
static void launch_cross_inv(gg_hshard* hs, Fe<C>* h, const Fe<C>* recv, hipStream_t st) {
    using F = Fe<C>;
    HShardT<C>* t = hs_impl<C>(hs);
    SmallRoots<F, N> R;
    for (int i = 0; i < N; i++) {
        R.fwd[i] = t->wN[i];
        R.inv[i] = t->wNi[i];
        R.cs[i] = t->invN_den * t->gmi[i];
    }
    PowTab<F> gi{t->gi_hi.template as<F>(), t->gi_lo.template as<F>(), t->S};
    hipLaunchKernelGGL((k_cross_inv_out<F, N>), dim3(grid_for(hs->chunk, 256)), dim3(256), 0, st, h, recv,
                       hs->chunk, hs->M, hs->log_w, (uint32_t)hs->rank, R, gi,
                       (const F*)t->ccoef.template as<F>());
    GG_HIP(hipGetLastError());
}

template <class C>
static void phase1_t(gg_hshard* hs, const Fe<C>* a, const Fe<C>* b, const Fe<C>* c, size_t len, Fe<C>* send,
                     hipStream_t st, bool compact) {
    using F = Fe<C>;
    HShardT<C>* t = hs_impl<C>(hs);
    const size_t m = hs->m;
    F* y = t->y.template as<F>();
    PowTab<F> twi{t->wi_hi.template as<F>(), t->wi_lo.template as<F>(), t->S};
    const F* src[3] = {a, b, c};
    for (int p = 0; p < 3; p++) {
        F* yp = y + (size_t)p * m;
        hipLaunchKernelGGL(k_gather_cyclic<F>, dim3(grid_for(m, 256)), dim3(256), 0, st, yp, src[p], len, m,
                           compact ? 0 : hs->rank, compact ? 1 : hs->world);
        GG_HIP(hipGetLastError());
        run_transform(t->loc.get(), yp, yp, false, true, -1, SK_NINV, (const F*)nullptr, (const F*)nullptr, st);
        hipLaunchKernelGGL(k_twist_scatter<F>, dim3(grid_for(m, 256)), dim3(256), 0, st, send, yp, m, hs->chunk,
                           hs->M, 3, p, (uint32_t)hs->rank, twi);
        GG_HIP(hipGetLastError());
    }
}

template <class C>
static void phase2_t(gg_hshard* hs, const Fe<C>* recv, Fe<C>* send, hipStream_t st) {
    switch (hs->world) {
        case 1: launch_cross_fwd<C, 1>(hs, send, recv, st); break;
        case 2: launch_cross_fwd<C, 2>(hs, send, recv, st); break;
        case 4: launch_cross_fwd<C, 4>(hs, send, recv, st); break;
        case 8: launch_cross_fwd<C, 8>(hs, send, recv, st); break;
        case 16: launch_cross_fwd<C, 16>(hs, send, recv, st); break;
        default: throw Error(GG_ERR_UNSUPPORTED, "distributed computeH: world must be 1, 2, 4, 8 or 16");
    }
}

template <class C>
static void phase3_t(gg_hshard* hs, const Fe<C>* recv, Fe<C>* send, hipStream_t st) {
    using F = Fe<C>;
    HShardT<C>* t = hs_impl<C>(hs);
    const size_t m = hs->m;
    F* y = t->y.template as<F>();
    const F* nul = nullptr;
    for (int p = 0; p < 2; p++) {
        hipLaunchKernelGGL(k_unpack<F>, dim3(grid_for(m, 256)), dim3(256), 0, st, y + (size_t)p * m, recv, m,
                           hs->chunk, 2, p);
        GG_HIP(hipGetLastError());
    }
    run_transform(t->loc.get(), y, y, true, false, -1, -1, nul, nul, st);
    run_transform(t->loc.get(), y + m, y + m, true, false, -1, -1, y, nul, st, EPI_MUL);
    run_transform(t->loc.get(), y + m, y + m, false, true, -1, SK_NINV, nul, nul, st);
    PowTab<F> twi{t->wi_hi.template as<F>(), t->wi_lo.template as<F>(), t->S};
    hipLaunchKernelGGL(k_twist_scatter<F>, dim3(grid_for(m, 256)), dim3(256), 0, st, send, y + m, m, hs->chunk,
                       hs->M, 1, 0, (uint32_t)hs->rank, twi);
    GG_HIP(hipGetLastError());
}

template <class C>
static void phase4_t(gg_hshard* hs, const Fe<C>* recv, Fe<C>* h, hipStream_t st) {
    switch (hs->world) {
        case 1: launch_cross_inv<C, 1>(hs, h, recv, st); break;
        case 2: launch_cross_inv<C, 2>(hs, h, recv, st); break;
        case 4: launch_cross_inv<C, 4>(hs, h, recv, st); break;
        case 8: launch_cross_inv<C, 8>(hs, h, recv, st); break;
        case 16: launch_cross_inv<C, 16>(hs, h, recv, st); break;
        default: throw Error(GG_ERR_UNSUPPORTED, "distributed computeH: world must be 1, 2, 4, 8 or 16");
    }
}

static void phase_order(gg_hshard* hs, int phase) {
    GG_CHECK(phase == 1 || hs->last_phase == phase - 1, GG_ERR_INVALID_ARG,
             "distributed computeH: phase " + std::to_string(phase) + " after phase " +
                 std::to_string(hs->last_phase) +
                 " on this handle (phases run 1, 2, 3, 4 in order, one proof at a time per handle)");
}
struct PhaseStep {
    gg_hshard* hs;
    int phase;
    bool ok = false;
    PhaseStep(gg_hshard* h, int p) : hs(h), phase(p) { phase_order(h, p); }
    ~PhaseStep() { hs->last_phase = ok && phase != 4 ? phase : 0; }
};
void hshard_phase1(gg_hshard* hs, const Fr* a, const Fr* b, const Fr* c, size_t len, Fr* send, hipStream_t st,
                   bool compact = false) {
    PhaseStep step(hs, 1);
    if (hs->curve == GG_CURVE_BN254) phase1_t<FrCfg>(hs, a, b, c, len, send, st, compact);
    else phase1_t<FrBlsCfg>(hs, (const FrBls*)a, (const FrBls*)b, (const FrBls*)c, len, (FrBls*)send, st, compact);
    step.ok = true;
}
void hshard_phase2(gg_hshard* hs, const Fr* recv, Fr* send, hipStream_t st) {
    PhaseStep step(hs, 2);
    if (hs->curve == GG_CURVE_BN254) phase2_t<FrCfg>(hs, recv, send, st);
    else phase2_t<FrBlsCfg>(hs, (const FrBls*)recv, (FrBls*)send, st);
    step.ok = true;
}
void hshard_phase3(gg_hshard* hs, const Fr* recv, Fr* send, hipStream_t st) {
    PhaseStep step(hs, 3);
    if (hs->curve == GG_CURVE_BN254) phase3_t<FrCfg>(hs, recv, send, st);
    else phase3_t<FrBlsCfg>(hs, (const FrBls*)recv, (FrBls*)send, st);
    step.ok = true;
}
void hshard_phase4(gg_hshard* hs, const Fr* recv, Fr* h, hipStream_t st) {
    PhaseStep step(hs, 4);
    if (hs->curve == GG_CURVE_BN254) phase4_t<FrCfg>(hs, recv, h, st);
    else phase4_t<FrBlsCfg>(hs, (const FrBls*)recv, (FrBls*)h, st);
    step.ok = true;
}

size_t hshard_m(const gg_hshard* hs, int* rank, int* world, int* log_n) {
    *rank = hs->rank;
    *world = hs->world;
    *log_n = hs->log_n;
    return hs->m;
}
int hshard_curve(const gg_hshard* hs) { return hs->curve; }
Fr* hshard_h(gg_hshard* hs) {
    return hs->curve == GG_CURVE_BN254 ? hs->bn->hblk.as<Fr>() : hs->bls->hblk.as<Fr>();
}

size_t hshard_exchange_bytes(const gg_hshard* hs, int phase) {
    return hs->chunk * 32 * (size_t)(phase == 1 ? 3 : phase == 2 ? 2 : 1);
}

template <class C>
static void hshard_build(gg_hshard* hs, HShardT<C>* t, const void* omega_mont, const void* coset_gen_mont) {
    using F = Fe<C>;
    F w, g;
    memcpy(w.v, omega_mont, 32);
    memcpy(g.v, coset_gen_mont, 32);
    F wm = pow_u64(w, (uint64_t)hs->world);
    t->loc.reset(domain_build<C>(hs->M, wm.v, g.v));
    GG_CHECK(!(pow_u64(w, hs->n / 2) == F::one()), GG_ERR_INVALID_ARG, "omega order < n");
    GG_CHECK(pow_u64(w, hs->n) == F::one(), GG_ERR_INVALID_ARG, "omega^n != 1");
    F wNroot = pow_u64(w, hs->m);
    F wNinv = inverse(wNroot);
    F a = F::one(), b = F::one();
    for (int i = 0; i < 16; i++) {
        t->wN[i] = a;
        t->wNi[i] = b;
        a = a * wNroot;
        b = b * wNinv;
    }
    F nn = F::zero();
    nn.v[0] = (uint32_t)hs->world;
    t->invN = inverse(to_mont(nn));
    F gn = pow_u64(g, hs->n) - F::one();
    GG_CHECK(!gn.is_zero(), GG_ERR_INVALID_ARG, "g^n == 1: coset generator in the domain");
    t->invN_den = t->invN * inverse(gn);
    {
        const F gmr = pow_u64(g, hs->m), gmr_i = inverse(gmr);
        F x = F::one(), y = F::one();
        for (int i = 0; i < 16; i++) {
            t->gm[i] = x;
            t->gmi[i] = y;
            x = x * gmr;
            y = y * gmr_i;
        }
    }
    t->S = (hs->log_n + 1) / 2;
    pow_tab_upload(hs->log_n, t->S, w, t->w_hi, t->w_lo);
    pow_tab_upload(hs->log_n, t->S, inverse(w), t->wi_hi, t->wi_lo);
    pow_tab_upload(hs->log_n, t->S, g, t->g_hi, t->g_lo);
    pow_tab_upload(hs->log_n, t->S, inverse(g), t->gi_hi, t->gi_lo);
    t->y.alloc(3 * hs->m * 32);
    t->hblk.alloc(hs->m * 32);
    t->ccoef.alloc(hs->m * 32);
}

gg_hshard* hshard_create(int curve, int log_n, const void* omega_mont, const void* coset_gen_mont, int rank,
                         int world) {
    GG_CHECK(omega_mont && coset_gen_mont, GG_ERR_INVALID_ARG, "null argument");
    GG_CHECK(curve == GG_CURVE_BN254 || curve == GG_CURVE_BLS12_381, GG_ERR_INVALID_ARG, "bad curve");
    GG_CHECK(world >= 1 && world <= 16 && (world & (world - 1)) == 0, GG_ERR_UNSUPPORTED,
             "distributed computeH: world must be a power of two <= 16");
    GG_CHECK(rank >= 0 && rank < world, GG_ERR_INVALID_ARG, "rank out of range");
    int lw = 0;
    while ((1 << lw) < world) lw++;
    GG_CHECK(log_n >= 1 && log_n <= 28 && log_n >= 2 * lw, GG_ERR_INVALID_ARG,
             "distributed computeH needs 2^log_n >= world^2");
    std::unique_ptr<gg_hshard> hs(new gg_hshard());
    hs->curve = curve;
    hs->log_n = log_n;
    hs->rank = rank;
    hs->world = world;
    hs->log_w = lw;
    hs->n = (size_t)1 << log_n;
    hs->M = log_n - lw;
    hs->m = hs->n >> lw;
    hs->chunk = hs->m >> lw;
    if (curve == GG_CURVE_BN254) {
        hs->bn.reset(new HShardT<FrCfg>());
        hshard_build(hs.get(), hs->bn.get(), omega_mont, coset_gen_mont);
    } else {
        hs->bls.reset(new HShardT<FrBlsCfg>());
        hshard_build(hs.get(), hs->bls.get(), omega_mont, coset_gen_mont);
    }
    return hs.release();
}

void hshard_run(gg_hshard* hs, const Fr* a, const Fr* b, const Fr* c, size_t len, bool compact, Fr* send,
                Fr* recv, gg_exchange_fn xchg, void* ctx, hipStream_t st) {
    std::lock_guard<std::mutex> lk(hs->mu);
    auto exchange = [&](int phase) {
        GG_WAIT_STREAM(st);
        set_last_error("");
        int rc = xchg(ctx, send, recv, hshard_exchange_bytes(hs, phase));
        if (rc == GG_ERR_TIMEOUT) throw Error(rc, gg_last_error());
        const std::string why = gg_last_error();
        GG_CHECK(rc == 0, GG_ERR_INTERNAL,
                 "exchange callback failed after phase " + std::to_string(phase) + (why.empty() ? "" : ": " + why));
    };
    hshard_phase1(hs, a, b, c, len, send, st, compact);
    exchange(1);
    hshard_phase2(hs, recv, send, st);
    exchange(2);
    hshard_phase3(hs, recv, send, st);
    exchange(3);
    hshard_phase4(hs, recv, hshard_h(hs), st);
}
}

extern "C" int gg_hshard_create_ex(int curve, int log_n, const void* omega_mont, const void* coset_gen_mont,
                                   int rank, int world, gg_hshard_t* out) {
    GG_CAPI_BEGIN
    GG_CHECK(out, GG_ERR_INVALID_ARG, "null argument");
    *out = hshard_create(curve, log_n, omega_mont, coset_gen_mont, rank, world);
    GG_CAPI_END
}

extern "C" int gg_hshard_create(int log_n, const void* omega_mont, const void* coset_gen_mont, int rank,
                                int world, gg_hshard_t* out) {
    return gg_hshard_create_ex(GG_CURVE_BN254, log_n, omega_mont, coset_gen_mont, rank, world, out);
}

extern "C" int gg_hshard_release(gg_hshard_t hs) {
    GG_CAPI_BEGIN
    delete hs;
    GG_CAPI_END
}

extern "C" int gg_hshard_info(gg_hshard_t hs, size_t* m, size_t* exchange_bytes) {
    GG_CAPI_BEGIN
    GG_CHECK(hs, GG_ERR_INVALID_ARG, "null argument");
    if (m) *m = hs->m;
    if (exchange_bytes) *exchange_bytes = hs->world * hshard_exchange_bytes(hs, 1);
    GG_CAPI_END
}

extern "C" int gg_hshard_exchange_bytes(gg_hshard_t hs, int phase, size_t* bytes_per_rank) {
    GG_CAPI_BEGIN
    GG_CHECK(hs && bytes_per_rank, GG_ERR_INVALID_ARG, "null argument");
    GG_CHECK(phase >= 1 && phase <= 3, GG_ERR_INVALID_ARG, "phase must be 1..3");
    *bytes_per_rank = hshard_exchange_bytes(hs, phase);
    GG_CAPI_END
}

extern "C" int gg_hshard_phase(gg_hshard_t hs, int phase, const void* a, const void* b, const void* c,
                               size_t len, int inputs_on_device, const void* recv, void* send_or_h,
                               void* hip_stream) {
    GG_CAPI_BEGIN
    GG_CHECK(hs && send_or_h, GG_ERR_INVALID_ARG, "null argument");
    std::lock_guard<std::mutex> lk(hs->mu);
    hipStream_t st = pick_stream(hip_stream);
    if (phase == 1) {
        GG_CHECK(a && b && c, GG_ERR_INVALID_ARG, "null input");
        GG_CHECK(len <= hs->n, GG_ERR_INVALID_ARG, "len > domain cardinality");
        const Fr* src[3] = {(const Fr*)a, (const Fr*)b, (const Fr*)c};
        if (!inputs_on_device) {
            DevBuf& full = hs->curve == GG_CURVE_BN254 ? hs->bn->full : hs->bls->full;
            full.reserve(3 * std::max<size_t>(len, 1) * 32);
            for (int i = 0; i < 3; i++) {
                Fr* d = full.as<Fr>() + i * len;
                if (len) GG_HIP(hipMemcpyAsync(d, src[i], len * 32, hipMemcpyHostToDevice, st));
                src[i] = d;
            }
        }
        hshard_phase1(hs, src[0], src[1], src[2], len, (Fr*)send_or_h, st);
    } else {
        GG_CHECK(recv, GG_ERR_INVALID_ARG, "null recv");
        if (phase == 2) hshard_phase2(hs, (const Fr*)recv, (Fr*)send_or_h, st);
        else if (phase == 3) hshard_phase3(hs, (const Fr*)recv, (Fr*)send_or_h, st);
        else if (phase == 4) hshard_phase4(hs, (const Fr*)recv, (Fr*)send_or_h, st);
        else throw Error(GG_ERR_INVALID_ARG, "phase must be 1..4");
    }
    GG_WAIT_STREAM(st);
    GG_CAPI_END
}
```

Measured before the change: 154.1 million.

## Batch G1 MSM tails across proof MSMs and read short NTT sources directly

```diff
diff --git a/gnark-fork_amd/csrc/groth16.hip b/gnark-fork_amd/csrc/groth16.hip
--- a/gnark-fork_amd/csrc/groth16.hip
+++ b/gnark-fork_amd/csrc/groth16.hip
@@ -17,7 +17,8 @@
 struct MsmSort;
 struct MsmScratch;
 struct MsmWork;
-void compute_h_device(gg_domain* d, Fr* A, Fr* B, Fr* C, Fr* H, hipStream_t st);
+void compute_h_device(gg_domain* d, const Fr* a, const Fr* b, const Fr* c, size_t len, Fr* A, Fr* B, Fr* C, Fr* H,
+                      hipStream_t st);
 void msm_device(gg_msm_base* b, const Fr* scalars_dev, void* out_jac, hipStream_t st);
 size_t msm_scalars_needed(gg_msm_base* b);
 gg_msm_base* msm_base_create_internal(int group, const void* host_points, size_t n,
@@ -28,6 +29,9 @@
 void msm_prepare_dev(gg_msm_base* b, MsmSort* s, const Fr* scalars_dev, hipStream_t st, int slog = 0,
                      uint32_t sres = 0);
 void msm_finish_dev(gg_msm_base* b, MsmSort* s, void* out_jac, hipStream_t st, MsmScratch* scr = nullptr);
+std::shared_ptr<void> msm_accum_dev(gg_msm_base* b, MsmSort* s, hipStream_t st, MsmScratch* scr = nullptr);
+void msm_tail_dev(int group, void* const* acc, int m, void* const* out_jac, hipStream_t st, MsmScratch* scr);
+MsmScratch* msm_own_scratch(gg_msm_base* b);
 MsmWork* msm_work_new();
 void msm_work_delete(MsmWork* w);
 MsmSort* msm_work_sort(MsmWork* w);
@@ -128,6 +132,7 @@
     }
     hipStream_t* act[5] = {};
     hipStream_t hprio = nullptr;
+    hipEvent_t acc_ev[4] = {};
     std::unique_ptr<Stager> stager;
     int device = 0;
     std::mutex mu;
@@ -139,6 +144,8 @@
         if (dom) gg_domain_release(dom);
         task_streams_release(tq, 5, device);
         if (hprio) (void)hipStreamDestroy(hprio);
+        for (hipEvent_t e : acc_ev)
+            if (e) (void)hipEventDestroy(e);
     }
 };
 
@@ -521,7 +528,13 @@
     }
     double t_up = now_ms();
 
-    set_g1_inf(pk->curve, out.z);
+    const bool tail_batch = getenv("GG_G16_TAIL_BATCH") && atoi(getenv("GG_G16_TAIL_BATCH")) != 0;
+    const int g1 = pk->curve == GG_CURVE_BN254 ? GG_G1 : GG_BLS12_381_G1;
+    std::shared_ptr<void> acc[4];
+    if (tail_batch)
+        for (hipEvent_t& e : pk->acc_ev)
+            if (!e) GG_HIP(hipEventCreateWithFlags(&e, hipEventDisableTiming));
+    for (void* p : {(void*)out.a, (void*)out.b1, (void*)out.k, (void*)out.z}) set_g1_inf(pk->curve, p);
     double t_h = 0, t_z = 0, t_a = 0, t_b = 0, t_k = 0, t_upabc = 0;
     std::mutex emu;
     std::string werr;
@@ -554,11 +567,7 @@
         len = n_cons;
         const double a = now_ms();
         if (inputs_on_device) {
-            for (int i = 0; i < 3; i++) {
-                if (dh) { dst[i] = (Fr*)src[i]; continue; }
-                if (n_cons) GG_HIP(hipMemcpyAsync(dst[i], src[i], n_cons * 32, hipMemcpyDeviceToDevice, pk->s1));
-                if (n_cons < n) GG_HIP(hipMemsetAsync((char*)dst[i] + n_cons * 32, 0, nbytes - n_cons * 32, pk->s1));
-            }
+            for (int i = 0; i < 3; i++) dst[i] = (Fr*)src[i];
         } else if (dh) {
             int rank = 0, world = 1, lg = 0;
             hshard_m(dh->hs, &rank, &world, &lg);
@@ -581,6 +590,17 @@
     pk->sa.reserve(nbytes);
     pk->sb.reserve(nbytes);
     pk->sc.reserve(nbytes);
+    auto msm_g1 = [&](int which, gg_msm_base_t b, MsmSort* srt, MsmScratch* scr, void* out_jac, hipStream_t st) {
+        if (!tail_batch) return msm_finish_dev(b, srt, out_jac, st, scr);
+        acc[which] = msm_accum_dev(b, srt, st, scr);
+        GG_HIP(hipEventRecord(pk->acc_ev[which], st));
+        if (serial) GG_WAIT_STREAM(st);
+    };
+    auto msm_z = [&](const Fr* h) {
+        if (!tail_batch) return msm_device(pk->Z, h, out.z, pk->s1);
+        msm_prepare_dev(pk->Z, msm_own_sort(pk->Z), h, pk->s1);
+        msm_g1(3, pk->Z, msm_own_sort(pk->Z), nullptr, out.z, pk->s1);
+    };
     if (dh) spawn(guarded([&] {
         Fr *A, *B, *C;
         size_t len;
@@ -591,7 +611,7 @@
         GG_WAIT_STREAM(pk->s1);
         double b = now_ms();
         t_h = b - a;
-        msm_device(pk->Z, hshard_h(dh->hs), out.z, pk->s1);
+        msm_z(hshard_h(dh->hs));
         t_z = now_ms() - b;
     }));
     else spawn(guarded([&] {
@@ -599,12 +619,14 @@
         size_t len;
         double a = now_ms();
         inputs_abc(A, B, C, len);
-        compute_h_device(pk->dom, A, B, C, A, pk->s1);
+        Fr* H = pk->sa.as<Fr>();
+        compute_h_device(pk->dom, A, B, C, inputs_on_device ? len : n, H, pk->sb.as<Fr>(), pk->sc.as<Fr>(), H,
+                         pk->s1);
         GG_WAIT_STREAM(pk->s1);
         double b = now_ms();
         t_h = b - a;
-        if (h_dev_out) GG_HIP(hipMemcpyAsync(h_dev_out, A, nbytes, hipMemcpyDeviceToDevice, pk->s1));
-        if (n > 1) msm_device(pk->Z, A + pk->z_lo, out.z, pk->s1);
+        if (h_dev_out) GG_HIP(hipMemcpyAsync(h_dev_out, H, nbytes, hipMemcpyDeviceToDevice, pk->s1));
+        if (n > 1) msm_z(H + pk->z_lo);
         t_z = now_ms() - b;
     }));
     MsmSort *sAK = nullptr, *sB = nullptr, *sK = nullptr, *sB2 = nullptr;
@@ -631,9 +653,32 @@
     })();
     double t2 = now_ms(), te = t2;
     if (wcode == GG_OK) {
-        spawn(guarded([&] { double a = now_ms(); msm_finish_dev(pk->A, sAK, out.a, pk->s2, xA); t_a = now_ms() - a; }));
-        spawn(guarded([&] { double a = now_ms(); msm_finish_dev(pk->B, sB, out.b1, pk->s3, xB); t_b = now_ms() - a; }));
-        spawn(guarded([&] { double a = now_ms(); msm_finish_dev(pk->K, sK, out.k, pk->s4, xK); t_k = now_ms() - a; }));
+        spawn(guarded([&] { double a = now_ms(); msm_g1(0, pk->A, sAK, xA, out.a, pk->s2); t_a = now_ms() - a; }));
+        spawn(guarded([&] { double a = now_ms(); msm_g1(1, pk->B, sB, xB, out.b1, pk->s3); t_b = now_ms() - a; }));
+        spawn(guarded([&] { double a = now_ms(); msm_g1(2, pk->K, sK, xK, out.k, pk->s4); t_k = now_ms() - a; }));
+        if (tail_batch) {
+            std::vector<gg::Task<void>> g1_tasks(workers.begin(), workers.end());
+            spawn(guarded([&, g1_tasks] {
+                for (auto& w : g1_tasks) w.wait();
+                {
+                    std::lock_guard<std::mutex> g(emu);
+                    if (wcode != GG_OK) return;
+                }
+                const double a = now_ms();
+                void* members[4];
+                void* outs[4];
+                void* const all_out[4] = {out.a, out.b1, out.k, out.z};
+                int m = 0;
+                for (int i = 0; i < 4; i++) {
+                    if (!acc[i]) continue;
+                    GG_HIP(hipStreamWaitEvent(pk->s2, pk->acc_ev[i], 0));
+                    members[m] = acc[i].get();
+                    outs[m++] = all_out[i];
+                }
+                if (m) msm_tail_dev(g1, members, m, outs, pk->s2, xA ? xA : msm_own_scratch(pk->A));
+                t_z += now_ms() - a;
+            }));
+        }
         t2 = now_ms();
         guarded([&] { msm_finish_dev(pk->B2, sB2, out.b2, pk->s0, xB2); })();
         te = now_ms();
diff --git a/gnark-fork_amd/csrc/msm.hip b/gnark-fork_amd/csrc/msm.hip
--- a/gnark-fork_amd/csrc/msm.hip
+++ b/gnark-fork_amd/csrc/msm.hip
@@ -1,5 +1,6 @@
 #include "msm_impl.cuh"
 #include <cmath>
+#include <memory>
 
 namespace gg {
 void create_base_g1(gg_msm_base* b, const void* points, size_t n, int on_device,
@@ -18,6 +19,10 @@
 void msm_finish_g1(gg_msm_base* b, MsmSort* s, MsmScratch* scr, void* out_jac, hipStream_t st);
 void msm_finish_g2(gg_msm_base* b, MsmSort* s, MsmScratch* scr, void* out_jac, hipStream_t st);
 void msm_finish_bls(gg_msm_base* b, MsmSort* s, MsmScratch* scr, void* out_jac, hipStream_t st);
+std::shared_ptr<void> msm_accum_g1(gg_msm_base* b, MsmSort* s, MsmScratch* scr, hipStream_t st);
+std::shared_ptr<void> msm_accum_bls(gg_msm_base* b, MsmSort* s, MsmScratch* scr, hipStream_t st);
+void msm_tail_g1(void* const* acc, int m, MsmScratch* scr, void* const* out_jac, hipStream_t st);
+void msm_tail_bls(void* const* acc, int m, MsmScratch* scr, void* const* out_jac, hipStream_t st);
 void msm_run_batch_g1(gg_msm_base* b, MsmWork* w, const VecPtrs& vp, int nvec, void* const* out_jac, hipStream_t st);
 void msm_run_batch_g2(gg_msm_base* b, MsmWork* w, const VecPtrs& vp, int nvec, void* const* out_jac, hipStream_t st);
 void msm_run_batch_bls(gg_msm_base* b, MsmWork* w, const VecPtrs& vp, int nvec, void* const* out_jac, hipStream_t st);
@@ -127,6 +132,17 @@
     else if (b->group == GG_BLS12_381_G1) msm_finish_bls(b, s, scr, out_jac, st);
     else msm_finish_bls2(b, s, scr, out_jac, st);
 }
+std::shared_ptr<void> msm_accum_dev(gg_msm_base* b, MsmSort* s, hipStream_t st, MsmScratch* scr) {
+    if (!scr) scr = &b->own.scr;
+    GG_CHECK(b->group == GG_G1 || b->group == GG_BLS12_381_G1, GG_ERR_INTERNAL, "msm_accum_dev: G1 bases only");
+    return b->group == GG_G1 ? msm_accum_g1(b, s, scr, st) : msm_accum_bls(b, s, scr, st);
+}
+void msm_tail_dev(int group, void* const* acc, int m, void* const* out_jac, hipStream_t st, MsmScratch* scr) {
+    GG_CHECK(group == GG_G1 || group == GG_BLS12_381_G1, GG_ERR_INTERNAL, "msm_tail_dev: G1 bases only");
+    if (group == GG_G1) msm_tail_g1(acc, m, scr, out_jac, st);
+    else msm_tail_bls(acc, m, scr, out_jac, st);
+}
+MsmScratch* msm_own_scratch(gg_msm_base* b) { return &b->own.scr; }
 void msm_prepare_derived_dev(gg_msm_base* a, MsmSort* sa, gg_msm_base* b, MsmSort* sb, const uint32_t* bmap,
                              hipStream_t st) {
     if (b->n) msm_prepare_derived(a, sa, b, sb, bmap, st);
diff --git a/gnark-fork_amd/csrc/msm_bls.hip b/gnark-fork_amd/csrc/msm_bls.hip
--- a/gnark-fork_amd/csrc/msm_bls.hip
+++ b/gnark-fork_amd/csrc/msm_bls.hip
@@ -1,4 +1,5 @@
 #include "msm_impl.cuh"
+#include <memory>
 
 namespace gg {
 void create_base_bls(gg_msm_base* b, const void* points, size_t n, int on_device,
@@ -22,4 +23,21 @@
         memcpy(out_jac[v], &j, sizeof(j));
     }
 }
+std::shared_ptr<void> msm_accum_bls(gg_msm_base* b, MsmSort* s, MsmScratch* scr, hipStream_t st) {
+    GG_CHECK(s->nvec == 1, GG_ERR_INTERNAL, "msm_accum of a batch sort");
+    auto t = std::make_shared<MsmTail<FpBls>>();
+    msm_accumulate<FpBls>(b, s, scr, st, *t, true);
+    return t;
 }
+void msm_tail_bls(void* const* acc, int m, MsmScratch* scr, void* const* out_jac, hipStream_t st) {
+    MsmTail<FpBls>* tl[MAX_TAIL];
+    Xyzz<FpBls> r[MAX_TAIL];
+    GG_CHECK(m >= 1 && m <= MAX_TAIL, GG_ERR_INTERNAL, "msm_tail: 1..8 members");
+    for (int i = 0; i < m; i++) tl[i] = (MsmTail<FpBls>*)acc[i];
+    msm_tail_multi<FpBls>(tl, m, scr, st, r);
+    for (int i = 0; i < m; i++) {
+        Jac<FpBls> j = xyzz_to_jac(r[i]);
+        memcpy(out_jac[i], &j, sizeof(j));
+    }
+}
+}
diff --git a/gnark-fork_amd/csrc/msm_g1.hip b/gnark-fork_amd/csrc/msm_g1.hip
--- a/gnark-fork_amd/csrc/msm_g1.hip
+++ b/gnark-fork_amd/csrc/msm_g1.hip
@@ -1,4 +1,5 @@
 #include "msm_impl.cuh"
+#include <memory>
 
 namespace gg {
 void create_base_g1(gg_msm_base* b, const void* points, size_t n, int on_device,
@@ -22,4 +23,21 @@
         memcpy(out_jac[v], &j, sizeof(j));
     }
 }
+std::shared_ptr<void> msm_accum_g1(gg_msm_base* b, MsmSort* s, MsmScratch* scr, hipStream_t st) {
+    GG_CHECK(s->nvec == 1, GG_ERR_INTERNAL, "msm_accum of a batch sort");
+    auto t = std::make_shared<MsmTail<Fp>>();
+    msm_accumulate<Fp>(b, s, scr, st, *t, true);
+    return t;
 }
+void msm_tail_g1(void* const* acc, int m, MsmScratch* scr, void* const* out_jac, hipStream_t st) {
+    MsmTail<Fp>* tl[MAX_TAIL];
+    Xyzz<Fp> r[MAX_TAIL];
+    GG_CHECK(m >= 1 && m <= MAX_TAIL, GG_ERR_INTERNAL, "msm_tail: 1..8 members");
+    for (int i = 0; i < m; i++) tl[i] = (MsmTail<Fp>*)acc[i];
+    msm_tail_multi<Fp>(tl, m, scr, st, r);
+    for (int i = 0; i < m; i++) {
+        G1Jac j = xyzz_to_jac(r[i]);
+        memcpy(out_jac[i], &j, sizeof(j));
+    }
+}
+}
diff --git a/gnark-fork_amd/csrc/msm_impl.cuh b/gnark-fork_amd/csrc/msm_impl.cuh
--- a/gnark-fork_amd/csrc/msm_impl.cuh
+++ b/gnark-fork_amd/csrc/msm_impl.cuh
@@ -725,13 +725,11 @@
 }
 
 template <class F>
-__global__ void __launch_bounds__(256) k_bucket_runsum(const typename PartialOf<F>::T* Sr, uint32_t nseg, int logL,
-                                                        Xyzz<F>* Dout, Xyzz<F>* Rout) {
+__device__ __forceinline__ void bucket_runsum_lane(const typename PartialOf<F>::T* Sr, uint32_t nseg, int logL,
+                                                   uint32_t t, Xyzz<F>* Dout, Xyzz<F>* Rout) {
     using O = PartialOps<F>;
     using T = typename O::T;
     constexpr bool kPf = !std::is_same<F, Fp2>::value;
-    const uint32_t t = blockIdx.x * blockDim.x + threadIdx.x;
-    if (t >= nseg) return;
     const int L = 1 << logL, steps = 2 * L + logL + 1;
     T R = O::inf(), A = O::inf(), cur, nxt;
     if constexpr (kPf) nxt = ld(Sr + (size_t)(L - 1) * nseg + t);
@@ -768,6 +766,34 @@
         }
     }
     st(Dout + t, to_std(A));
+}
+template <class F>
+__global__ void __launch_bounds__(256) k_bucket_runsum(const typename PartialOf<F>::T* Sr, uint32_t nseg, int logL,
+                                                        Xyzz<F>* Dout, Xyzz<F>* Rout) {
+    const uint32_t t = blockIdx.x * blockDim.x + threadIdx.x;
+    if (t >= nseg) return;
+    bucket_runsum_lane<F>(Sr, nseg, logL, t, Dout, Rout);
+}
+constexpr int MAX_TAIL = 8;
+template <class F>
+struct RunsumJob {
+    const typename PartialOf<F>::T* Sr;
+    Xyzz<F>*D, *R;
+    uint32_t nseg;
+    int logL;
+};
+template <class F>
+struct RunsumJobs {
+    RunsumJob<F> j[MAX_TAIL];
+    int n;
+};
+template <class F>
+__global__ void __launch_bounds__(256) k_bucket_runsum_multi(RunsumJobs<F> J) {
+    uint32_t t = blockIdx.x * blockDim.x + threadIdx.x;
+    int q = 0;
+    while (q < J.n && t >= J.j[q].nseg) { t -= J.j[q].nseg; q++; }
+    if (q >= J.n) return;
+    bucket_runsum_lane<F>(J.j[q].Sr, J.j[q].nseg, J.j[q].logL, t, J.j[q].D, J.j[q].R);
 }
 
 constexpr int MAX_GATHER = 192;
@@ -1155,6 +1181,14 @@
     for (int r = 0; r < nres; r++) out[r] = finish(r);
     return out;
 }
+inline size_t red_host_items(uint32_t n, bool plain) {
+    uint32_t HOST_N = 8;
+    if (const char* e = getenv("GG_RED_HOST_N")) HOST_N = (uint32_t)std::max(2, atoi(e));
+    if (n <= HOST_N) return 1;
+    const int mlg = (31 - __builtin_clz(n)) / 2;
+    const uint32_t M = 1u << mlg, rows = n >> mlg;
+    return plain ? red_host_items(rows, true) : red_host_items(rows, false) + red_host_items(M, false);
+}
 template <class F>
 inline Xyzz<F> reduce_terms(std::vector<RedItem<F>> items, MsmScratch* scr, hipStream_t st) {
     return reduce_terms_multi<F>(std::move(items), 1, scr, st)[0];
@@ -1193,12 +1227,22 @@
 }
 
 template <class F>
-inline void msm_finish_multi(gg_msm_base* b, MsmSort* s, MsmScratch* scr, hipStream_t st, Xyzz<F>* out) {
+struct MsmTail {
+    std::vector<RedItem<F>> terms;
+    size_t nb = 0;
+    bool runsum = false;
+    RunsumJob<F> job{};
+};
+template <class F>
+inline void msm_accumulate(gg_msm_base* b, MsmSort* s, MsmScratch* scr, hipStream_t st, MsmTail<F>& tl,
+                           bool defer_runsum) {
     const int slog = s->slog, nvec = s->nvec, kp = s->kp;
     const size_t n = b->n, nb = (b->nb >> slog) * (size_t)kp;
     const int ce = b->c - slog;
     const int Gb = b->G, Ge = b->G * kp;
-    for (int v = 0; v < nvec; v++) out[v] = Xyzz<F>::inf();
+    tl.terms.clear();
+    tl.runsum = false;
+    tl.nb = nb;
     if (n == 0) return;
     GG_HIP(hipStreamWaitEvent(st, s->ready_ev, 0));
     const uint32_t* offs = s->offsets.as<uint32_t>();
@@ -1282,22 +1326,23 @@
             hipLaunchKernelGGL(k_bucket_sum_r<F>, dim3(grid_for(nb, 256)), dim3(256), 0, st, (const PT*)hP,
                                (const PT*)tP, (const PT*)SP, offs, (uint32_t)nb, ce, K, logL, Sr);
             GG_HIP(hipGetLastError());
-            hipLaunchKernelGGL(k_bucket_runsum<F>, dim3(grid_for((size_t)G * Tg, 256)), dim3(256), 0, st,
-                               (const PT*)Sr, (uint32_t)(G * Tg), logL, D, Rs);
-            GG_HIP(hipGetLastError());
+            if (defer_runsum) {
+                tl.runsum = true;
+                tl.job = RunsumJob<F>{(const PT*)Sr, D, Rs, (uint32_t)(G * Tg), logL};
+            } else {
+                hipLaunchKernelGGL(k_bucket_runsum<F>, dim3(grid_for((size_t)G * Tg, 256)), dim3(256), 0, st,
+                                   (const PT*)Sr, (uint32_t)(G * Tg), logL, D, Rs);
+                GG_HIP(hipGetLastError());
+            }
             ps_acc2.stop(st);
-            ProfScope ps_red("msm_reduce", st, (double)nb);
             const int sneg = slog ? -(int)((1u << slog) - 1u - s->sres) : 0;
-            std::vector<RedItem<F>> terms;
+            std::vector<RedItem<F>>& terms = tl.terms;
             for (int jg = 0; jg < nvec * Gb; jg++) {
                 const int j = jg % Gb, v = jg / Gb;
                 terms.push_back({(const Xyzz<F>*)Rs + (size_t)jg * Tg, Tg, 1u, j * b->c + logL + slog, false, 1, v});
                 terms.push_back({(const Xyzz<F>*)D + (size_t)jg * Tg, Tg, 0u, j * b->c + slog, true, 1, v});
                 if (sneg) terms.push_back({(const Xyzz<F>*)Rs + (size_t)jg * Tg, Tg, 0u, j * b->c, true, sneg, v});
             }
-            const std::vector<Xyzz<F>> res = reduce_terms_multi<F>(std::move(terms), nvec, scr, st);
-            for (int v = 0; v < nvec; v++) out[v] = res[v];
-            ps_red.stop(st);
             return;
         }
     }
@@ -1337,17 +1382,71 @@
         GG_HIP(hipGetLastError());
     }
     ps_acc2.stop(st);
-    ProfScope ps_red("msm_reduce", st, (double)nb);
     const int sneg = slog ? -(int)((1u << slog) - 1u - s->sres) : 0;
-    std::vector<RedItem<F>> terms;
+    std::vector<RedItem<F>>& terms = tl.terms;
     for (int jg = 0; jg < nvec * Gb; jg++) {
         const int j = jg % Gb, v = jg / Gb;
         const Xyzz<F>* Sj = (const Xyzz<F>*)S + (size_t)jg * nbg;
         terms.push_back({Sj, (uint32_t)nbg, 1u, j * b->c + slog, false, 1, v});
         if (sneg) terms.push_back({Sj, (uint32_t)nbg, 0u, j * b->c, true, sneg, v});
     }
-    const std::vector<Xyzz<F>> res = reduce_terms_multi<F>(std::move(terms), nvec, scr, st);
+}
+
+template <class F>
+inline void msm_finish_multi(gg_msm_base* b, MsmSort* s, MsmScratch* scr, hipStream_t st, Xyzz<F>* out) {
+    const int nvec = s->nvec;
+    for (int v = 0; v < nvec; v++) out[v] = Xyzz<F>::inf();
+    MsmTail<F> tl;
+    msm_accumulate<F>(b, s, scr, st, tl, false);
+    if (tl.terms.empty()) return;
+    ProfScope ps_red("msm_reduce", st, (double)tl.nb);
+    const std::vector<Xyzz<F>> res = reduce_terms_multi<F>(std::move(tl.terms), nvec, scr, st);
     for (int v = 0; v < nvec; v++) out[v] = res[v];
+    ps_red.stop(st);
+}
+
+template <class F>
+inline void msm_tail_multi(MsmTail<F>* const* tails, int m, MsmScratch* scr, hipStream_t st, Xyzz<F>* out) {
+    GG_CHECK(m >= 1 && m <= MAX_TAIL, GG_ERR_INTERNAL, "msm_tail_multi: 1..8 members");
+    size_t nb = 0;
+    for (int i = 0; i < m; i++) nb += tails[i]->nb;
+    ProfScope ps_red("msm_reduce", st, (double)nb);
+    RunsumJobs<F> J;
+    J.n = 0;
+    size_t lanes = 0;
+    for (int i = 0; i < m; i++) {
+        out[i] = Xyzz<F>::inf();
+        if (!tails[i]->runsum) continue;
+        J.j[J.n++] = tails[i]->job;
+        lanes += tails[i]->job.nseg;
+        tails[i]->runsum = false;
+    }
+    if (J.n) {
+        GG_CHECK(lanes < 0xffffff00ull, GG_ERR_INTERNAL, "msm_tail_multi: too many segments");
+        hipLaunchKernelGGL(k_bucket_runsum_multi<F>, dim3(grid_for(lanes, 256)), dim3(256), 0, st, J);
+        GG_HIP(hipGetLastError());
+    }
+    for (int i0 = 0; i0 < m;) {
+        std::vector<RedItem<F>> items;
+        size_t pieces = 0;
+        int i1 = i0;
+        for (; i1 < m; i1++) {
+            size_t p = 0;
+            for (const auto& it : tails[i1]->terms) p += red_host_items(it.n, it.plain);
+            if (i1 > i0 && pieces + p > (size_t)MAX_GATHER) break;
+            pieces += p;
+            for (auto it : tails[i1]->terms) {
+                GG_CHECK(it.res == 0, GG_ERR_INTERNAL, "msm_tail_multi: member of a batch sort");
+                it.res = i1 - i0;
+                items.push_back(it);
+            }
+        }
+        if (!items.empty()) {
+            const std::vector<Xyzz<F>> res = reduce_terms_multi<F>(std::move(items), i1 - i0, scr, st);
+            for (int i = i0; i < i1; i++) out[i] = res[i - i0];
+        }
+        i0 = i1;
+    }
     ps_red.stop(st);
 }
 
diff --git a/gnark-fork_amd/csrc/ntt.hip b/gnark-fork_amd/csrc/ntt.hip
--- a/gnark-fork_amd/csrc/ntt.hip
+++ b/gnark-fork_amd/csrc/ntt.hip
@@ -50,6 +50,7 @@
     const F* ea;
     const F* eb;
     int canon_out;
+    uint32_t src_len;
 };
 
 template <class F>
@@ -136,7 +137,7 @@
 
 __device__ __forceinline__ int lidx(int e) { return e + (e >> 5); }
 
-template <class F, int NB, bool DIT>
+template <class F, int NB, bool DIT, bool SRCLEN = false>
 __device__ __forceinline__ void ntt_round(const PassParams<F>& P, uint32_t* lds, int TP, int T, int qlo,
                                           bool first, bool last, uint32_t base_hi, uint32_t lo0) {
     constexpr int R = 1 << NB;
@@ -157,7 +158,8 @@
         if (first) {
 #pragma unroll
             for (int m = 0; m < R; m++) {
-                x[m] = ld_fr(P.in + g[m]);
+                if constexpr (SRCLEN) x[m] = g[m] < P.src_len ? ld_fr(P.in + g[m]) : F::zero();
+                else x[m] = ld_fr(P.in + g[m]);
                 if (P.has_pre) x[m] = apply_scale(P.pre, g[m], P.log_n, x[m]);
             }
         } else {
@@ -226,7 +228,7 @@
 constexpr int kNttThreads = MAXNB == 3 ? 256 : (MAXNB == 2 ? 512 : 1024);
 template <int MAXNB>
 constexpr int kNttWaves = MAXNB == 3 ? 1 : (MAXNB == 2 ? 4 : 8);
-template <class F, bool DIT, int MAXNB>
+template <class F, bool DIT, int MAXNB, bool SRCLEN = false>
 __global__ void __launch_bounds__(kNttThreads<MAXNB>, kNttWaves<MAXNB>) k_ntt_pass(PassParams<F> P) {
     extern __shared__ __attribute__((aligned(16))) uint32_t lds[];
     const int k = P.k, tl = P.tl;
@@ -241,7 +243,7 @@
     if (k == 0) {
         for (int e = threadIdx.x; e < T; e += blockDim.x) {
             uint32_t g = base_hi | (lo0 + (uint32_t)e);
-            F x = ld_fr(P.in + g);
+            F x = (!SRCLEN || g < P.src_len) ? ld_fr(P.in + g) : F::zero();
             if (P.has_pre) x = apply_scale(P.pre, g, P.log_n, x);
             if (P.has_post) x = apply_scale(P.post, g, P.log_n, x);
             if (P.epi_mul_sub) x = ld_fr(P.ea + g) * ld_fr(P.eb + g) - x;
@@ -260,7 +262,7 @@
         if (!first) __syncthreads();
         if constexpr (MAXNB >= 3) {
             if (nb == 3) {
-                ntt_round<F, 3, DIT>(P, lds, TP, T, qlo, first, last, base_hi, lo0);
+                ntt_round<F, 3, DIT, SRCLEN>(P, lds, TP, T, qlo, first, last, base_hi, lo0);
                 first = false;
                 done += nb;
                 continue;
@@ -268,13 +270,13 @@
         }
         if constexpr (MAXNB >= 2) {
             if (nb == 2) {
-                ntt_round<F, 2, DIT>(P, lds, TP, T, qlo, first, last, base_hi, lo0);
+                ntt_round<F, 2, DIT, SRCLEN>(P, lds, TP, T, qlo, first, last, base_hi, lo0);
                 first = false;
                 done += nb;
                 continue;
             }
         }
-        ntt_round<F, 1, DIT>(P, lds, TP, T, qlo, first, last, base_hi, lo0);
+        ntt_round<F, 1, DIT, SRCLEN>(P, lds, TP, T, qlo, first, last, base_hi, lo0);
         first = false;
         done += nb;
     }
@@ -377,9 +379,11 @@
 template <class C>
 void run_transform(DomainT<C>* d, const Fe<C>* in, Fe<C>* out, bool dit, bool inverse_tw, int pre_kind,
                    int post_kind, const Fe<C>* ea, const Fe<C>* eb, hipStream_t st, int epi = EPI_MUL_SUB,
-                   const std::vector<Pass>* only = nullptr) {
+                   const std::vector<Pass>* only = nullptr, size_t src_len = (size_t)-1) {
     using F = Fe<C>;
     const int L = d->log_n;
+    const bool short_src = src_len < d->n;
+    GG_CHECK(!(short_src && dit), GG_ERR_INTERNAL, "short source on a DIT transform");
     auto passes = only ? *only : plan_passes(L, dit);
     const F* src = in;
     for (size_t pi = 0; pi < passes.size(); pi++) {
@@ -407,18 +411,23 @@
         int T = 1 << (ps.k + ps.tl);
         unsigned tiles = (unsigned)(d->n / (size_t)T);
         size_t lds = (ps.k > 3) ? (size_t)(T + (T >> 5)) * 32 : 0;
+        const bool srclen = short_src && pi == 0;
+        P.src_len = srclen ? (uint32_t)src_len : 0u;
         ProfScope prof("ntt_pass", st, (double)d->n);
         static const int radix = ntt_radix();
         if (radix == 4) {
             lds = (ps.k > 2) ? (size_t)(T + (T >> 5)) * 32 : 0;
             if (dit) hipLaunchKernelGGL((k_ntt_pass<F, true, 2>), dim3(tiles), dim3(512), lds, st, P);
+            else if (srclen) hipLaunchKernelGGL((k_ntt_pass<F, false, 2, true>), dim3(tiles), dim3(512), lds, st, P);
             else hipLaunchKernelGGL((k_ntt_pass<F, false, 2>), dim3(tiles), dim3(512), lds, st, P);
         } else if (radix == 2) {
             lds = (ps.k > 1) ? (size_t)(T + (T >> 5)) * 32 : 0;
             if (dit) hipLaunchKernelGGL((k_ntt_pass<F, true, 1>), dim3(tiles), dim3(1024), lds, st, P);
+            else if (srclen) hipLaunchKernelGGL((k_ntt_pass<F, false, 1, true>), dim3(tiles), dim3(1024), lds, st, P);
             else hipLaunchKernelGGL((k_ntt_pass<F, false, 1>), dim3(tiles), dim3(1024), lds, st, P);
         } else {
             if (dit) hipLaunchKernelGGL((k_ntt_pass<F, true, 3>), dim3(tiles), dim3(256), lds, st, P);
+            else if (srclen) hipLaunchKernelGGL((k_ntt_pass<F, false, 3, true>), dim3(tiles), dim3(256), lds, st, P);
             else hipLaunchKernelGGL((k_ntt_pass<F, false, 3>), dim3(tiles), dim3(256), lds, st, P);
         }
         GG_HIP(hipGetLastError());
@@ -560,19 +569,26 @@
 
 namespace gg {
 template <class C>
-static void compute_h_t(DomainT<C>* d, Fe<C>* A, Fe<C>* B, Fe<C>* Cv, Fe<C>* H, hipStream_t st) {
+static void compute_h_t(DomainT<C>* d, const Fe<C>* a, const Fe<C>* b, const Fe<C>* c, size_t len, Fe<C>* A,
+                        Fe<C>* B, Fe<C>* Cv, Fe<C>* H, hipStream_t st) {
     const Fe<C>* nul = nullptr;
-    run_transform(d, A, A, false, true, -1, SK_H_FWD, nul, nul, st);
+    GG_CHECK(len <= d->n, GG_ERR_INTERNAL, "computeH: len > domain cardinality");
+    GG_CHECK((a == A && b == B && c == Cv) ? len == d->n : (a != A && b != B && c != Cv), GG_ERR_INTERNAL,
+             "computeH: sources in place need len = n");
+    run_transform(d, a, A, false, true, -1, SK_H_FWD, nul, nul, st, EPI_MUL_SUB, nullptr, len);
     run_transform(d, A, A, true, false, -1, -1, nul, nul, st);
-    run_transform(d, B, B, false, true, -1, SK_H_FWD, nul, nul, st);
+    run_transform(d, b, B, false, true, -1, SK_H_FWD, nul, nul, st, EPI_MUL_SUB, nullptr, len);
     run_transform(d, B, B, true, false, -1, -1, (const Fe<C>*)A, nul, st, EPI_MUL);
-    run_transform(d, Cv, Cv, false, true, -1, SK_DEN_N, nul, nul, st);
+    run_transform(d, c, Cv, false, true, -1, SK_DEN_N, nul, nul, st, EPI_MUL_SUB, nullptr, len);
     GG_CHECK(H != Cv, GG_ERR_INTERNAL, "computeH: h must not alias c");
     run_transform(d, B, H, false, true, -1, SK_H_INV, (const Fe<C>*)Cv, nul, st, EPI_SUB);
 }
-void compute_h_device(gg_domain* dom, Fr* A, Fr* B, Fr* C, Fr* H, hipStream_t st) {
-    if (dom->curve == GG_CURVE_BN254) compute_h_t(dom->bn.get(), A, B, C, H, st);
-    else compute_h_t(dom->bls.get(), (FrBls*)A, (FrBls*)B, (FrBls*)C, (FrBls*)H, st);
+void compute_h_device(gg_domain* dom, const Fr* a, const Fr* b, const Fr* c, size_t len, Fr* A, Fr* B, Fr* C,
+                      Fr* H, hipStream_t st) {
+    if (dom->curve == GG_CURVE_BN254) compute_h_t(dom->bn.get(), a, b, c, len, A, B, C, H, st);
+    else
+        compute_h_t(dom->bls.get(), (const FrBls*)a, (const FrBls*)b, (const FrBls*)c, len, (FrBls*)A, (FrBls*)B,
+                    (FrBls*)C, (FrBls*)H, st);
 }
 }
 
@@ -590,14 +606,17 @@
     Fr* A = (Fr*)base;
     Fr* B = (Fr*)(base + nb);
     Fr* C = (Fr*)(base + 2 * nb);
-    hipMemcpyKind kind = inputs_on_device ? hipMemcpyDeviceToDevice : hipMemcpyHostToDevice;
-    const void* src[3] = {a, b, c};
-    Fr* dst[3] = {A, B, C};
-    for (int i = 0; i < 3; i++) {
-        if (len) GG_HIP(hipMemcpyAsync(dst[i], src[i], len * 32, kind, st));
-        if (len < d->n) GG_HIP(hipMemsetAsync((char*)dst[i] + len * 32, 0, nb - len * 32, st));
-    }
-    compute_h_device(d, A, B, C, (Fr*)h_dev, st);
+    if (inputs_on_device) {
+        compute_h_device(d, (const Fr*)a, (const Fr*)b, (const Fr*)c, len, A, B, C, (Fr*)h_dev, st);
+    } else {
+        const void* src[3] = {a, b, c};
+        Fr* dst[3] = {A, B, C};
+        for (int i = 0; i < 3; i++) {
+            if (len) GG_HIP(hipMemcpyAsync(dst[i], src[i], len * 32, hipMemcpyHostToDevice, st));
+            if (len < d->n) GG_HIP(hipMemsetAsync((char*)dst[i] + len * 32, 0, nb - len * 32, st));
+        }
+        compute_h_device(d, A, B, C, d->n, A, B, C, (Fr*)h_dev, st);
+    }
     GG_WAIT_STREAM(st);
     GG_CAPI_END
 }
```

New measurement: 155.0 million (median of 6 runs). Within noise of the previous version (+0.6%).
